# EdwardjkFeng/gradslam

Measured on AMD Instinct MI355X. Metric: RGB-D frames/sec (640x480, 10 ICP iters), higher is better.
Workload: dtype f32; 1 GPU; c2: ICP odometry localisation step, 640x480 TUM-shape synthetic RGB-D, batch 1 per GPU, dsratio 4 (~19k x ~19k points), 10 LM iterations, map 288269 points; parallelism=one sequence per GPU, final RCCL all_gather of poses, timing=one timed region of 1356 steps

## Files before the change

### gradslam_amd/_native.py

```python
import ctypes
import os
import subprocess

import torch

_HERE = os.path.dirname(os.path.abspath(__file__))
LIB_PATH = os.path.join(_HERE, "libgradslam_hip.so")
CSRC = os.path.join(_HERE, "csrc")

c_i, c_i64, c_f, c_p, c_sz = ctypes.c_int, ctypes.c_int64, ctypes.c_float, ctypes.c_void_p, ctypes.c_size_t

SIGNATURES = {
    "gs_abi_version": (c_i, []),
    "gs_last_error": (ctypes.c_char_p, []),
    "gs_vertex_normal_maps": (c_i, [c_p, c_p, c_p, c_i, c_i, c_i, c_i, c_p, c_p, c_p, c_p, c_p]),
    "gs_vertex_normal_maps_backward_ws_bytes": (c_sz, [c_i, c_i, c_i, c_i]),
    "gs_vertex_normal_maps_backward": (c_i, [c_p, c_p, c_p, c_i, c_i, c_i, c_i, c_p, c_p, c_p, c_p, c_p, c_p, c_p,
                                             c_p, c_sz, c_p]),
    "gs_vertex_normal_maps_backward_det_ws_bytes": (c_sz, [c_i, c_i, c_i, c_i]),
    "gs_vertex_normal_maps_backward_det": (c_i, [c_p, c_p, c_p, c_i, c_i, c_i, c_i, c_p, c_p, c_p, c_p, c_p, c_p, c_p,
                                                 c_p, c_sz, c_p]),
    "gs_get_alpha": (c_i, [c_p, c_i64, c_f, c_f, c_p, c_p]),
    "gs_get_alpha_backward": (c_i, [c_p, c_i64, c_f, c_f, c_p, c_p, c_p]),
    "gs_frames_from_raw": (c_i, [c_p, c_p, c_i, c_i, c_i, c_i, c_i, c_f, c_i, c_p, c_p, c_p]),
    "gs_compact_ws_bytes": (c_sz, [c_i64]),
    "gs_compact_rows": (c_i, [c_p, c_p, c_i64, c_i, c_p, c_p, c_p, c_sz, c_p]),
    "gs_compact_multi": (c_i, [c_i, c_p, c_p, c_p, c_p, c_i64, c_p, c_p, c_sz, c_p]),
    "gs_expand_multi": (c_i, [c_i, c_p, c_p, c_p, c_p, c_i64, c_p, c_sz, c_p]),
    "gs_append_rows_ws_bytes": (c_sz, [c_i64]),
    "gs_append_rows": (c_i, [c_i, c_p, c_p, c_p, c_p, c_i64, c_p, c_i, c_p, c_p, c_p, c_sz, c_p]),
    "gs_fusion_merge_inplace_ws_bytes": (c_sz, [c_i, c_i]),
    "gs_fusion_merge_inplace": (c_i, [c_p, c_p, c_i64, c_p, c_p, c_p, c_p, c_i, c_i, c_i, c_i, c_p, c_p, c_p, c_p, c_p, c_p,
                                      c_sz, c_p]),
    "gs_aggregate_update_ws_bytes": (c_sz, [c_i, c_i, c_i]),
    "gs_aggregate_update": (c_i, [c_p, c_p, c_p, c_p, c_i, c_i, c_i, c_p, c_p, c_p, c_p, c_i, c_p, c_p, c_sz, c_p]),
    "gs_pointfusion_update_ws_bytes": (c_sz, [c_i, c_i, c_i, c_i]),
    "gs_pointfusion_update": (c_i, [c_p, c_p, c_p, c_p, c_i, c_i, c_i, c_p, c_p, c_p, c_p, c_p, c_i, c_f, c_f, c_f, c_p, c_p,
                                    c_sz, c_p]),
    "gs_downsample_frame_ws_bytes": (c_sz, [c_i, c_i, c_i]),
    "gs_downsample_frame": (c_i, [c_p, c_p, c_p, c_p, c_i, c_i, c_i, c_i, c_i, c_p, c_p, c_p, c_p, c_p, c_p, c_sz, c_p]),
    "gs_build_icp_target_ws_bytes": (c_sz, [c_i, c_i, c_i, c_i]),
    "gs_build_icp_target": (c_i, [c_p, c_p, c_i64, c_i, c_i, c_i, c_i, c_p, c_p, c_i, c_i, c_p, c_p, c_p, c_p, c_p, c_p, c_p,
                                  c_p, c_p, c_sz, c_p]),
    "gs_bucket_by_pixel_ws_bytes": (c_sz, [c_i, c_i, c_i, c_i]),
    "gs_bucket_by_pixel": (c_i, [c_p, c_p, c_i64, c_i, c_i, c_i, c_i, c_p, c_i, c_i, c_p, c_p, c_p, c_p, c_p, c_sz, c_p]),
    "gs_project_active_ws_bytes": (c_sz, [c_i, c_i]),
    "gs_project_active": (c_i, [c_p, c_p, c_i, c_i, c_p, c_p, c_i, c_i, c_i, c_p, c_p, c_p, c_sz, c_p]),
    "gs_gather_table_rows_ws_bytes": (c_sz, [c_i]),
    "gs_gather_table_rows": (c_i, [c_p, c_p, c_i64, c_p, c_i, c_i, c_i, c_i, c_p, c_p, c_p, c_sz, c_p]),
    "gs_table_ds_mask": (c_i, [c_p, c_i64, c_i, c_p, c_p]),
    "gs_knn1_ws_bytes": (c_sz, [c_i]),
    "gs_knn1": (c_i, [c_p, c_p, c_i, c_p, c_p, c_i, c_p, c_p, c_sz, c_p]),
    "gs_knn1_bruteforce": (c_i, [c_p, c_p, c_i, c_p, c_p, c_i, c_p, c_p]),
    "gs_knn1_unpack": (c_i, [c_p, c_p, c_i, c_p, c_p, c_p]),
    "gs_icp_linearize_ws_bytes": (c_sz, [c_i]),
    "gs_icp_linearize": (c_i, [c_p, c_p, c_i, c_p, c_p, c_p, c_f, c_p, c_p, c_sz, c_p]),
    "gs_icp_rows": (c_i, [c_p, c_p, c_i, c_p, c_p, c_p, c_f, c_p, c_p, c_p, c_p]),
    "gs_icp_linearize_backward": (c_i, [c_p, c_p, c_i, c_p, c_p, c_p, c_f, c_p, c_p, c_p, c_p, c_p]),
    "gs_icp_linearize_backward_det_ws_bytes": (c_sz, [c_i, c_i]),
    "gs_icp_linearize_backward_det": (c_i, [c_p, c_p, c_i, c_p, c_p, c_p, c_i, c_p, c_f, c_p, c_p, c_p, c_p, c_p, c_sz, c_p]),
    "gs_transform_points": (c_i, [c_p, c_p, c_i, c_p, c_p, c_p]),
    "gs_icp_ws_bytes": (c_sz, [c_i, c_i]),
    "gs_icp_point_to_plane": (c_i, [c_p, c_p, c_i, c_p, c_p, c_p, c_i, c_p, c_i, c_f, c_f, c_p, c_p, c_p, c_p, c_p, c_sz,
                                    c_p]),
    "gs_icp_point_to_plane_grad": (c_i, [c_p, c_p, c_i, c_p, c_p, c_p, c_i, c_p, c_i, c_f, c_f, c_f, c_f, c_f, c_f,
                                         c_p, c_p, c_p, c_p, c_p, c_sz, c_p]),
    "gs_icp_tape_bytes": (c_sz, [c_i, c_i, c_i]),
    "gs_icp_point_to_plane_taped": (c_i, [c_p, c_p, c_i, c_p, c_p, c_p, c_i, c_p, c_i, c_f, c_f, c_i, c_f, c_f, c_f, c_f,
                                          c_p, c_p, c_p, c_p, c_sz, c_p, c_sz, c_p]),
    "gs_icp_backward_ws_bytes": (c_sz, [c_i]),
    "gs_icp_point_to_plane_backward": (c_i, [c_p, c_p, c_i, c_p, c_p, c_p, c_i, c_p, c_i, c_f, c_i, c_f, c_f, c_f, c_f, c_p, c_sz,
                                             c_p, c_p, c_p, c_p, c_p, c_p, c_sz, c_p]),
    "gs_icp_backward_det_ws_bytes": (c_sz, [c_i, c_i, c_i, c_i]),
    "gs_icp_point_to_plane_backward_det": (c_i, [c_p, c_p, c_i, c_p, c_p, c_p, c_i, c_p, c_i, c_f, c_i, c_f, c_f, c_f, c_f, c_p,
                                                 c_sz, c_p, c_p, c_p, c_p, c_p, c_p, c_sz, c_p]),
    "gs_slam_localize_tape_bytes": (c_sz, [c_i, c_i, c_i, c_i, c_i, c_i, c_i]),
    "gs_slam_localize_taped": (c_i, [c_p, c_p, c_p, c_p, c_i, c_i, c_i, c_i, c_p, c_p, c_p, c_i, c_i, c_i, c_f, c_f, c_f, c_f,
                                     c_f, c_f, c_p, c_p, c_sz, c_p, c_sz, c_p]),
    "gs_slam_localize_backward_ws_bytes": (c_sz, [c_i, c_i, c_i, c_i, c_i]),
    "gs_slam_localize_backward": (c_i, [c_p, c_i, c_i, c_i, c_i, c_p, c_p, c_i, c_i, c_i, c_f, c_f, c_f, c_f, c_f, c_p, c_sz,
                                        c_p, c_p, c_p, c_p, c_p, c_i, c_p, c_sz, c_p]),
    "gs_slam_localize_backward_det_ws_bytes": (c_sz, [c_i, c_i, c_i, c_i, c_i, c_i, c_i]),
    "gs_slam_localize_backward_det": (c_i, [c_p, c_i, c_i, c_i, c_i, c_p, c_p, c_i, c_i, c_i, c_f, c_f, c_f, c_f, c_f, c_p, c_sz,
                                            c_p, c_p, c_p, c_p, c_p, c_i, c_p, c_sz, c_p]),
    "gs_pointfusion_update_tape_bytes": (c_sz, [c_i, c_i, c_i]),
    "gs_pointfusion_update_taped": (c_i, [c_p, c_p, c_p, c_p, c_i, c_i, c_i, c_p, c_p, c_p, c_p, c_p, c_i, c_f, c_f, c_f, c_p, c_p,
                                          c_sz, c_p, c_sz, c_p]),
    "gs_pointfusion_update_backward_ws_bytes": (c_sz, [c_i, c_i, c_i]),
    "gs_pointfusion_update_backward": (c_i, [c_p, c_p, c_p, c_p, c_i, c_i, c_i, c_p, c_p, c_p, c_p, c_p, c_i, c_f, c_p, c_sz,
                                             c_p, c_p, c_p, c_p, c_p, c_p, c_p, c_p, c_p, c_sz, c_p]),
    "gs_compose_poses": (c_i, [c_p, c_p, c_i, c_p, c_p]),
    "gs_set_graph_mode": (None, [c_i]),
    "gs_graph_stats": (c_i, [ctypes.POINTER(ctypes.c_double)]),
    "gs_slam_localize_ws_bytes": (c_sz, [c_i, c_i, c_i, c_i, c_i]),
    "gs_slam_localize": (c_i, [c_p, c_p, c_p, c_i, c_i, c_i, c_i, c_p, c_p, c_p, c_i, c_i, c_i, c_f, c_f, c_f, c_f, c_f,
                               c_f, c_p, c_p, c_p, c_p, c_p, c_p, c_sz, c_p]),
    "gs_set_grid_search": (None, [c_i]),
    "gs_set_fused_setup": (None, [c_i]),
    "gs_set_tile_points": (None, [c_i]),
    "gs_set_loop_waves": (c_i, [c_i]),
    "gs_icp_launch_geometry": (c_i, [c_i, c_i, ctypes.POINTER(c_i), ctypes.POINTER(c_i), ctypes.POINTER(c_i)]),
    "gs_loop_counts": (c_i, [ctypes.POINTER(ctypes.c_uint), c_i]),
    "gs_profile_enable": (None, [c_i]),
    "gs_profile_read": (c_i, [c_i, ctypes.POINTER(ctypes.c_long), ctypes.POINTER(ctypes.c_double)]),
    "gs_fusion_similar": (c_i, [c_p, c_p, c_i64, c_p, c_p, c_i, c_i, c_p, c_p, c_i, c_f, c_f, c_p, c_p, c_p]),
    "gs_fusion_unique_ws_bytes": (c_sz, [c_i, c_i, c_i]),
    "gs_fusion_unique": (c_i, [c_p, c_p, c_p, c_i64, c_p, c_i, c_i, c_i, c_p, c_p, c_i, c_p, c_p, c_p, c_sz, c_p]),
    "gs_fusion_merge_ws_bytes": (c_sz, [c_i, c_i]),
    "gs_fusion_merge": (c_i, [c_p, c_p, c_i64, c_p, c_p, c_p, c_p, c_i, c_i, c_i, c_i, c_p, c_p, c_p, c_p, c_p, c_p,
                              c_p, c_p, c_p, c_p, c_sz, c_p]),
    "gs_fusion_merge_backward": (c_i, [c_p, c_p, c_i64, c_p, c_p, c_p, c_p, c_i, c_i, c_i, c_i, c_p, c_p, c_p, c_p,
                                       c_p, c_p, c_p, c_p, c_p, c_p, c_p, c_p, c_p, c_p, c_p, c_p, c_p, c_p, c_sz,
                                       c_p]),
    "gs_fusion_new_mask": (c_i, [c_p, c_p, c_p, c_i64, c_i, c_i, c_i, c_p, c_p]),
    "gs_render_map_ws_bytes": (c_sz, [c_i, c_i, c_i]),
    "gs_render_map": (c_i, [c_p, c_p, c_p, c_p, c_i, c_i, c_p, c_p, c_i, c_i, c_p, c_p, c_p, c_p, c_p, c_p, c_sz, c_p]),
    "gs_render_map_backward_ws_bytes": (c_sz, [c_i, c_i, c_i]),
    "gs_render_map_backward": (c_i, [c_p, c_p, c_i, c_i, c_p, c_i, c_i, c_p, c_p, c_p, c_p, c_p, c_p, c_p, c_p, c_p, c_p, c_sz,
                                     c_p]),
    "gs_chamfer_ws_bytes": (c_sz, [c_i, c_i, c_i]),
    "gs_chamfer": (c_i, [c_p, c_p, c_i, c_p, c_p, c_i, c_i, c_f, c_i, c_p, c_p, c_p, c_p, c_sz, c_p]),
    "gs_chamfer_backward_ws_bytes": (c_sz, [c_i, c_i, c_i]),
    "gs_chamfer_backward": (c_i, [c_p, c_p, c_i, c_p, c_p, c_i, c_i, c_p, c_p, c_p, c_p, c_p, c_p, c_p, c_sz, c_p]),
    "gs_chamfer_backward_det_ws_bytes": (c_sz, [c_i, c_i, c_i]),
    "gs_chamfer_backward_det": (c_i, [c_p, c_p, c_i, c_p, c_p, c_i, c_i, c_p, c_p, c_p, c_p, c_p, c_p, c_p, c_sz, c_p]),
}

_lib = None


def build(verbose: bool = False) -> str:
    cmd = ["make", "-s", "-C", CSRC, "-j4"]
    if verbose:
        cmd.remove("-s")
    subprocess.check_call(cmd)
    return LIB_PATH


def lib() -> ctypes.CDLL:
    global _lib
    if _lib is None:
        if not os.path.exists(LIB_PATH):
            raise RuntimeError(
                "gradslam_amd: native library {} is missing -- build it with "
                "`python -c 'import __graft_entry__ as g; g.build()'` (needs hipcc). "
                "There is no CPU / PyTorch fallback for the hot path.".format(LIB_PATH)
            )
        handle = ctypes.CDLL(LIB_PATH)
        for name, (res, args) in SIGNATURES.items():
            fn = getattr(handle, name)
            fn.restype, fn.argtypes = res, args
        if handle.gs_abi_version() != 3:
            raise RuntimeError("gradslam_amd: ABI version mismatch")
        _lib = handle
    return _lib


def ptr(t):
    return None if t is None else t.data_ptr()


_raw_stream = getattr(torch._C, "_cuda_getCurrentRawStream", None)
_raw_device = getattr(torch._C, "_cuda_getDevice", None)


def stream():
    if _raw_stream is not None and _raw_device is not None:
        return _raw_stream(_raw_device())
    return torch.cuda.current_stream().cuda_stream


def current_device_index() -> int:
    return _raw_device() if _raw_device is not None else torch.cuda.current_device()


def require_hip(*tensors, op: str = "op"):
    cur = None
    for t in tensors:
        if t is None:
            continue
        if not t.is_cuda:
            raise RuntimeError(
                "gradslam_amd.{}: tensor is on {}; the ICP / PointFusion hot path only runs on a HIP "
                "device (no CPU fallback is provided).".format(op, t.device)
            )
        if cur is None:
            cur = current_device_index()
        if t.device.index != cur:
            raise RuntimeError(
                "gradslam_amd.{}: tensor is on {} but the current HIP device is cuda:{}; kernels are launched on "
                "the current device's stream -- call torch.cuda.set_device({}) (or wrap the call in "
                "`with torch.cuda.device(...)`) first.".format(op, t.device, cur, t.device.index)
            )


def call(name: str, *args):
    rc = getattr(lib(), name)(*args)
    if rc != 0:
        msg = lib().gs_last_error().decode("utf-8", "replace")
        raise RuntimeError("{} failed (code {}): {}".format(name, rc, msg))


def ws_bytes(name: str, *args) -> int:
    return int(getattr(lib(), name)(*args))


_ws_cache = {}


def workspace(nbytes: int, device, tag: str = "default") -> torch.Tensor:
    key = (str(device), stream(), tag)
    buf = _ws_cache.get(key)
    if buf is None or buf.numel() < nbytes:
        buf = torch.empty(1 << max(int(nbytes) - 1, 255).bit_length(), dtype=torch.uint8, device=device)
        _ws_cache[key] = buf
    return buf
```

### gradslam_amd/csrc/gs_drivers.hpp

```cpp
#pragma once

#include "gs_common.hpp"
#include "gs_project.hpp"

namespace gs {

int vertex_normal_maps_cam(const float *depth, const float *intrinsics, const float *poses, int B, int H, int W, float *vertex,
                           float *normal, float *gvertex, float *gnormal, float *cam_out, hipStream_t st);
int vertex_normal_maps_fusion(const float *depth, const float *intrinsics, const float *poses, int B, int H, int W, float *gvertex,
                              float *gnormal, float *alpha, float sigma, float eps, unsigned long long *pix_key, unsigned int *pix_n,
                              int32_t *zero, int n_zero, hipStream_t st);

constexpr int kBucketPixMax = 24 * 1024;
size_t project_target1_ws_bytes(int H, int W, int ds, int Nmax);
int project_target1(const float *points, const int32_t *counts, int Nmax, const float *poses, const float *intrinsics, int H, int W, int ds,
                    const float *map_normals, int cap, int64_t *rows, int32_t *nrows, float *tgt, float *tnrm, int32_t *nt,
                    float *scan_points, int32_t *scan_orig, int32_t *pix_start, int32_t *tgt_index, int32_t *tgt_pix, void *ws,
                    size_t ws_bytes, hipStream_t st, const DsJob *frame);
int project_front1(const float *depth, const float *points, const int32_t *counts, int Nmax, const float *poses, const float *intrinsics,
                   int H, int W, int ds, const float *map_normals, int cap, float *vertex, float *normal, float *gvertex, float *gnormal,
                   float *cam_out, int32_t *row_pix, float *tgt, float *tnrm, int32_t *nt, int32_t *tgt_index, float *scan_points,
                   int32_t *scan_orig, int32_t *pix_start, const DsJob &frame, void *ws, size_t ws_bytes, hipStream_t st);

size_t fusion_corr_state_bytes(int B, int H, int W, int Nmax);
void fusion_corr_init_ptrs(void *state, int B, int H, int W, int Nmax, unsigned long long **pix_key, unsigned int **pix_n);
int fusion_correspond(void *state, const float *map_points, const float *map_normals, const float *map_ccounts, const int32_t *counts,
                      int B, int Nmax, const float *poses, const float *intrinsics, int H, int W, const float *gvertex,
                      const float *gnormal, float dist_th, float dot_th, int32_t *ctr, hipStream_t st);
int fusion_merge_corr(void *state, const int32_t *ctr, const float *gvertex, const float *gnormal, const float *rgb, const float *alpha,
                      int B, int H, int W, int Nmax, const int32_t *counts, float *points, float *normals, float *colors, float *ccounts,
                      hipStream_t st);
int fusion_append_corr(void *state, int B, int H, int W, int Nmax, int b, const float *depth, const float *const *h_src,
                       const int *h_row_floats, float *const *h_dst, const int32_t *d_count, int cap, int *d_total, void *cws,
                       hipStream_t st);
int fusion_finish(void *state, int B, int H, int W, int Nmax, int32_t *ctr, int32_t *counts, const int *totals, int cap, int32_t *appended,
                  int32_t *stats, hipStream_t st);
size_t fusion_tape_bytes(int B, int H, int W);
int fusion_tape_record(const void *state, void *tape, int B, int H, int W, int Nmax, const int32_t *counts, const float *points,
                       const float *normals, const float *colors, const float *ccounts, hipStream_t st);
int fusion_tape_appended(void *tape, int B, int H, int W, const int32_t *appended, hipStream_t st);
int fusion_update_reverse(const void *tape, int B, int H, int W, int Nmax, const float *depth, const float *gvertex, const float *gnormal,
                          const float *rgb, const float *alpha, float *points, float *normals, float *colors, float *ccounts,
                          int32_t *counts, float *Gp, float *Gn, float *Gc, float *Gcc, float *g_gvertex, float *g_gnormal, float *g_rgb,
                          float *g_alpha, void *cws, hipStream_t st);
int append_valid_pixels(int n_arrays, const float *depth_b, int64_t HW, const float *const *h_src, const int *h_row_floats,
                        float *const *h_dst, int32_t *d_count, int cap, int32_t *d_appended, int32_t *d_overflow, void *cws,
                        hipStream_t st);

}
```

### gradslam_amd/csrc/gs_icp.hpp

```cpp
#pragma once

#include "gs_common.hpp"

namespace gs {

bool profiling_enabled();
int icp_localize_run(int grad_lm, const float *src, const int32_t *d_ns, int max_ns, const float *tgt, const float *nrm,
                     const int32_t *d_nt, int max_nt, int numiters, float damp, float thresh, float lambda_max, float Bp,
                     float B2, float nu, const gs_icp_hints *hints, float *out_T, void *ws, size_t ws_bytes, hipStream_t st,
                     void *tape, size_t tape_bytes, const float *compose_right, float *compose_out);
int icp_config_stamp();

}
```

### gradslam_amd/csrc/gs_icp_loop.hpp

```cpp
#pragma once

#include "gs_icp_step.hpp"
#include "gs_project.hpp"

namespace gs {

struct LoopConst {
    const float *user_src, *tgt, *nrm, *boxes, *sboxes;
    const int32_t *d_ns, *d_nt;
    float *trace, *out_T;
    gs_icp_hints hints;
    GradParams gp;
    float thresh;
    int ns, nt;
    int cert_off;
    int tile_points;
    int grid_variant;
    CamK cam;
    int cam_ok;
    int32_t *cells;
    int cells_stride;
};

__device__ __forceinline__ f3 cam_point(const CamK &k, const f3 p) {
// ... 308 lines not shown
    }
    __syncthreads();
    if (step_mode >= 0 && blockIdx.x == 0 && threadIdx.x < kWords) {
        const int v = reinterpret_cast<const int *>(&st_sm)[threadIdx.x];
        reinterpret_cast<int *>(S_out)[threadIdx.x] = v;
        if (rec) reinterpret_cast<int *>(rec)[REC_WORDS + REC_STATE + threadIdx.x] = v;
    }
    GS_STAMP(7);
    const IcpState *S = &st_sm;
    if (tile0 >= ns) {
        if (threadIdx.x < NACC) partials[blockIdx.x * NACC + threadIdx.x] = 0.0f;
        return;
    }
    const int p_cur = S->p_cur, b_cur = S->b_cur;
    const float *in = first ? user_src : B.P(p_cur);
    float *out = B.P(out_slot >= 0 ? out_slot : 1 - p_cur);
    unsigned long long *best = B.N(out_slot >= 0 ? out_slot : 1 - b_cur);
    f3 s{0.0f, 0.0f, 0.0f};
    if (ok) {
        s = xform(S->dT, ld3(in, i));
        if (wave == 0) st3(out, i, s);
    }
    if (nt <= 0) {
        if (ok && wave == 0) best[i] = KEY_NONE;
        if (threadIdx.x < NACC) partials[blockIdx.x * NACC + threadIdx.x] = 0.0f;
        return;
    }
    unsigned long long key;
    bool need = false;
    int rel = 2;
    if (grid) {
        GS_STAMP(0);
        rel = sh.wflag[lane];
        if (wave == 0) {
            unsigned long long k0 = KEY_NONE;
            if (ok) {
                const int u = (first || b_cur == S_in->b_cur) ? 0 : 1;
                const float4 q = *reinterpret_cast<const float4 *>(sh.seed[u][lane]);
                k0 = pack_key(dist2(s, q.x, q.y, q.z), __float_as_int(q.w));
            }
            atomicMin(&sh.key[lane], k0);
        }
        {
            float bd = INFINITY;
            int bi = 0x7fffffff;
#pragma unroll
            for (int r = 0; r < WROWS; ++r) {
                const int wr = sh.win[r][lane];
                const int kk = (rel & 3) + r, wn = LaneWin::len(wr, nt);
                const int po = sh.band[WBANDS + min(kk, WBANDS - 1)];
                const float *row = sh.u.stage + 4 * (max(po, 0) + LaneWin::lo(wr) - sh.band[min(kk, WBANDS - 1)]);
                for (int p = wave; p < wn; p += NW) {
                    float4 q;
                    if (po >= 0) {
                        q = *reinterpret_cast<const float4 *>(row + 4 * p);
                    } else {
                        const int slot = LaneWin::lo(wr) + p;
                        const f3 g3 = ld3(C->hints.scan_points, slot);
                        q = make_float4(g3.x, g3.y, g3.z, __int_as_float(C->hints.scan_orig[slot]));
                    }
                    const float d = dist2(s, q.x, q.y, q.z);
                    const int jj = __float_as_int(q.w);
                    const bool better = (d < bd) | ((d == bd) & (jj < bi));
                    bd = better ? d : bd;
                    bi = better ? jj : bi;
                }
            }
            if (ok && bd < INFINITY) atomicMin(&sh.key[lane], pack_key(bd, bi));
        }
        __syncthreads();
        GS_STAMP(1);
        float bd;
        int bi;
        key_unpack(sh.key[lane], bd, bi);
        const float bound2 = (ok && C->cam_ok) ? cam_bound2(sh.cam, s, sh.centre[lane], rel >> 3) : 0.0f;
        const bool proven = !C->cert_off & ((rel & 4) != 0) & (bd * 1.0001f < bound2);
        need = ok & !proven;
        const unsigned long long need_mask = __ballot(need);
        GS_COUNT(12, (unsigned long long)__popcll(need_mask));
        bool tile_search = __popcll(need_mask) > 6;
        if (!tile_search && need_mask) {
            tile_search = !knn_point_search<NW>(sh, s, need_mask, C->hints.scan_points, C->hints.scan_orig, C->boxes, C->sboxes, nt);
        }
        if (tile_search) {
            tile_box(sh, s, need);
            __syncthreads();
            knn_prune_search<true, NW>(sh, s, ok, need, C->hints.scan_points, C->hints.scan_orig, C->boxes, C->sboxes, nt);
        }
        GS_STAMP(2);
        key = ok ? sh.key[lane] : KEY_NONE;
        GS_STAMP(3);
        GS_COUNT(5, ((unsigned long long)__builtin_amdgcn_s_getreg((31 << 11) | 4) << 16) |
                        ((unsigned long long)__builtin_amdgcn_s_getreg((31 << 11) | 20) << 48));
    } else {
        int sj = -1;
        if (!first) {
            sj = -2;
            if (wave == 0) {
                unsigned long long k0 = KEY_NONE;
                if (ok) {
                    const float4 q = *reinterpret_cast<const float4 *>(sh.seed[b_cur == S_in->b_cur ? 0 : 1][lane]);
                    k0 = pack_key(dist2(s, q.x, q.y, q.z), __float_as_int(q.w));
                }
                sh.key[lane] = k0;
            }
        }
        const bool window_seed = first && C->hints.scan_points && C->hints.src_pix && C->hints.pix_start && C->hints.grid_w > 0;
        if (window_seed) sj = -2;
        const float *scan = C->hints.scan_points ? C->hints.scan_points : C->tgt;
        const int32_t *scan_orig = C->hints.scan_points ? C->hints.scan_orig : nullptr;
        if (window_seed) knn_window_seed<NW>(sh, s, ok, i, C->hints, nt);
        key = knn_tile<NW>(sh, s, ok, sj, C->tgt, scan, scan_orig, C->boxes, C->sboxes, nt);
    }
    if (wave == 0) {
        if (ok) best[i] = key;
        if (grid && ok && C->cam_ok) C->cells[par * C->cells_stride + i] = cam_cell(sh.cam, s);
        float acc[NACC];
#pragma unroll
        for (int k = 0; k < NACC; ++k) acc[k] = 0.0f;
        const Row r = make_row_from(s, ok, key, C->tgt, C->nrm, C->thresh);
        if (r.valid) accumulate_row(r, acc);
#pragma unroll
        for (int k = 0; k < NACC; ++k) sh.u.a.rows[k][lane] = acc[k];
    }
    __syncthreads();
    static_assert(NACC * 16 <= NW * 64, "the J epilogue's first stage is one pass");
    if (threadIdx.x < NACC * 16) {
        const int k = threadIdx.x >> 4, p4 = (threadIdx.x & 15) * 4;
        sh.u.a.part[k][threadIdx.x & 15] = ((sh.u.a.rows[k][p4] + sh.u.a.rows[k][p4 + 1]) + sh.u.a.rows[k][p4 + 2]) + sh.u.a.rows[k][p4 + 3];
    }
    __syncthreads();
    if (threadIdx.x < NACC) {
        float v = 0.0f;
#pragma unroll
        for (int q = 0; q < 16; ++q) v += sh.u.a.part[threadIdx.x][q];
        partials[blockIdx.x * NACC + threadIdx.x] = v;
    }
}

__global__ void icp_init_state_k(IcpState *S, const float *__restrict__ init_T , float damp) {
    if (threadIdx.x == 0 && blockIdx.x == 0) {
        for (int i = 0; i < 16; ++i) {
            const float v = init_T ? init_T[i] : ((i % 5 == 0) ? 1.0f : 0.0f);
            S->T[i] = v; S->dT[i] = v;
        }
        for (int i = 0; i < 44; ++i) S->cur[i] = 0.0f;
        S->damp = damp;
        S->p_cur = 1;
        S->b_cur = 1; S->b_first = 0;
        S->it = 0;
    }
}

__global__ __launch_bounds__(SUPER * CHUNK) void icp_prepare_k(IcpState *S, const float *__restrict__ init_T, float damp,
                                                              const float *__restrict__ tgt, const int32_t *__restrict__ d_nt,
                                                              float *__restrict__ boxes, float *__restrict__ sboxes,
                                                              LoopConst lc, LoopConst *__restrict__ lc_out, float *__restrict__ part0,
                                                              float *__restrict__ part1, int rows_written, int rows_read) {
    static_assert(SUPER * CHUNK == 1024, "one block per super-box");
    for (int q = rows_written * NACC + blockIdx.x * blockDim.x + threadIdx.x; q < rows_read * NACC; q += gridDim.x * blockDim.x) {
        part0[q] = 0.0f; part1[q] = 0.0f;
    }
    __shared__ float wb[16][6];
    if (blockIdx.x == 0 && threadIdx.x < sizeof(LoopConst) / 4) {
        int v = reinterpret_cast<const int *>(&lc)[threadIdx.x];
        if (threadIdx.x == offsetof(LoopConst, ns) / 4) v = *lc.d_ns;
        if (threadIdx.x == offsetof(LoopConst, nt) / 4) v = *lc.d_nt;
        if (threadIdx.x == offsetof(LoopConst, tile_points) / 4) {
            atomicAdd(&g_loop_counts[0], 1u);
            if (lc.grid_variant) atomicAdd(&g_loop_counts[1], 1u);
            if (lc.tile_points != 64) atomicAdd(&g_loop_counts[2], 1u);
        }
        reinterpret_cast<int *>(lc_out)[threadIdx.x] = v;
    }
    if (lc.cells) {
        const int n = *lc.d_ns;
        int32_t *pix = lc.cells + 2 * (size_t)lc.cells_stride;
        for (int i = blockIdx.x * blockDim.x + threadIdx.x; i < lc.cells_stride; i += gridDim.x * blockDim.x)
            pix[i] = (i < n && lc.hints.src_pix) ? lc.hints.src_pix[i] : 0;
    }
    if (blockIdx.x == 0) {
        __syncthreads();
        if (threadIdx.x == 0 && lc.hints.cam_pose && lc.hints.cam_K && lc.hints.ds > 0) {
            const float *T = lc.hints.cam_pose, *K = lc.hints.cam_K;
            const Cam c = make_cam(T, K);
            for (int q = 0; q < 9; ++q) lc_out->cam.R[q] = c.R[q];
            for (int q = 0; q < 3; ++q) lc_out->cam.T[q] = c.tinv[q];
            lc_out->cam.fx = K[0]; lc_out->cam.fy = K[5]; lc_out->cam.cx = K[2]; lc_out->cam.cy = K[6];
            lc_out->cam.ds = lc.hints.ds; lc_out->cam.Wd = lc.hints.grid_w; lc_out->cam.Hd = lc.hints.grid_h;
            const bool pinhole = K[1] == 0.0f && K[3] == 0.0f && K[4] == 0.0f && K[7] == 0.0f && K[8] == 0.0f && K[9] == 0.0f &&
                                 K[10] == 1.0f && K[11] == 0.0f && K[0] != 0.0f && K[5] != 0.0f;
            lc_out->cam_ok = pinhole ? 1 : 0;
        }
    }
    if (threadIdx.x == 0 && blockIdx.x == 0) {
        for (int i = 0; i < 16; ++i) {
            const float v = init_T ? init_T[i] : ((i % 5 == 0) ? 1.0f : 0.0f);
            S->T[i] = v; S->dT[i] = v;
        }
        for (int i = 0; i < 44; ++i) S->cur[i] = 0.0f;
        for (int i = 0; i < 6; ++i) S->xi[i] = 0.0f;
        S->damp = damp;
        S->p_cur = 1;
        S->b_cur = 1; S->b_first = 0;
        S->it = 0;
    }
    const int nt = *d_nt;
    const int j = blockIdx.x * (SUPER * CHUNK) + threadIdx.x;
    if (blockIdx.x * (SUPER * CHUNK) >= nt) return;
    float lo[3] = {INFINITY, INFINITY, INFINITY}, hi[3] = {-INFINITY, -INFINITY, -INFINITY};
    if (j < nt) {
        const f3 p = ld3(tgt, j);
        lo[0] = hi[0] = p.x; lo[1] = hi[1] = p.y; lo[2] = hi[2] = p.z;
    }
#pragma unroll
    for (int a = 0; a < 3; ++a) {
#pragma unroll
        for (int off = CHUNK / 2; off > 0; off >>= 1) {
            lo[a] = fminf(lo[a], __shfl_xor(lo[a], off, kWave));
            hi[a] = fmaxf(hi[a], __shfl_xor(hi[a], off, kWave));
        }
    }
    if ((threadIdx.x % CHUNK) == 0 && j < nt) {
        float *b = boxes + 6 * (int64_t)(j / CHUNK);
        b[0] = lo[0]; b[1] = lo[1]; b[2] = lo[2]; b[3] = hi[0]; b[4] = hi[1]; b[5] = hi[2];
    }
#pragma unroll
    for (int a = 0; a < 3; ++a) {
#pragma unroll
        for (int off = 32; off >= CHUNK; off >>= 1) {
            lo[a] = fminf(lo[a], __shfl_xor(lo[a], off, kWave));
            hi[a] = fmaxf(hi[a], __shfl_xor(hi[a], off, kWave));
        }
    }
    const int lane = threadIdx.x & 63, wave = threadIdx.x >> 6;
    if (lane == 0) { wb[wave][0] = lo[0]; wb[wave][1] = lo[1]; wb[wave][2] = lo[2]; wb[wave][3] = hi[0]; wb[wave][4] = hi[1]; wb[wave][5] = hi[2]; }
    __syncthreads();
    if (threadIdx.x < 6) {
        float v = wb[0][threadIdx.x];
        for (int w = 1; w < 16; ++w) v = threadIdx.x < 3 ? fminf(v, wb[w][threadIdx.x]) : fmaxf(v, wb[w][threadIdx.x]);
        sboxes[6 * (int64_t)blockIdx.x + threadIdx.x] = v;
    }
}

__global__ void copy_best_last_k(const IcpState *__restrict__ S, LoopBufs B, const int32_t *__restrict__ d_ns,
                                 unsigned long long *__restrict__ out) {
    const unsigned long long *src = B.N(S->b_first);
    const int ns = *d_ns;
    for (int i = blockIdx.x * blockDim.x + threadIdx.x; i < ns; i += gridDim.x * blockDim.x) out[i] = src[i];
}

}
```

### gradslam_amd/csrc/icp.hip

```cpp
#include <stddef.h>
#include <stdlib.h>
#include <algorithm>
#include <vector>

#include "gs_detfold.hpp"
#include "gs_icp.hpp"
#include "gs_icp_reduce.hpp"

namespace gs {

__global__ __launch_bounds__(KNN_T) void knn1_brute_k(const float *__restrict__ src, const int32_t *__restrict__ d_ns,
                                                      const float *__restrict__ tgt, const int32_t *__restrict__ d_nt,
                                                      int nsplit, unsigned long long *__restrict__ best) {
    const int ns = *d_ns, nt = *d_nt;
    const int i = blockIdx.x * KNN_T + threadIdx.x;
    if (blockIdx.x * KNN_T >= ns) return;
    const int chunk = (nt + nsplit - 1) / nsplit;
    const int j0 = blockIdx.y * chunk, j1 = min(nt, j0 + chunk);
    const bool ok = i < ns;
    const f3 s = ok ? ld3(src, i) : f3{0.0f, 0.0f, 0.0f};
    float bd = INFINITY;
    int bi = 0;
    for (int j = j0; j < j1; ++j) {
        const float d = dist2(s, tgt[3 * j], tgt[3 * j + 1], tgt[3 * j + 2]);
        if (d < bd) { bd = d; bi = j; }
    }
    if (ok && bd < INFINITY) atomicMin(best + i, pack_key(bd, bi));
}

__global__ __launch_bounds__(64) void tgt_boxes_k(const float *__restrict__ tgt, const int32_t *__restrict__ d_nt,
                                                  float *__restrict__ boxes) {
    const int nt = *d_nt;
    const int j = blockIdx.x * 64 + threadIdx.x;
    if (blockIdx.x * 64 >= nt) return;
    float lo[3] = {INFINITY, INFINITY, INFINITY}, hi[3] = {-INFINITY, -INFINITY, -INFINITY};
    if (j < nt) {
        const f3 p = ld3(tgt, j);
        lo[0] = hi[0] = p.x; lo[1] = hi[1] = p.y; lo[2] = hi[2] = p.z;
    }
#pragma unroll
    for (int a = 0; a < 3; ++a) {
#pragma unroll
        for (int off = CHUNK / 2; off > 0; off >>= 1) {
            lo[a] = fminf(lo[a], __shfl_xor(lo[a], off, kWave));
            hi[a] = fmaxf(hi[a], __shfl_xor(hi[a], off, kWave));
        }
    }
    if ((threadIdx.x % CHUNK) == 0 && j < nt) {
        float *b = boxes + 6 * (int64_t)(j / CHUNK);
        b[0] = lo[0]; b[1] = lo[1]; b[2] = lo[2]; b[3] = hi[0]; b[4] = hi[1]; b[5] = hi[2];
    }
}

__global__ __launch_bounds__(KNN_BT) void knn1_box_k(const float *__restrict__ src, const int32_t *__restrict__ d_ns,
                                                     const float *__restrict__ tgt, const float *__restrict__ boxes,
                                                     const int32_t *__restrict__ d_nt, unsigned long long *__restrict__ best) {
    __shared__ KnnShared sh;
    const int ns = *d_ns, nt = *d_nt;
    const int tile0 = blockIdx.x * 64;
    if (tile0 >= ns) return;
    const int lane = threadIdx.x & 63, wave = threadIdx.x >> 6;
    const int i = tile0 + lane;
    const bool ok = i < ns;
    const f3 s = ok ? ld3(src, i) : f3{0.0f, 0.0f, 0.0f};
    if (nt <= 0) {
        if (ok && wave == 0) best[i] = KEY_NONE;
        return;
    }
    const unsigned long long key = knn_tile<KNN_NW>(sh, s, ok, -1, tgt, tgt, nullptr, boxes, nullptr, nt);
    if (ok && wave == 0) best[i] = key;
}

__global__ void knn_unpack_k(const unsigned long long *__restrict__ best, const int32_t *__restrict__ d_ns,
                             float *__restrict__ dist2_out, int64_t *__restrict__ idx) {
    const int ns = *d_ns;
    for (int i = blockIdx.x * blockDim.x + threadIdx.x; i < ns; i += gridDim.x * blockDim.x) {
        const unsigned long long k = best[i];
        if (dist2_out) dist2_out[i] = bitsf((uint32_t)(k >> 32));
        if (idx) idx[i] = (int64_t)(uint32_t)(k & 0xffffffffu);
    }
}

__global__ void fill_u64_k(unsigned long long *__restrict__ p, int n, unsigned long long v) {
    for (int i = blockIdx.x * blockDim.x + threadIdx.x; i < n; i += gridDim.x * blockDim.x) p[i] = v;
}

__global__ __launch_bounds__(LIN_T) void linearize_k(const float *__restrict__ src, const int32_t *__restrict__ d_ns,
                                                     const float *__restrict__ tgt, const float *__restrict__ nrm,
                                                     const unsigned long long *__restrict__ best, float thresh,
                                                     float *__restrict__ partials ) {
    const int ns = *d_ns;
    float acc[NACC];
#pragma unroll
    for (int k = 0; k < NACC; ++k) acc[k] = 0.0f;
    for (int i = blockIdx.x * LIN_T + threadIdx.x; i < ns; i += gridDim.x * LIN_T) {
        const Row r = make_row(src, tgt, nrm, best, i, ns, thresh);
        if (r.valid) accumulate_row(r, acc);
    }
    block_reduce_store(acc, partials);
}

__global__ __launch_bounds__(1024) void finalize44_k(const float *__restrict__ partials, int nblocks, float *__restrict__ out44) {
    __shared__ float acc[NACC];
    reduce_partials(partials, nblocks, acc);
    if (threadIdx.x == 0) expand44(acc, out44);
}

__global__ void icp_rows_k(const float *__restrict__ src, const int32_t *__restrict__ d_ns, const float *__restrict__ tgt,
                           const float *__restrict__ nrm, const unsigned long long *__restrict__ best, float thresh,
                           float *__restrict__ A, float *__restrict__ bvec, uint8_t *__restrict__ keep) {
    const int ns = *d_ns;
    for (int i = blockIdx.x * blockDim.x + threadIdx.x; i < ns; i += gridDim.x * blockDim.x) {
        const Row r = make_row(src, tgt, nrm, best, i, ns, thresh);
        keep[i] = r.valid ? 1 : 0;
#pragma unroll
        for (int u = 0; u < 6; ++u) A[6 * (int64_t)i + u] = r.valid ? r.a[u] : 0.0f;
        bvec[i] = r.valid ? r.b : 0.0f;
    }
}

template <bool DET>
__global__ void linearize_bwd_k(const float *__restrict__ src, const int32_t *__restrict__ d_ns,
                                const float *__restrict__ tgt, const float *__restrict__ nrm,
                                const unsigned long long *__restrict__ best, float thresh,
                                const float *__restrict__ gout , float *__restrict__ g_src,
                                float *__restrict__ g_tgt, float *__restrict__ g_nrm) {
    const int ns = *d_ns;
    __shared__ float G[43];
    if (threadIdx.x < 43) G[threadIdx.x] = gout[threadIdx.x];
    __syncthreads();
    for (int i = blockIdx.x * blockDim.x + threadIdx.x; i < ns; i += gridDim.x * blockDim.x) {
        const Row r = make_row(src, tgt, nrm, best, i, ns, thresh);
        if (!r.valid) {
            if (g_src) st3(g_src, i, f3{0, 0, 0});
            if (DET && g_tgt) det_store_none(g_tgt, i);
            continue;
        }
        const uint32_t j = (uint32_t)(best[i] & 0xffffffffu);
        const f3 s = ld3(src, i), d = ld3(tgt, j), n = ld3(nrm, j);
        float ab[6];
#pragma unroll
        for (int u = 0; u < 6; ++u) {
            float v = G[36 + u] * r.b;
#pragma unroll
            for (int w = 0; w < 6; ++w) v += (G[6 * u + w] + G[6 * w + u]) * r.a[w];
            ab[u] = v;
        }
        float bb = 2.0f * G[42] * r.b;
#pragma unroll
        for (int u = 0; u < 6; ++u) bb += G[36 + u] * r.a[u];
        const f3 an{ab[0], ab[1], ab[2]}, ac{ab[3], ab[4], ab[5]};
        f3 sb{n.y * ac.z - n.z * ac.y, n.z * ac.x - n.x * ac.z, n.x * ac.y - n.y * ac.x};
        f3 nb{an.x + (ac.y * s.z - ac.z * s.y), an.y + (ac.z * s.x - ac.x * s.z), an.z + (ac.x * s.y - ac.y * s.x)};
        sb.x -= bb * n.x; sb.y -= bb * n.y; sb.z -= bb * n.z;
        nb.x += bb * (d.x - s.x); nb.y += bb * (d.y - s.y); nb.z += bb * (d.z - s.z);
        if (g_src) st3(g_src, i, sb);
        if constexpr (DET) {
            if (g_tgt) det_store_row(g_tgt, i, f3{bb * n.x, bb * n.y, bb * n.z}, nb, (int)j);
            continue;
        }
        if (g_tgt) {
            atomicAdd(g_tgt + 3 * (int64_t)j, bb * n.x);
            atomicAdd(g_tgt + 3 * (int64_t)j + 1, bb * n.y);
            atomicAdd(g_tgt + 3 * (int64_t)j + 2, bb * n.z);
        }
        if (g_nrm) {
            atomicAdd(g_nrm + 3 * (int64_t)j, nb.x);
            atomicAdd(g_nrm + 3 * (int64_t)j + 1, nb.y);
            atomicAdd(g_nrm + 3 * (int64_t)j + 2, nb.z);
        }
    }
}

__global__ void transform_k(const float *__restrict__ pts, const int32_t *__restrict__ d_n, const float *__restrict__ T,
                            float *__restrict__ out) {
    const int n = *d_n;
    for (int i = blockIdx.x * blockDim.x + threadIdx.x; i < n; i += gridDim.x * blockDim.x) st3(out, i, xform(T, ld3(pts, i)));
}

}

#include "gs_icp_loop.hpp"
#include "gs_icp_bwd.hpp"

namespace gs {

static inline int knn_nsplit_brute(int max_ns, int max_nt) {
    const int tiles = cdiv(max_ns, KNN_T);
    int ns = cdiv(2048, tiles);
    const int cap = cdiv(max_nt, 64);
    if (ns > cap) ns = cap;
    if (ns < 1) ns = 1;
    if (ns > 4096) ns = 4096;
    return ns;
}
static inline int lin_blocks(int max_ns) {
    int nb = cdiv(max_ns, LIN_T);
    if (nb > LIN_MAXB) nb = LIN_MAXB;
    if (nb < 1) nb = 1;
    return nb;
}
static inline size_t boxes_bytes(int max_nt) { return align_up((size_t)cdiv(max_nt > 0 ? max_nt : 1, CHUNK) * 6 * 4, 256); }

struct Prof {
    bool on = false;
    std::vector<hipEvent_t> ev[2][2];
    size_t used[2] = {0, 0};
    double total_ms[2] = {0.0, 0.0};
    long count[2] = {0, 0};
};
static Prof g_prof;
static inline void prof_mark(int tag, int which, hipStream_t st) {
    if (!g_prof.on) return;
    auto &v = g_prof.ev[tag][which];
    const size_t i = g_prof.used[tag];
    if (i >= v.size()) {
        hipEvent_t e;
        if (hipEventCreate(&e) != hipSuccess) return;
        v.push_back(e);
    }
    (void)hipEventRecord(v[i], st);
    if (which == 1) g_prof.used[tag] = i + 1;
}

bool profiling_enabled() { return g_prof.on; }

static int g_grid_mode = getenv("GS_GRID_MODE") ? atoi(getenv("GS_GRID_MODE")) : 1;
static int g_tile_points = 0;
static int g_loop_waves = 0;

constexpr int TILE_MIN = 32;
static inline int loop_tile_points() {
    static const int env = getenv("GS_TILE_POINTS") ? atoi(getenv("GS_TILE_POINTS")) : 0;
    const int forced = g_tile_points ? g_tile_points : env;
    return (forced >= TILE_MIN && forced <= 64) ? forced : 64;
}
constexpr int LOOP_WAVES_DENSE = 64;
static inline int loop_waves(bool grid_search, int max_nt, int cells) {
    static const int env = getenv("GS_LOOP_WAVES") ? atoi(getenv("GS_LOOP_WAVES")) : 0;
    const int forced = g_loop_waves ? g_loop_waves : env;
    if (forced == 8 || forced == 16) return forced;
    return (grid_search && (int64_t)max_nt <= (int64_t)LOOP_WAVES_DENSE * cells) ? 8 : 16;
}
int icp_config_stamp() { return g_grid_mode | (g_tile_points << 4) | (g_loop_waves << 12); }
static inline int loop_blocks_max(int max_ns) { return cdiv(max_ns, TILE_MIN); }
static inline int partial_rows_alloc(int max_ns) { return std::max(loop_blocks_max(max_ns), 32 * RP_LOADS) + 1; }

struct IcpWs {
    IcpState *S[2];
    LoopBufs B;
    float *partials[2];
    float *boxes, *sboxes;
    LoopConst *lc;
    int32_t *cells;
};
static inline size_t icp_ws_layout(int max_ns, int max_nt, void *ws, IcpWs *out) {
    size_t off = 0;
    auto take = [&](size_t bytes) { size_t o = off; off += align_up(bytes, 256); return o; };
    const size_t oS = take(sizeof(IcpState)), oS1 = take(sizeof(IcpState));
    const size_t oP0 = take((size_t)max_ns * 12), oP1 = take((size_t)max_ns * 12);
    const size_t oB0 = take((size_t)max_ns * 8), oB1 = take((size_t)max_ns * 8);
    const size_t oPart = take((size_t)partial_rows_alloc(max_ns) * NACC * 4), oPart1 = take((size_t)partial_rows_alloc(max_ns) * NACC * 4);
    const size_t oBox = take(boxes_bytes(max_nt)), oSBox = take((size_t)cdiv(max_nt > 0 ? max_nt : 1, 1024) * 6 * 4);
    const size_t oLc = take(sizeof(LoopConst)), oCells = take((size_t)max_ns * 12);
    if (ws && out) {
        char *p = (char *)ws;
        out->S[0] = (IcpState *)(p + oS); out->S[1] = (IcpState *)(p + oS1);
        out->B.pts = (float *)(p + oP0);
        out->B.pts_stride = (int64_t)(oP1 - oP0) / 4;
        out->B.best = (unsigned long long *)(p + oB0);
        out->B.best_stride = (int64_t)(oB1 - oB0) / 8;
        out->partials[0] = (float *)(p + oPart); out->partials[1] = (float *)(p + oPart1);
        out->boxes = (float *)(p + oBox);
        out->sboxes = (float *)(p + oSBox);
        out->lc = (LoopConst *)(p + oLc);
        out->cells = (int32_t *)(p + oCells);
    }
    return off;
}

struct Tape {
    float *rec;
    LoopBufs B;
    int nslots;
};
static inline int tape_launches(bool grad, int numiters) { return grad ? 2 * numiters : numiters + 1; }
static inline size_t tape_layout(bool grad, int max_ns, int numiters, void *tape, Tape *out) {
    const int n = tape_launches(grad, numiters > 0 ? numiters : 1);
    const size_t rec_b = align_up((size_t)(n + 1) * REC_WORDS * 4, 256);
    const size_t pts_b = align_up((size_t)max_ns * 12, 256), best_b = align_up((size_t)max_ns * 8, 256);
    if (tape && out) {
        char *p = (char *)tape;
        out->rec = (float *)p;
        out->B.pts = (float *)(p + rec_b);
        out->B.pts_stride = (int64_t)pts_b / 4;
        out->B.best = (unsigned long long *)(p + rec_b + (size_t)n * pts_b);
        out->B.best_stride = (int64_t)best_b / 8;
        out->nslots = n;
    }
    return rec_b + (size_t)n * (pts_b + best_b);
}

static inline GradParams make_grad_params(float lambda_max, float B, float B2, float nu) {
    return GradParams{(float)(1.0 / (double)lambda_max), (float)((double)lambda_max - 1.0 / (double)lambda_max), B, B2,
                      (float)(1.0 / (double)nu)};
}
static inline GradParams lm_grad_params() { return GradParams{0.5f, 1.5f, 1.0f, 1.0f, 0.005f}; }

static int icp_run(bool grad, const float *src, const int32_t *d_ns, int max_ns, const float *tgt, const float *nrm,
                   const int32_t *d_nt, int max_nt, const float *init_T, int numiters, float damp, float thresh,
                   GradParams gp, const gs_icp_hints *hints_in, float *out_T, uint64_t *best_last, float *trace, void *ws,
                   size_t ws_bytes, hipStream_t st, const char *name, void *tape = nullptr, size_t tape_bytes = 0,
                   const float *compose_right = nullptr, float *compose_out = nullptr) {
    gs_icp_hints hints{nullptr, nullptr, nullptr, nullptr, nullptr, 0, 0, nullptr, nullptr, 0};
    if (hints_in) hints = *hints_in;
    GS_REQUIRE(!hints.scan_points || hints.scan_orig, "%s: hints.scan_points needs hints.scan_orig", name);
    GS_REQUIRE(src && d_ns && tgt && nrm && d_nt && out_T, "%s: NULL argument", name);
    GS_REQUIRE(max_ns > 0 && max_nt > 0 && numiters >= 0, "%s: bad sizes max_ns=%d max_nt=%d numiters=%d", name, max_ns, max_nt, numiters);
    if (!ws || ws_bytes < icp_ws_layout(max_ns, max_nt, nullptr, nullptr)) {
        set_error("%s: workspace too small (%zu < %zu)", name, ws_bytes, icp_ws_layout(max_ns, max_nt, nullptr, nullptr));
        return GS_ERR_WORKSPACE_TOO_SMALL;
    }
    if (numiters == 0) {
        if (init_T) {
            GS_HIP(hipMemcpyAsync(out_T, init_T, 64, hipMemcpyDeviceToDevice, st), name);
        } else {
            hipLaunchKernelGGL(icp_init_state_k, dim3(1), dim3(64), 0, st, (IcpState *)ws, init_T, damp);
            GS_HIP(hipMemcpyAsync(out_T, ws, 64, hipMemcpyDeviceToDevice, st), name);
        }
        return GS_OK;
    }
    IcpWs w;
    icp_ws_layout(max_ns, max_nt, ws, &w);
    Tape tp{nullptr, {}, 0};
    if (tape) {
        if (tape_bytes < tape_layout(grad, max_ns, numiters, nullptr, nullptr)) {
            set_error("%s: tape too small (%zu < %zu)", name, tape_bytes, tape_layout(grad, max_ns, numiters, nullptr, nullptr));
            return GS_ERR_WORKSPACE_TOO_SMALL;
        }
        tape_layout(grad, max_ns, numiters, tape, &tp);
        w.B = tp.B;
    }
    int n_assoc = 0, n_step = 0;
    const int tile_points = loop_tile_points();
    const dim3 kgrid(cdiv(max_ns, tile_points));
    const int lb = (int)kgrid.x;
    const int fb = min(cdiv(max_ns, 256), 256);

    static const int cert_off = getenv("GS_CERT_OFF") != nullptr;
    static const bool grid_off = getenv("GS_NO_GRID_SEARCH") != nullptr;
    const bool grid_search = !grid_off && g_grid_mode != 0 && hints.scan_points && hints.scan_orig && hints.src_pix && hints.pix_start &&
                             hints.cam_pose && hints.cam_K && hints.ds > 0 && hints.grid_w > 0 && hints.grid_h > 0;
    LoopConst lc{src, tgt, nrm, w.boxes, w.sboxes, d_ns, d_nt, trace, out_T, hints, gp, thresh, 0, 0, cert_off, tile_points,
                 grid_search ? 1 : 0, CamK{}, 0, w.cells, max_ns};
    hipLaunchKernelGGL(icp_prepare_k, dim3(cdiv(max_nt, SUPER * CHUNK)), dim3(SUPER * CHUNK), 0, st, w.S[0], init_T, damp,
                       hints.scan_points ? hints.scan_points : tgt, d_nt, w.boxes, w.sboxes, lc, w.lc, w.partials[0], w.partials[1], lb,
                       std::max(lb, 32 * RP_LOADS));
    GS_LAUNCH_CHECK(name);
    int cur = 0;
    int pending = -1;
    int pending_slot = -1;
    const bool fold = (int)kgrid.x <= 2 * 256;
    auto assoc = [&](int first) {
        if (!fold && pending >= 0) {
            hipLaunchKernelGGL(icp_step_k, dim3(1), dim3(1024), 0, st, w.S[cur], w.partials[cur], lb, pending, gp, trace, out_T,
                               pending_slot, tape ? tp.rec + (size_t)n_step * REC_WORDS : nullptr, 1, (const float *)nullptr,
                               (float *)nullptr);
            ++n_step;
            pending = -1;
        }
        const int nxt = pending >= 0 ? 1 - cur : cur;
        prof_mark(0, 0, st);
        float *rec_p = (tape && pending >= 0) ? tp.rec + (size_t)n_step * REC_WORDS : nullptr;
        const int nw = loop_waves(grid_search, max_nt, hints.grid_w * hints.grid_h);
        auto launch_nw = [&](auto kernel, int waves) {
            hipLaunchKernelGGL(kernel, kgrid, dim3(waves * 64), 0, st, (const LoopConst *)w.lc, (const IcpState *)w.S[cur], (const float *)w.partials[cur],
                               (const int32_t *)(w.cells + 2 * (size_t)max_ns), (const int32_t *)(w.cells + (size_t)(1 - (n_assoc & 1)) * max_ns),
                               max_ns, tile_points, first | ((n_assoc & 1) << 1), pending, pending_slot, lb, w.S[nxt], rec_p,
                               tape ? n_assoc : -1, w.B, w.partials[nxt], src);
        };
        auto launch = [&](auto k16, auto k8) {
            if (nw == 16) launch_nw(k16, 16); else launch_nw(k8, 8);
        };
        if (grid_search && lb <= 32 * RP_FEW) launch(knn1_loop_k<true, RP_FEW, 16>, knn1_loop_k<true, RP_FEW, 8>);
        else if (grid_search) launch(knn1_loop_k<true, RP_LOADS, 16>, knn1_loop_k<true, RP_LOADS, 8>);
        else launch(knn1_loop_k<false, RP_LOADS, 16>, knn1_loop_k<false, RP_LOADS, 8>);
        prof_mark(0, 1, st);
        if (pending >= 0) ++n_step;
        cur = nxt;
        pending = -1;
        ++n_assoc;
    };
    auto step = [&](int mode) {
        pending = mode;
        pending_slot = tape ? n_assoc - 1 : -1;
    };
    auto finish = [&]() {
        hipLaunchKernelGGL(icp_step_k, dim3(1), dim3(1024), 0, st, w.S[cur], w.partials[cur], lb, pending, gp, trace, out_T,
                           pending_slot, tape ? tp.rec + (size_t)n_step * REC_WORDS : nullptr, 0, compose_right, compose_out);
        ++n_step;
        pending = -1;
    };
    assoc(1);
    step(STEP_ADOPT);
    if (!grad) {
        for (int it = 0; it < numiters; ++it) {
            assoc(0);
            step(STEP_LM);
        }
    } else {
        for (int it = 0; it < numiters; ++it) {
            assoc(0);
            step(STEP_GRAD_B);
            if (it + 1 < numiters) {
                assoc(0);
                step(STEP_ADOPT);
            }
        }
    }
    finish();
    GS_LAUNCH_CHECK(name);
    if (best_last) {
        hipLaunchKernelGGL(copy_best_last_k, dim3(fb), dim3(256), 0, st, w.S[cur], w.B, d_ns, (unsigned long long *)best_last);
        GS_LAUNCH_CHECK(name);
    }
    return GS_OK;
}

static inline int bwd_launches(bool grad, int numiters) { return grad ? 2 * numiters : numiters; }
static inline size_t bwd_det_ws_bytes(bool grad, int max_ns, int max_nt, int numiters) {
    return align_up(bwd_ws_layout(max_ns, nullptr, nullptr), 256) +
           det_ws_layout(bwd_launches(grad, numiters > 0 ? numiters : 1), max_ns, max_nt, nullptr, nullptr);
}

static int icp_backward_run(bool grad, const float *src, const int32_t *d_ns, int max_ns, const float *tgt, const float *nrm,
                            const int32_t *d_nt, int max_nt, const float *init_T, int numiters, float thresh, GradParams gp, const void *tape,
                            size_t tape_bytes, const float *grad_T, float *g_src, float *g_tgt, float *g_nrm, float *g_init_T,
                            void *ws, size_t ws_bytes, hipStream_t st, bool det = false) {
    const char *name = det ? "gs_icp_backward_det" : "gs_icp_backward";
    GS_REQUIRE(src && d_ns && tgt && nrm && d_nt && init_T && tape && grad_T && g_src && g_init_T, "%s: NULL argument", name);
    GS_REQUIRE(max_ns > 0 && max_nt > 0 && numiters >= 0, "%s: bad sizes", name);
    GS_REQUIRE(!det || bwd_launches(grad, numiters) <= 65535, "%s: too many iterations for the deterministic fold", name);
    if (!ws || ws_bytes < (det ? bwd_det_ws_bytes(grad, max_ns, max_nt, numiters) : bwd_ws_layout(max_ns, nullptr, nullptr))) {
        set_error("%s: workspace too small", name);
        return GS_ERR_WORKSPACE_TOO_SMALL;
    }
    GS_REQUIRE(tape_bytes >= tape_layout(grad, max_ns, numiters, nullptr, nullptr), "%s: tape too small", name);
    Tape tp;
    tape_layout(grad, max_ns, numiters, (void *)tape, &tp);
    BwdWs w;
    bwd_ws_layout(max_ns, ws, &w);
    DetWs dw{};
    const bool fold = det && (g_tgt || g_nrm);
    if (fold) det_ws_layout(bwd_launches(grad, numiters), max_ns, max_nt, (char *)ws + align_up(bwd_ws_layout(max_ns, nullptr, nullptr), 256), &dw);
    auto rows_of = [&](int q) { return fold ? dw.rows + (size_t)q * max_ns * DET_ROW : nullptr; };
    float *walk_nrm = det ? nullptr : g_nrm;
    const int nb = min(cdiv(max_ns, BWD_T), BWD_MAXB);
    int cur = 0;
    hipLaunchKernelGGL(bwd_begin_k, dim3(min(cdiv(3 * max(max_nt, max_ns), 256), 1024)), dim3(256), 0, st, w.S[0], grad_T, w.gP, 3 * max_ns,
                       w.partials[0], nb * 12, det ? nullptr : g_tgt, walk_nrm, d_nt, max_nt);
    for (int k = numiters - 1, q = 0; k >= 0; --k) {
        if (!grad) {
            const float *rec = tp.rec + (size_t)(1 + k) * REC_WORDS;
            float *gt = det ? rows_of(q++) : g_tgt;
            hipLaunchKernelGGL(det ? bwd_lin_k<true> : bwd_lin_k<false>, dim3(nb), dim3(BWD_T), 0, st, (const BwdState *)w.S[cur],
                               w.S[1 - cur], (int)FOLD_LM, rec, (const float *)w.partials[cur], nb, k, 1, tp.B, src, d_ns, tgt, nrm, thresh,
                               w.gP, gt, walk_nrm, w.partials[1 - cur]);
            cur = 1 - cur;
        } else {
            const float *rec = tp.rec + (size_t)(1 + 2 * k) * REC_WORDS;
            float *gt = det ? rows_of(q++) : g_tgt;
            hipLaunchKernelGGL(det ? bwd_look_k<true> : bwd_look_k<false>, dim3(nb), dim3(BWD_T), 0, st, (const BwdState *)w.S[cur],
                               w.S[1 - cur], rec, (const float *)w.partials[cur], nb, gp, k == 0 ? -1 : (k == 1 ? 0 : 2 * (k - 1)), tp.B, d_ns,
                               tgt, nrm, thresh, w.gP, gt, walk_nrm, w.partials[1 - cur]);
            cur = 1 - cur;
            gt = det ? rows_of(q++) : g_tgt;
            hipLaunchKernelGGL(det ? bwd_lin_k<true> : bwd_lin_k<false>, dim3(nb), dim3(BWD_T), 0, st, (const BwdState *)w.S[cur],
                               w.S[1 - cur], (int)FOLD_G2, rec, (const float *)w.partials[cur], nb, 0, 0, tp.B, src, d_ns, tgt, nrm, thresh,
                               w.gP, gt, walk_nrm, w.partials[1 - cur]);
            cur = 1 - cur;
        }
    }
    hipLaunchKernelGGL(bwd_finish_k, dim3(nb), dim3(BWD_T), 0, st, init_T, d_ns, (const float *)w.gP, g_src, (const BwdState *)w.S[cur],
                       (const float *)w.partials[cur], nb, g_init_T);
    GS_LAUNCH_CHECK(name);
    if (fold) return det_fold_run(dw, bwd_launches(grad, numiters), max_ns, d_ns, d_nt, max_nt, g_tgt, g_nrm, st, name);
    return GS_OK;
}

int icp_localize_run(int grad_lm, const float *src, const int32_t *d_ns, int max_ns, const float *tgt, const float *nrm,
                     const int32_t *d_nt, int max_nt, int numiters, float damp, float thresh, float lambda_max, float Bp,
                     float B2, float nu, const gs_icp_hints *hints, float *out_T, void *ws, size_t ws_bytes, hipStream_t st,
                     void *tape, size_t tape_bytes, const float *compose_right, float *compose_out) {
    const GradParams gp = grad_lm ? make_grad_params(lambda_max, Bp, B2, nu) : lm_grad_params();
    return icp_run(grad_lm != 0, src, d_ns, max_ns, tgt, nrm, d_nt, max_nt, nullptr, numiters, damp, thresh, gp, hints, out_T, nullptr,
                   nullptr, ws, ws_bytes, st, "gs_slam_localize/icp", tape, tape_bytes, compose_right, compose_out);
}

}

using namespace gs;

extern "C" {

#ifdef GS_DIAG_STAMPS
int gs_diag_set_buffer(void *p) {
    return (int)hipMemcpyToSymbol(HIP_SYMBOL(g_diag), &p, sizeof(p));
}
#endif

void gs_set_grid_search(int on) { g_grid_mode = on; }
void gs_set_tile_points(int n) { g_tile_points = n; }
int gs_set_loop_waves(int n) {
    if (n == 0 || n == 8 || n == 16) g_loop_waves = n;
    return g_loop_waves;
}
int gs_icp_launch_geometry(int max_ns, int have_hints, int *blocks, int *tile_points_dense, int *partial_rows) {
    GS_REQUIRE(max_ns > 0, "gs_icp_launch_geometry: max_ns must be positive");
    (void)have_hints;
    const int tp = loop_tile_points();
    if (blocks) *blocks = cdiv(max_ns, tp);
    if (tile_points_dense) *tile_points_dense = tp;
    if (partial_rows) *partial_rows = partial_rows_alloc(max_ns);
    return GS_OK;
}

int gs_loop_counts(unsigned int *out4, int reset) {
    GS_REQUIRE(out4, "gs_loop_counts: NULL argument");
    GS_HIP(hipMemcpyFromSymbol(out4, HIP_SYMBOL(g_loop_counts), 16), "gs_loop_counts");
    if (reset) {
        const unsigned int z[4] = {0, 0, 0, 0};
        GS_HIP(hipMemcpyToSymbol(HIP_SYMBOL(g_loop_counts), z, 16), "gs_loop_counts/reset");
    }
    return GS_OK;
}

void gs_profile_enable(int on) {
    g_prof.on = on != 0;
    for (int t = 0; t < 2; ++t) { g_prof.used[t] = 0; g_prof.total_ms[t] = 0.0; g_prof.count[t] = 0; }
}

int gs_profile_read(int tag, long *launches, double *total_ms) {
    GS_REQUIRE(tag == 0 || tag == 1, "gs_profile_read: tag must be 0 or 1");
    for (int t = 0; t < 2; ++t) {
        for (size_t i = 0; i < g_prof.used[t]; ++i) {
            float ms = 0.0f;
            if (hipEventElapsedTime(&ms, g_prof.ev[t][0][i], g_prof.ev[t][1][i]) == hipSuccess) {
                g_prof.total_ms[t] += ms;
                g_prof.count[t] += 1;
            }
        }
        g_prof.used[t] = 0;
    }
    if (launches) *launches = g_prof.count[tag];
    if (total_ms) *total_ms = g_prof.total_ms[tag];
    return GS_OK;
}

size_t gs_knn1_ws_bytes(int max_nt) { return boxes_bytes(max_nt); }

int gs_knn1(const float *src, const int32_t *d_ns, int max_ns, const float *tgt, const int32_t *d_nt, int max_nt,
            uint64_t *best, void *ws, size_t ws_bytes, gs_stream_t stream) {
    GS_REQUIRE(src && d_ns && tgt && d_nt && best, "gs_knn1: NULL argument");
    GS_REQUIRE(max_ns >= 0 && max_nt >= 0, "gs_knn1: negative size");
    if (max_ns == 0) return GS_OK;
    hipStream_t st = (hipStream_t)stream;
    if (max_nt == 0) {
        hipLaunchKernelGGL(fill_u64_k, dim3(min(cdiv(max_ns, 256), 1024)), dim3(256), 0, st, (unsigned long long *)best, max_ns, KEY_NONE);
        GS_LAUNCH_CHECK("gs_knn1/fill");
        return GS_OK;
    }
    if (!ws || ws_bytes < boxes_bytes(max_nt)) {
        set_error("gs_knn1: workspace too small (%zu < %zu)", ws_bytes, boxes_bytes(max_nt));
        return GS_ERR_WORKSPACE_TOO_SMALL;
    }
    hipLaunchKernelGGL(tgt_boxes_k, dim3(cdiv(max_nt, 64)), dim3(64), 0, st, tgt, d_nt, (float *)ws);
    GS_LAUNCH_CHECK("gs_knn1/boxes");
    hipLaunchKernelGGL(knn1_box_k, dim3(cdiv(max_ns, 64)), dim3(KNN_BT), 0, st, src, d_ns, tgt, (const float *)ws, d_nt,
                       (unsigned long long *)best);
    GS_LAUNCH_CHECK("gs_knn1");
    return GS_OK;
}

int gs_knn1_bruteforce(const float *src, const int32_t *d_ns, int max_ns, const float *tgt, const int32_t *d_nt,
                       int max_nt, uint64_t *best, gs_stream_t stream) {
    GS_REQUIRE(src && d_ns && tgt && d_nt && best, "gs_knn1_bruteforce: NULL argument");
    GS_REQUIRE(max_ns >= 0 && max_nt >= 0, "gs_knn1_bruteforce: negative size");
    if (max_ns == 0) return GS_OK;
    hipStream_t st = (hipStream_t)stream;
    hipLaunchKernelGGL(fill_u64_k, dim3(min(cdiv(max_ns, 256), 1024)), dim3(256), 0, st, (unsigned long long *)best, max_ns, KEY_NONE);
    GS_LAUNCH_CHECK("gs_knn1_bruteforce/fill");
    if (max_nt == 0) return GS_OK;
    const int nsplit = knn_nsplit_brute(max_ns, max_nt);
    hipLaunchKernelGGL(knn1_brute_k, dim3(cdiv(max_ns, KNN_T), nsplit), dim3(KNN_T), 0, st, src, d_ns, tgt, d_nt, nsplit,
                       (unsigned long long *)best);
    GS_LAUNCH_CHECK("gs_knn1_bruteforce");
    return GS_OK;
}

int gs_knn1_unpack(const uint64_t *best, const int32_t *d_ns, int max_ns, float *dist2, int64_t *idx, gs_stream_t stream) {
    GS_REQUIRE(best && d_ns && max_ns >= 0, "gs_knn1_unpack: bad arguments");
    if (max_ns == 0) return GS_OK;
    hipLaunchKernelGGL(knn_unpack_k, dim3(min(cdiv(max_ns, 256), 1024)), dim3(256), 0, (hipStream_t)stream,
                       (const unsigned long long *)best, d_ns, dist2, idx);
    GS_LAUNCH_CHECK("gs_knn1_unpack");
    return GS_OK;
}

size_t gs_icp_linearize_ws_bytes(int max_ns) { (void)max_ns; return align_up((size_t)LIN_MAXB * NACC * 4, 256); }

int gs_icp_linearize(const float *src, const int32_t *d_ns, int max_ns, const float *tgt, const float *tgt_normals,
                     const uint64_t *best, float dist_thresh, float *out44, void *ws, size_t ws_bytes,
                     gs_stream_t stream) {
    GS_REQUIRE(src && d_ns && tgt && tgt_normals && best && out44, "gs_icp_linearize: NULL argument");
    GS_REQUIRE(max_ns >= 0, "gs_icp_linearize: negative size");
    if (!ws || ws_bytes < gs_icp_linearize_ws_bytes(max_ns)) {
        set_error("gs_icp_linearize: workspace too small");
        return GS_ERR_WORKSPACE_TOO_SMALL;
    }
    hipStream_t st = (hipStream_t)stream;
    const int nb = lin_blocks(max_ns);
    hipLaunchKernelGGL(linearize_k, dim3(nb), dim3(LIN_T), 0, st, src, d_ns, tgt, tgt_normals,
                       (const unsigned long long *)best, dist_thresh, (float *)ws);
    GS_LAUNCH_CHECK("gs_icp_linearize");
    hipLaunchKernelGGL(finalize44_k, dim3(1), dim3(1024), 0, st, (const float *)ws, nb, out44);
    GS_LAUNCH_CHECK("gs_icp_linearize/finalize");
    return GS_OK;
}

int gs_icp_rows(const float *src, const int32_t *d_ns, int max_ns, const float *tgt, const float *tgt_normals,
                const uint64_t *best, float dist_thresh, float *A, float *b, uint8_t *keep, gs_stream_t stream) {
    GS_REQUIRE(src && d_ns && tgt && tgt_normals && best && A && b && keep, "gs_icp_rows: NULL argument");
    if (max_ns <= 0) return GS_OK;
    hipLaunchKernelGGL(icp_rows_k, dim3(min(cdiv(max_ns, 256), 2048)), dim3(256), 0, (hipStream_t)stream, src, d_ns, tgt,
                       tgt_normals, (const unsigned long long *)best, dist_thresh, A, b, keep);
    GS_LAUNCH_CHECK("gs_icp_rows");
    return GS_OK;
}

int gs_icp_linearize_backward(const float *src, const int32_t *d_ns, int max_ns, const float *tgt,
                              const float *tgt_normals, const uint64_t *best, float dist_thresh, const float *g_out43,
                              float *g_src, float *g_tgt, float *g_normals, gs_stream_t stream) {
    GS_REQUIRE(src && d_ns && tgt && tgt_normals && best && g_out43, "gs_icp_linearize_backward: NULL argument");
    if (max_ns <= 0) return GS_OK;
    hipLaunchKernelGGL(linearize_bwd_k<false>, dim3(min(cdiv(max_ns, 256), 2048)), dim3(256), 0, (hipStream_t)stream, src, d_ns,
                       tgt, tgt_normals, (const unsigned long long *)best, dist_thresh, g_out43, g_src, g_tgt, g_normals);
    GS_LAUNCH_CHECK("gs_icp_linearize_backward");
    return GS_OK;
}
// ... 120 lines not shown
```

### gradslam_amd/csrc/project.hip

```cpp
#include "gs_common.hpp"
#include "gs_compact.hpp"
#include "gs_drivers.hpp"
#include "gs_maps.hpp"
#include "gs_project.hpp"

namespace gs {

constexpr int kCamB = 32;
__device__ __forceinline__ Cam *cam_cache() {
    __shared__ Cam cams[kCamB];
    return cams;
}

__global__ void build_cams_k(const float *__restrict__ poses, const float *__restrict__ Ks, int B, Cam *__restrict__ cams) {
    const int b = blockIdx.x * blockDim.x + threadIdx.x;
    if (b >= B) return;
    const float *T = poses + 16 * b;
    Cam c;
#pragma unroll
    for (int i = 0; i < 3; ++i)
#pragma unroll
        for (int j = 0; j < 3; ++j) c.R[3 * i + j] = T[4 * i + j];
    const float t0 = T[3], t1 = T[7], t2 = T[11];
#pragma unroll
    for (int j = 0; j < 3; ++j) {
        c.tinv[j] = ((-T[j]) * t0 + (-T[4 + j]) * t1) + (-T[8 + j]) * t2;
    }
#pragma unroll
    for (int i = 0; i < 16; ++i) c.K[i] = Ks[16 * b + i];
    cams[b] = c;
}

struct ActivePred {
    const float *points;
    const int32_t *counts;
    const Cam *cams;
    int Nmax, H, W, ds;
    float umax, vmax;
    __device__ bool operator()(int64_t i) const {
        const int b = (int)(i / Nmax), n = (int)(i - (int64_t)b * Nmax);
        if (n >= counts[b]) return false;
        int h, w;
        if (!project_point(cams[b], ld3(points, i), H, W, umax, vmax, h, w)) return false;
        return ds <= 0 || ((h % ds == 0) && (w % ds == 0));
    }
};
struct ActiveWriter {
    const float *points;
    const Cam *cams;
    int64_t *rows;
    int Nmax, H, W;
    float umax, vmax;
    __device__ void operator()(int64_t i, int64_t pos) const {
        const int b = (int)(i / Nmax), n = (int)(i - (int64_t)b * Nmax);
        int h, w;
        project_point(cams[b], ld3(points, i), H, W, umax, vmax, h, w);
        st_table_row(rows, pos, b, n, h, w);
    }
};

struct ActivePredL {
    const float *points;
    const int32_t *counts;
    const float *poses, *Ks;
    int B, Nmax, H, W, ds;
    float umax, vmax;
    __device__ void block_init(int , int , int ) const {
        for (int b = threadIdx.x; b < B; b += blockDim.x) cam_cache()[b] = make_cam(poses + 16 * b, Ks + 16 * b);
    }
    struct Item { f3 p; };
    __device__ Item fetch(int64_t i) const { return Item{ld3(points, i)}; }
    __device__ bool test(const Item &it, int64_t i) const {
        const int b = (int)(i / Nmax), n = (int)(i - (int64_t)b * Nmax);
        if (n >= counts[b]) return false;
        int h, w;
        if (!project_point(cam_cache()[b], it.p, H, W, umax, vmax, h, w)) return false;
        return ds <= 0 || ((h % ds == 0) && (w % ds == 0));
    }
    __device__ bool operator()(int64_t i) const { return test(fetch(i), i); }
};
struct ActiveWriterL {
    const float *points;
    int64_t *rows;
    int Nmax, H, W;
    float umax, vmax;
    __device__ void put(const ActivePredL::Item &it, int64_t i, int64_t pos) const {
        const int b = (int)(i / Nmax), n = (int)(i - (int64_t)b * Nmax);
        int h, w;
        project_point(cam_cache()[b], it.p, H, W, umax, vmax, h, w);
        longlong4 r;
        r.x = b; r.y = n; r.z = h; r.w = w;
        st_table_row(rows, pos, r);
    }
    __device__ void operator()(int64_t i, int64_t pos) const { put(ActivePredL::Item{ld3(points, i)}, i, pos); }
};

struct ActivePredH {
    const float *points;
    const int32_t *counts;
    const float *poses, *Ks;
    int Nmax, H, W, ds;
    float umax, vmax;
    int *cnt, *fill;
    int npix;
    __device__ void block_init(int pass, int bid, int nb) const {
        if (threadIdx.x == 0) cam_cache()[0] = make_cam(poses, Ks);
        if (pass == 0)
            for (int i = bid * blockDim.x + threadIdx.x; i < npix; i += nb * blockDim.x) { cnt[i] = 0; fill[i] = 0; }
    }
    struct Item { f3 p; };
    __device__ Item fetch(int64_t i) const { return Item{ld3(points, i)}; }
    __device__ bool test(const Item &it, int64_t i) const {
        if (i >= counts[0]) return false;
        int h, w;
        if (!project_point(cam_cache()[0], it.p, H, W, umax, vmax, h, w)) return false;
        return (h % ds == 0) && (w % ds == 0);
    }
    __device__ bool operator()(int64_t i) const { return test(fetch(i), i); }
};
struct ActiveWriterH {
    const float *points;
    int64_t *rows;
    int H, W, ds, Wd;
    float umax, vmax;
    int *cnt;
    __device__ void put(const ActivePredH::Item &it, int64_t i, int64_t pos) const {
        int h, w;
        project_point(cam_cache()[0], it.p, H, W, umax, vmax, h, w);
        st_table_row(rows, pos, 0, i, h, w);
        atomicAdd(cnt + (h / ds) * Wd + (w / ds), 1);
    }
    __device__ void operator()(int64_t i, int64_t pos) const { put(ActivePredH::Item{ld3(points, i)}, i, pos); }
};

struct ActiveWriterT {
    const float *points, *normals;
    int H, W, ds, Wd;
    float umax, vmax;
    int *cnt;
    int cap;
    float *tgt, *tnrm;
    int32_t *tgt_index;
    int32_t *row_pix;
    __device__ void put(const ActivePredH::Item &it, int64_t i, int64_t pos) const {
        int h, w;
        project_point(cam_cache()[0], it.p, H, W, umax, vmax, h, w);
        const int pix = (h / ds) * Wd + (w / ds);
        atomicAdd(cnt + pix, 1);
        row_pix[pos] = pix;
        if (pos < cap) {
            st3(tgt, pos, it.p);
            st3(tnrm, pos, ld3(normals, i));
            if (tgt_index) tgt_index[pos] = (int32_t)i;
        }
    }
    __device__ void operator()(int64_t i, int64_t pos) const { put(ActivePredH::Item{ld3(points, i)}, i, pos); }
};

__global__ void table_starts_k(const int64_t *__restrict__ rows, const int32_t *__restrict__ d_n, int B, int32_t *__restrict__ starts) {
    const int b = blockIdx.x * blockDim.x + threadIdx.x;
    if (b > B) return;
    const int n = *d_n;
    int lo = 0, hi = n;
    while (lo < hi) {
        const int mid = (lo + hi) >> 1;
        if (rows[4 * (int64_t)mid] < b) lo = mid + 1; else hi = mid;
    }
    starts[b] = lo;
}

__global__ void gather_table_k(const int64_t *__restrict__ rows, const int32_t *__restrict__ d_n,
                               const int32_t *__restrict__ starts, const float *__restrict__ attr, int B, int Nmax, int C,
                               int cap, float *__restrict__ out, int32_t *__restrict__ counts) {
    const int n = *d_n;
    if (blockIdx.x == 0 && threadIdx.x < B && counts) counts[threadIdx.x] = starts[threadIdx.x + 1] - starts[threadIdx.x];
    for (int64_t i = (int64_t)blockIdx.x * blockDim.x + threadIdx.x; i < n; i += (int64_t)gridDim.x * blockDim.x) {
        const int b = (int)rows[4 * i], p = (int)rows[4 * i + 1];
        const int k = (int)(i - starts[b]);
        if (k >= cap) continue;
        const float *s = attr + ((int64_t)b * Nmax + p) * C;
        float *d = out + ((int64_t)b * cap + k) * C;
        for (int c = 0; c < C; ++c) d[c] = s[c];
    }
}

__global__ void table_ds_mask_k(const int64_t *__restrict__ rows, int64_t n, int ds, uint8_t *__restrict__ mask) {
    for (int64_t i = (int64_t)blockIdx.x * blockDim.x + threadIdx.x; i < n; i += (int64_t)gridDim.x * blockDim.x)
        mask[i] = ((rows[4 * i + 2] % ds) == 0 && (rows[4 * i + 3] % ds) == 0) ? 1 : 0;
}

__global__ void pix_count_k(const int64_t *__restrict__ rows, const int32_t *__restrict__ d_n,
                            const int32_t *__restrict__ starts, int Wd, int npix, int ds, int *__restrict__ cnt) {
    const int n = *d_n;
    for (int64_t i = (int64_t)blockIdx.x * blockDim.x + threadIdx.x; i < n; i += (int64_t)gridDim.x * blockDim.x) {
        const longlong4 r = ld_table_row(rows, i);
        const int b = (int)r.x;
        const int pix = (int)(r.z / ds) * Wd + (int)(r.w / ds);
        atomicAdd(cnt + (int64_t)b * npix + pix, 1);
    }
}
constexpr int PIX_TILE = 24 * 1024;
__global__ __launch_bounds__(1024) void pix_scan_k(const int *__restrict__ cnt, int npix, int *__restrict__ start) {
    __shared__ int sm[1024 / 64 + 1];
    __shared__ int bins[PIX_TILE];
    __shared__ int carry;
    const int b = blockIdx.x;
    cnt += (int64_t)b * npix; start += (int64_t)b * (npix + 1);
    if (threadIdx.x == 0) carry = 0;
    __syncthreads();
    for (int t0 = 0; t0 < npix; t0 += PIX_TILE) {
        const int nb = min(PIX_TILE, npix - t0);
        for (int i = threadIdx.x; i < nb; i += 1024) bins[i] = cnt[t0 + i];
        __syncthreads();
        const int per = (nb + 1023) / 1024;
        const int i0 = min(nb, (int)threadIdx.x * per), i1 = min(nb, i0 + per);
        int sum = 0;
        for (int i = i0; i < i1; ++i) sum += bins[i];
        int total;
        int run = carry + block_excl_scan<1024>(sum, sm, &total);
        for (int i = i0; i < i1; ++i) { const int c = bins[i]; bins[i] = run; run += c; }
        __syncthreads();
        for (int i = threadIdx.x; i < nb; i += 1024) start[t0 + i] = bins[i];
        if (threadIdx.x == 0) carry += total;
        __syncthreads();
    }
    if (threadIdx.x == 0) start[npix] = carry;
}
__global__ void pix_scatter_k(const int64_t *__restrict__ rows, const int32_t *__restrict__ d_n,
                              const int32_t *__restrict__ starts, int Wd, int npix, int ds,
                              const int *__restrict__ start, int *__restrict__ fill, const float *__restrict__ map_points,
                              int Nmax, int cap, float *__restrict__ scan_pts, int32_t *__restrict__ scan_orig,
                              int32_t *__restrict__ tgt_pix ) {
    const int n = *d_n;
    for (int64_t i = (int64_t)blockIdx.x * blockDim.x + threadIdx.x; i < n; i += (int64_t)gridDim.x * blockDim.x) {
        const longlong4 r = ld_table_row(rows, i);
        const int b = (int)r.x;
        const int pix = (int)(r.z / ds) * Wd + (int)(r.w / ds);
        const int k = (int)(i - starts[b]);
        if (tgt_pix && k < cap) tgt_pix[(int64_t)b * cap + k] = pix;
        const int slot = start[(int64_t)b * (npix + 1) + pix] + atomicAdd(fill + (int64_t)b * npix + pix, 1);
        if (slot >= cap) continue;
        st3(scan_pts, (int64_t)b * cap + slot, ld3(map_points, (int64_t)b * Nmax + r.y));
        scan_orig[(int64_t)b * cap + slot] = (int32_t)k;
    }
}
__global__ void tgt_init_k(int *__restrict__ cnt, int *__restrict__ fill, int64_t n, const int64_t *__restrict__ rows,
                           const int32_t *__restrict__ d_n, int B, int32_t *__restrict__ starts) {
    for (int64_t i = (int64_t)blockIdx.x * blockDim.x + threadIdx.x; i < n; i += (int64_t)gridDim.x * blockDim.x) {
        cnt[i] = 0; fill[i] = 0;
    }
    if (blockIdx.x == 0) {
        for (int b = threadIdx.x; b <= B; b += blockDim.x) {
            int lo = 0, hi = *d_n;
            while (lo < hi) {
                const int mid = (lo + hi) >> 1;
                if (rows[4 * (int64_t)mid] < b) lo = mid + 1; else hi = mid;
            }
            starts[b] = lo;
        }
    }
}
__global__ void tgt_gather_count_k(const int64_t *__restrict__ rows, const int32_t *__restrict__ d_n,
                                   const int32_t *__restrict__ starts, const float *__restrict__ map_points,
                                   const float *__restrict__ map_normals, int B, int Nmax, int cap,
                                   float *__restrict__ tgt, float *__restrict__ tnrm, int32_t *__restrict__ counts, int Wd,
                                   int npix, int ds, int *__restrict__ cnt, int32_t *__restrict__ tgt_index) {
    const int n = *d_n;
    if (blockIdx.x == 0 && threadIdx.x < B) counts[threadIdx.x] = starts[threadIdx.x + 1] - starts[threadIdx.x];
    for (int64_t i = (int64_t)blockIdx.x * blockDim.x + threadIdx.x; i < n; i += (int64_t)gridDim.x * blockDim.x) {
        const longlong4 r = ld_table_row(rows, i);
        const int b = (int)r.x;
        const int k = (int)(i - starts[b]);
        const int pix = (int)(r.z / ds) * Wd + (int)(r.w / ds);
        atomicAdd(cnt + (int64_t)b * npix + pix, 1);
        if (k >= cap) continue;
        const int64_t src = (int64_t)b * Nmax + r.y, dst = (int64_t)b * cap + k;
        st3(tgt, dst, ld3(map_points, src));
        st3(tnrm, dst, ld3(map_normals, src));
        if (tgt_index) tgt_index[dst] = (int32_t)r.y;
    }
}

__global__ void tgt_scatter_gather1_k(const int64_t *__restrict__ rows, const int32_t *__restrict__ d_n,
                                      const float *__restrict__ map_points, const float *__restrict__ map_normals, int cap,
                                      float *__restrict__ tgt, float *__restrict__ tnrm, int32_t *__restrict__ counts,
                                      int32_t *__restrict__ tgt_index, int Wd, int ds, const int *__restrict__ start,
                                      int *__restrict__ fill, float *__restrict__ scan_pts, int32_t *__restrict__ scan_orig,
                                      int32_t *__restrict__ tgt_pix ) {
    const int n = *d_n;
    if (blockIdx.x == 0 && threadIdx.x == 0) counts[0] = n;
    for (int64_t i = (int64_t)blockIdx.x * blockDim.x + threadIdx.x; i < n; i += (int64_t)gridDim.x * blockDim.x) {
        const longlong4 r = ld_table_row(rows, i);
        const f3 p = ld3(map_points, r.y);
        if (i < cap) {
            st3(tgt, i, p);
            st3(tnrm, i, ld3(map_normals, r.y));
            if (tgt_index) tgt_index[i] = (int32_t)r.y;
        }
        const int pix = (int)(r.z / ds) * Wd + (int)(r.w / ds);
        if (tgt_pix && i < cap) tgt_pix[i] = pix;
        const int slot = start[pix] + atomicAdd(fill + pix, 1);
        if (slot >= cap) continue;
        st3(scan_pts, slot, p);
        scan_orig[slot] = (int32_t)i;
    }
}

}

using namespace gs;

extern "C" {

size_t gs_project_active_ws_bytes(int B, int Nmax) {
    return align_up(sizeof(Cam) * (size_t)(B > 0 ? B : 1), 256) + compact_ws_bytes((int64_t)B * Nmax);
}

int gs_project_active(const float *points, const int32_t *counts, int B, int Nmax, const float *poses,
                      const float *intrinsics, int H, int W, int ds, int64_t *out_rows, int32_t *out_count, void *ws,
                      size_t ws_bytes, gs_stream_t stream) {
    GS_REQUIRE(points && counts && poses && intrinsics && out_rows && out_count, "gs_project_active: NULL argument");
    GS_REQUIRE(B > 0 && Nmax > 0 && H > 0 && W > 0, "gs_project_active: bad shape B=%d Nmax=%d H=%d W=%d", B, Nmax, H, W);
    if (!ws || ws_bytes < gs_project_active_ws_bytes(B, Nmax)) {
        set_error("gs_project_active: workspace too small (%zu < %zu)", ws_bytes, gs_project_active_ws_bytes(B, Nmax));
        return GS_ERR_WORKSPACE_TOO_SMALL;
    }
    hipStream_t st = (hipStream_t)stream;
    Cam *cams = (Cam *)ws;
    void *cws = (char *)ws + align_up(sizeof(Cam) * (size_t)B, 256);
    const float umax = (float)((double)W - 0.999), vmax = (float)((double)H - 0.999);
    if (B <= kCamB) {
        ActivePredL pred{points, counts, poses, intrinsics, B, Nmax, H, W, ds, umax, vmax};
        ActiveWriterL wr{points, out_rows, Nmax, H, W, umax, vmax};
        return compact_launch((int64_t)B * Nmax, pred, wr, out_count, cws, st, "gs_project_active");
    }
    hipLaunchKernelGGL(build_cams_k, dim3(cdiv(B, 64)), dim3(64), 0, st, poses, intrinsics, B, cams);
    GS_LAUNCH_CHECK("gs_project_active/cams");
    ActivePred pred{points, counts, cams, Nmax, H, W, ds, umax, vmax};
    ActiveWriter wr{points, cams, out_rows, Nmax, H, W, umax, vmax};
    return compact_launch((int64_t)B * Nmax, pred, wr, out_count, cws, st, "gs_project_active");
}

}

namespace gs {
size_t project_target1_ws_bytes(int H, int W, int ds, int Nmax) {
    const size_t npix = (size_t)cdiv(H, ds) * cdiv(W, ds);
    return compact_ws_bytes(Nmax) + 2 * align_up(npix * 4, 256) + compact_flags_bytes(Nmax) + compact_ws_bytes((int64_t)npix);
}
int project_target1(const float *points, const int32_t *counts, int Nmax, const float *poses, const float *intrinsics, int H,
                    int W, int ds, const float *map_normals, int cap, int64_t *rows, int32_t *nrows, float *tgt, float *tnrm,
                    int32_t *nt, float *scan_points, int32_t *scan_orig, int32_t *pix_start, int32_t *tgt_index, int32_t *tgt_pix,
                    void *ws, size_t ws_bytes, hipStream_t st, const DsJob *frame) {
    const char *name = "gs_slam_localize/target";
    if (!ws || ws_bytes < project_target1_ws_bytes(H, W, ds, Nmax)) {
        set_error("%s: workspace too small", name);
        return GS_ERR_WORKSPACE_TOO_SMALL;
    }
    const int Wd = cdiv(W, ds), npix = cdiv(H, ds) * Wd;
    char *p = (char *)ws;
    void *cws = p; p += compact_ws_bytes(Nmax);
    int *cnt = (int *)p, *fill = (int *)(p + align_up((size_t)npix * 4, 256));
    unsigned char *flags = (unsigned char *)(p + 2 * align_up((size_t)npix * 4, 256));
    const float umax = (float)((double)W - 0.999), vmax = (float)((double)H - 0.999);
    ActivePredH pred{points, counts, poses, intrinsics, Nmax, H, W, ds, umax, vmax, cnt, fill, npix};
    ActiveWriterH wr{points, rows, H, W, ds, Wd, umax, vmax, cnt};
    int rc;
    if (frame) {
        const int Hd = cdiv(H, ds);
        DsPred dp{frame->depth, W, Wd, ds};
        DsWriter dw{frame->gvertex, nullptr, nullptr, frame->out_points, nullptr, nullptr, frame->out_pix, W, Wd, ds};
        void *dws = (char *)flags + compact_flags_bytes(Nmax);
        if (compact_blocks((int64_t)Hd * Wd) <= kSelfScanBlocks) {
            rc = compact_launch2((int64_t)Nmax, pred, wr, nrows, cws, flags, (int64_t)Hd * Wd, dp, dw, frame->count, dws, st, name);
        } else {
            rc = compact_launch((int64_t)Hd * Wd, dp, dw, frame->count, dws, st, name);
            if (rc == GS_OK) rc = compact_launch((int64_t)Nmax, pred, wr, nrows, cws, st, name, flags);
        }
    } else {
        rc = compact_launch((int64_t)Nmax, pred, wr, nrows, cws, st, name, flags);
    }
    if (rc) return rc;
    hipLaunchKernelGGL(pix_scan_k, dim3(1), dim3(1024), 0, st, cnt, npix, pix_start);
    hipLaunchKernelGGL(tgt_scatter_gather1_k, dim3(min(cdiv(Nmax, 256), 1024)), dim3(256), 0, st, rows, nrows, points, map_normals, cap,
                       tgt, tnrm, nt, tgt_index, Wd, ds, pix_start, fill, scan_points, scan_orig, tgt_pix);
    GS_LAUNCH_CHECK(name);
    return GS_OK;
}

template <class PA, class PB>
__global__ __launch_bounds__(kCT) void setup_count_k(int64_t nA, PA pa, int *__restrict__ countsA, unsigned char *__restrict__ flagsA, int nbA,
                                                     int64_t nB, PB pb, int *__restrict__ countsB, int nbB, const float *__restrict__ depth,
                                                     const float *__restrict__ Ks, const float *__restrict__ poses, int H, int W, int gx,
                                                     float *__restrict__ vertex, float *__restrict__ normal, float *__restrict__ gvertex,
                                                     float *__restrict__ gnormal, VnExtra ex) {
    static_assert(kCT == TW * TH, "one block size for all three jobs");
    const int bid = (int)blockIdx.x;
    if (bid < nbA) {
        compact_count_body(nA, pa, countsA, flagsA, bid, nbA);
    } else if (bid < nbA + nbB) {
        compact_count_body(nB, pb, countsB, (unsigned char *)nullptr, bid - nbA, nbB);
    } else {
        const int t = bid - nbA - nbB;
        vertex_normal_body(depth, Ks, poses, 1, H, W, vertex, normal, gvertex, gnormal, ex, t % gx, t / gx, 0);
    }
}

constexpr int kBucketBlocks = 128;
__global__ __launch_bounds__(1024) void bucket_scatter_k(const float *__restrict__ tgt, const int32_t *__restrict__ d_nt, int cap,
                                                         const int32_t *__restrict__ row_pix, const int *__restrict__ cnt,
                                                         int *__restrict__ fill, int npix, int32_t *__restrict__ pix_start,
                                                         float *__restrict__ scan_pts, int32_t *__restrict__ scan_orig) {
    __shared__ int starts[kBucketPixMax];
    __shared__ int sm[1024 / 64 + 1];
    const int nt = *d_nt;
    for (int i = threadIdx.x; i < npix; i += 1024) starts[i] = cnt[i];
    const int stride = gridDim.x * 1024;
    int r = blockIdx.x * 1024 + threadIdx.x, pix = 0;
    f3 p{0.0f, 0.0f, 0.0f};
    if (r < nt) { pix = row_pix[r]; p = ld3(tgt, r); }
    __syncthreads();
    const int per = (npix + 1023) / 1024;
    const int i0 = min(npix, (int)threadIdx.x * per), i1 = min(npix, i0 + per);
    int sum = 0;
    for (int i = i0; i < i1; ++i) sum += starts[i];
    int total;
    int run = block_excl_scan<1024>(sum, sm, &total);
    for (int i = i0; i < i1; ++i) { const int c = starts[i]; starts[i] = run; run += c; }
    __syncthreads();
    if (blockIdx.x == 0) {
        for (int i = threadIdx.x; i < npix; i += 1024) pix_start[i] = starts[i];
        if (threadIdx.x == 0) pix_start[npix] = total;
    }
    for (; r < nt; r += stride) {
        const int slot = starts[pix] + atomicAdd(fill + pix, 1);
        const int rn = r + stride;
        int pn = 0;
        f3 pp{0.0f, 0.0f, 0.0f};
        if (rn < nt) { pn = row_pix[rn]; pp = ld3(tgt, rn); }
        if (slot < cap) {
            st3(scan_pts, slot, p);
            scan_orig[slot] = r;
        }
        pix = pn; p = pp;
    }
}

int project_front1(const float *depth, const float *points, const int32_t *counts, int Nmax, const float *poses, const float *intrinsics,
                   int H, int W, int ds, const float *map_normals, int cap, float *vertex, float *normal, float *gvertex, float *gnormal,
                   float *cam_out, int32_t *row_pix, float *tgt, float *tnrm, int32_t *nt, int32_t *tgt_index, float *scan_points,
                   int32_t *scan_orig, int32_t *pix_start, const DsJob &frame, void *ws, size_t ws_bytes, hipStream_t st) {
    const char *name = "gs_slam_localize/front";
    if (!ws || ws_bytes < project_target1_ws_bytes(H, W, ds, Nmax)) {
        set_error("%s: workspace too small", name);
        return GS_ERR_WORKSPACE_TOO_SMALL;
    }
    const int Wd = cdiv(W, ds), Hd = cdiv(H, ds), npix = Hd * Wd;
    if (npix > kBucketPixMax) {
        set_error("%s: ds-grid too large for the fused form", name);
        return GS_ERR_INVALID_ARG;
    }
    int *cnt = (int *)ws, *fill = (int *)((char *)ws + align_up((size_t)npix * 4, 256));
    char *p = (char *)ws + 2 * align_up((size_t)npix * 4, 256);
    int *countsA = (int *)p; p += compact_ws_bytes(Nmax);
    unsigned char *flags = (unsigned char *)p; p += compact_flags_bytes(Nmax);
    int *countsB = (int *)p;
    const float umax = (float)((double)W - 0.999), vmax = (float)((double)H - 0.999);
    ActivePredH pa{points, counts, poses, intrinsics, Nmax, H, W, ds, umax, vmax, cnt, fill, npix};
    ActiveWriterT wa{points, map_normals, H, W, ds, Wd, umax, vmax, cnt, cap, tgt, tnrm, tgt_index, row_pix};
    DsPred pb{frame.depth, W, Wd, ds};
    DsWriter wb{frame.gvertex, nullptr, nullptr, frame.out_points, nullptr, nullptr, frame.out_pix, W, Wd, ds};
    const int64_t nA = Nmax, nB = (int64_t)npix;
    const int nbA = compact_blocks(nA), nbB = compact_blocks(nB), gx = cdiv(W, TW), nbV = depth ? gx * cdiv(H, TH) : 0;
    if (nbB > kSelfScanBlocks) {
        set_error("%s: ds-grid too large for the fused form", name);
        return GS_ERR_INVALID_ARG;
    }
    const VnExtra ex{nullptr, 1.0f, 0.0f, nullptr, nullptr, nullptr, 0, cam_out};
    hipLaunchKernelGGL((setup_count_k<ActivePredH, DsPred>), dim3(nbA + nbB + nbV), dim3(kCT), 0, st, nA, pa, countsA, flags, nbA, nB, pb,
                       countsB, nbB, depth, intrinsics, poses, H, W, gx, vertex, normal, gvertex, gnormal, ex);
    GS_LAUNCH_CHECK(name);
    if (nbA <= kSelfScanBlocks) {
        hipLaunchKernelGGL((compact_write2_k<ActivePredH, ActiveWriterT, true, DsPred, DsWriter>), dim3(nbA + nbB), dim3(kCT), 0, st, nA, pa, wa,
                           (const int *)countsA, nt, (const unsigned char *)flags, nbA, nB, pb, wb, (const int *)countsB, frame.count, nbB);
    } else {
        int *offsetsA = countsA + nbA;
        hipLaunchKernelGGL(compact_scan_k, dim3(1), dim3(1024), 0, st, countsA, nbA, offsetsA, nt);
        GS_LAUNCH_CHECK(name);
        hipLaunchKernelGGL((compact_write2_k<ActivePredH, ActiveWriterT, false, DsPred, DsWriter>), dim3(nbA + nbB), dim3(kCT), 0, st, nA, pa, wa,
                           (const int *)offsetsA, (int *)nullptr, (const unsigned char *)flags, nbA, nB, pb, wb, (const int *)countsB,
                           frame.count, nbB);
    }
    GS_LAUNCH_CHECK(name);
    hipLaunchKernelGGL(bucket_scatter_k, dim3(std::min(cdiv(cap, 1024), kBucketBlocks)), dim3(1024), 0, st, (const float *)tgt,
                       (const int32_t *)nt, cap, (const int32_t *)row_pix, (const int *)cnt, fill, npix, pix_start, scan_points, scan_orig);
    GS_LAUNCH_CHECK(name);
    return GS_OK;
}
}

extern "C" {

size_t gs_gather_table_rows_ws_bytes(int B) { return align_up(sizeof(int32_t) * (size_t)(B + 1), 256); }

int gs_gather_table_rows(const int64_t *rows, const int32_t *d_n_rows, int64_t max_rows, const float *attr, int B,
                         int Nmax, int C, int cap, float *out, int32_t *counts, void *ws, size_t ws_bytes,
                         gs_stream_t stream) {
    GS_REQUIRE(rows && d_n_rows && attr && out, "gs_gather_table_rows: NULL argument");
    GS_REQUIRE(B > 0 && B <= 256 && Nmax > 0 && C > 0 && cap >= 0 && max_rows >= 0, "gs_gather_table_rows: bad shape (B <= 256)");
    if (!ws || ws_bytes < gs_gather_table_rows_ws_bytes(B)) {
        set_error("gs_gather_table_rows: workspace too small");
        return GS_ERR_WORKSPACE_TOO_SMALL;
    }
    hipStream_t st = (hipStream_t)stream;
    int32_t *starts = (int32_t *)ws;
    hipLaunchKernelGGL(table_starts_k, dim3(cdiv(B + 1, 64)), dim3(64), 0, st, rows, d_n_rows, B, starts);
    GS_LAUNCH_CHECK("gs_gather_table_rows/starts");
    const int nb = max_rows > 0 ? min(cdiv(max_rows, 256), 2048) : 1;
    hipLaunchKernelGGL(gather_table_k, dim3(nb), dim3(256), 0, st, rows, d_n_rows, starts, attr, B, Nmax,
                       C, cap, out, counts);
    GS_LAUNCH_CHECK("gs_gather_table_rows");
    return GS_OK;
}

size_t gs_bucket_by_pixel_ws_bytes(int B, int H, int W, int ds) {
    const size_t npix = (size_t)cdiv(H, ds) * cdiv(W, ds);
    return align_up(sizeof(int32_t) * (size_t)(B + 1), 256) + 2 * align_up((size_t)B * npix * 4, 256);
}

int gs_bucket_by_pixel(const int64_t *rows, const int32_t *d_n_rows, int64_t max_rows, int B, int H, int W, int ds,
                       const float *map_points, int Nmax, int cap, float *scan_points, int32_t *scan_orig,
                       int32_t *pix_start, int32_t *tgt_pix, void *ws, size_t ws_bytes, gs_stream_t stream) {
    GS_REQUIRE(rows && d_n_rows && map_points && scan_points && scan_orig && pix_start, "gs_bucket_by_pixel: NULL argument");
    GS_REQUIRE(B > 0 && B <= 256 && H > 0 && W > 0 && ds > 0 && Nmax > 0 && cap > 0 && max_rows >= 0, "gs_bucket_by_pixel: bad shape");
    if (!ws || ws_bytes < gs_bucket_by_pixel_ws_bytes(B, H, W, ds)) {
        set_error("gs_bucket_by_pixel: workspace too small");
        return GS_ERR_WORKSPACE_TOO_SMALL;
    }
    hipStream_t st = (hipStream_t)stream;
    const int Wd = cdiv(W, ds), npix = cdiv(H, ds) * Wd;
    char *p = (char *)ws;
    int32_t *starts = (int32_t *)p; p += align_up(sizeof(int32_t) * (size_t)(B + 1), 256);
    const size_t seg = align_up((size_t)B * npix * 4, 256);
    int *cnt = (int *)p, *fill = (int *)(p + seg);
    const int64_t nbins = (int64_t)B * npix;
    hipLaunchKernelGGL(tgt_init_k, dim3(min(cdiv(nbins, 256), 1024)), dim3(256), 0, st, cnt, fill, nbins, rows, d_n_rows, B, starts);
    const int nb = max_rows > 0 ? min(cdiv(max_rows, 256), 1024) : 1;
    hipLaunchKernelGGL(pix_count_k, dim3(nb), dim3(256), 0, st, rows, d_n_rows, starts, Wd, npix, ds, cnt);
    hipLaunchKernelGGL(pix_scan_k, dim3(B), dim3(1024), 0, st, cnt, npix, pix_start);
    hipLaunchKernelGGL(pix_scatter_k, dim3(nb), dim3(256), 0, st, rows, d_n_rows, starts, Wd, npix, ds, pix_start, fill, map_points,
                       Nmax, cap, scan_points, scan_orig, tgt_pix);
    GS_LAUNCH_CHECK("gs_bucket_by_pixel");
    return GS_OK;
}

size_t gs_build_icp_target_ws_bytes(int B, int H, int W, int ds) { return gs_bucket_by_pixel_ws_bytes(B, H, W, ds); }

int gs_build_icp_target(const int64_t *rows, const int32_t *d_n_rows, int64_t max_rows, int B, int H, int W, int ds,
                        const float *map_points, const float *map_normals, int Nmax, int cap, float *tgt, float *tgt_normals,
                        int32_t *counts, float *scan_points, int32_t *scan_orig, int32_t *pix_start, int32_t *tgt_index,
                        int32_t *tgt_pix, void *ws, size_t ws_bytes, gs_stream_t stream) {
    GS_REQUIRE(rows && d_n_rows && map_points && map_normals && tgt && tgt_normals && counts && scan_points && scan_orig && pix_start,
               "gs_build_icp_target: NULL argument");
    GS_REQUIRE(B > 0 && B <= 256 && H > 0 && W > 0 && ds > 0 && Nmax > 0 && cap > 0 && max_rows >= 0, "gs_build_icp_target: bad shape");
    if (!ws || ws_bytes < gs_build_icp_target_ws_bytes(B, H, W, ds)) {
        set_error("gs_build_icp_target: workspace too small");
        return GS_ERR_WORKSPACE_TOO_SMALL;
    }
    hipStream_t st = (hipStream_t)stream;
    const int Wd = cdiv(W, ds), npix = cdiv(H, ds) * Wd;
    char *p = (char *)ws;
    int32_t *starts = (int32_t *)p; p += align_up(sizeof(int32_t) * (size_t)(B + 1), 256);
    const size_t seg = align_up((size_t)B * npix * 4, 256);
    int *cnt = (int *)p, *fill = (int *)(p + seg);
    const int64_t nbins = (int64_t)B * npix;
    hipLaunchKernelGGL(tgt_init_k, dim3(min(cdiv(nbins, 256), 1024)), dim3(256), 0, st, cnt, fill, nbins, rows, d_n_rows, B, starts);
    const int nb = max_rows > 0 ? min(cdiv(max_rows, 256), 1024) : 1;
    hipLaunchKernelGGL(tgt_gather_count_k, dim3(nb), dim3(256), 0, st, rows, d_n_rows, starts, map_points, map_normals, B, Nmax,
                       cap, tgt, tgt_normals, counts, Wd, npix, ds, cnt, tgt_index);
    hipLaunchKernelGGL(pix_scan_k, dim3(B), dim3(1024), 0, st, cnt, npix, pix_start);
    hipLaunchKernelGGL(pix_scatter_k, dim3(nb), dim3(256), 0, st, rows, d_n_rows, starts, Wd, npix, ds, pix_start, fill, map_points,
                       Nmax, cap, scan_points, scan_orig, tgt_pix);
    GS_LAUNCH_CHECK("gs_build_icp_target");
    return GS_OK;
}

int gs_table_ds_mask(const int64_t *rows, int64_t n_rows, int ds, uint8_t *mask, gs_stream_t stream) {
    GS_REQUIRE(rows && mask && n_rows >= 0 && ds > 0, "gs_table_ds_mask: bad arguments");
    if (n_rows == 0) return GS_OK;
    hipLaunchKernelGGL(table_ds_mask_k, dim3(min(cdiv(n_rows, 256), 2048)), dim3(256), 0, (hipStream_t)stream, rows,
                       n_rows, ds, mask);
    GS_LAUNCH_CHECK("gs_table_ds_mask");
    return GS_OK;
}

}
```

### gradslam_amd/csrc/slam.hip

```cpp
#include <algorithm>
#include <chrono>
#include <mutex>
#include <stdlib.h>
#include <vector>

#include "gs_common.hpp"
#include "gs_drivers.hpp"
#include "gs_icp.hpp"

namespace gs {

struct GraphKey {
    void *ws;
    int B, capS, capT, numiters, use_grad;
    float damp, thresh, lmax, Bp, B2, nu;
    int icp_cfg;
    int H, W, ds;
    bool operator==(const GraphKey &o) const {
        return H == o.H && W == o.W && ds == o.ds && ws == o.ws && B == o.B && capS == o.capS && capT == o.capT && numiters == o.numiters && use_grad == o.use_grad &&
               damp == o.damp && thresh == o.thresh && lmax == o.lmax && Bp == o.Bp && B2 == o.B2 && nu == o.nu &&
               icp_cfg == o.icp_cfg;
    }
};
struct GraphEntry {
    GraphKey key;
    int device;
    hipGraphExec_t exec;
    unsigned long long last_use;
};
static std::mutex g_graph_mu;
static std::vector<GraphEntry> g_graphs;
static std::vector<GraphKey> g_seen_once;
static unsigned long long g_graph_clock = 0;
static int g_graph_mode = -1;
constexpr double kSlowLaunchUs = 8.0;
static int g_auto_samples = 0;
static double g_auto_min_us = 1e30;
static int g_captures = 0, g_replays = 0;
static bool graphs_allowed() {
    static const bool env_off = getenv("GS_NO_GRAPH") != nullptr, env_on = getenv("GS_GRAPH") != nullptr;
    if (profiling_enabled()) return false;
    if (g_graph_mode >= 0) return g_graph_mode != 0;
    if (env_off) return false;
    if (env_on) return true;
    return g_auto_samples >= 4 && g_auto_min_us > kSlowLaunchUs;
}

template <class Enqueue>
static int graph_replay(const GraphKey &key, hipStream_t st, Enqueue &&enqueue, bool *launched) {
    std::lock_guard<std::mutex> lock(g_graph_mu);
    int device = 0;
    (void)hipGetDevice(&device);
    GraphEntry *hit = nullptr;
    for (auto &e : g_graphs)
        if (e.device == device && e.key == key) hit = &e;
    bool seen = false;
    if (!hit) {
        for (auto &k : g_seen_once) seen = seen || (k == key);
        if (!seen) {
            if (g_seen_once.size() >= 16) g_seen_once.erase(g_seen_once.begin());
            g_seen_once.push_back(key);
        }
    }
    if (!hit && seen) {
        hipStream_t cs = nullptr;
        hipGraph_t graph = nullptr;
        hipGraphExec_t exec = nullptr;
        bool ok = hipStreamCreateWithFlags(&cs, hipStreamNonBlocking) == hipSuccess;
        ok = ok && hipStreamBeginCapture(cs, hipStreamCaptureModeThreadLocal) == hipSuccess;
        if (ok) {
            const int r = enqueue(cs);
            const hipError_t e = hipStreamEndCapture(cs, &graph);
            ok = (r == GS_OK) && e == hipSuccess && graph != nullptr;
        }
        ok = ok && hipGraphInstantiate(&exec, graph, nullptr, nullptr, 0) == hipSuccess;
        if (graph) (void)hipGraphDestroy(graph);
        if (cs) (void)hipStreamDestroy(cs);
        if (ok) {
            if (g_graphs.size() >= 8) {
                size_t v = 0;
                for (size_t i = 1; i < g_graphs.size(); ++i)
                    if (g_graphs[i].last_use < g_graphs[v].last_use) v = i;
                (void)hipGraphExecDestroy(g_graphs[v].exec);
                g_graphs.erase(g_graphs.begin() + v);
            }
            g_graphs.push_back(GraphEntry{key, device, exec, 0});
            hit = &g_graphs.back();
            ++g_captures;
        } else {
            (void)hipGetLastError();
        }
    }
    if (hit) {
        hit->last_use = ++g_graph_clock;
        ++g_replays;
        GS_HIP(hipGraphLaunch(hit->exec, st), "gs_slam_localize/graph");
        *launched = true;
    }
    return GS_OK;
}

template <class Enqueue>
static int eager_timed(int launches, Enqueue &&enqueue) {
    const auto t0 = std::chrono::steady_clock::now();
    const int rc = enqueue();
    if (rc) return rc;
    const double us = std::chrono::duration<double, std::micro>(std::chrono::steady_clock::now() - t0).count();
    std::lock_guard<std::mutex> lock(g_graph_mu);
    if (g_auto_samples < 64) {
        ++g_auto_samples;
        g_auto_min_us = std::min(g_auto_min_us, us / launches);
    }
    return GS_OK;
}

__global__ void compose_k(const float *__restrict__ T, const float *__restrict__ P, int B, float *__restrict__ out) {
    const int b = blockIdx.x * blockDim.x + threadIdx.x;
    if (b >= B) return;
    compose44(T + 16 * b, P + 16 * b, out + 16 * b);
}

__global__ void eye4_k(float *__restrict__ T, int B) {
    const int i = blockIdx.x * blockDim.x + threadIdx.x;
    if (i < 16 * B) T[i] = ((i % 16) % 5 == 0) ? 1.0f : 0.0f;
}

struct LocWs {
    float *src;
    int32_t *src_pix;
    float *scan;
    int32_t *scan_orig;
    int32_t *pix_start;
    int32_t *ns;
    int64_t *rows;
    int32_t *nrows;
    float *tgt, *tnrm;
    int32_t *nt;
    float *T;
    float *eye;
    float *cam;
    void *sub;
    size_t sub_bytes;
};

static inline int target_cap(int Nmax) {
    int c = 1024;
    while (c < Nmax && c < (1 << 30)) c <<= 1;
    return c;
}

static size_t loc_layout(int B, int H, int W, int ds, int Nmax, void *ws, LocWs *out) {
    const int capS = cdiv(H, ds) * cdiv(W, ds), capT = target_cap(Nmax);
    Carve c{(char *)ws};
    LocWs scratch, &w = out ? *out : scratch;
    w.src = c.take<float>((size_t)B * capS * 12); w.ns = c.take<int32_t>((size_t)B * 4);
    w.src_pix = c.take<int32_t>((size_t)B * capS * 4); w.scan = c.take<float>((size_t)B * capT * 12);
    w.scan_orig = c.take<int32_t>((size_t)B * capT * 4); w.pix_start = c.take<int32_t>((size_t)B * (capS + 1) * 4);
    w.rows = c.take<int64_t>((size_t)B * capT * 32); w.nrows = c.take<int32_t>(4);
    w.tgt = c.take<float>((size_t)B * capT * 12); w.tnrm = c.take<float>((size_t)B * capT * 12); w.nt = c.take<int32_t>((size_t)B * 4);
    w.T = c.take<float>((size_t)B * 64); w.eye = c.take<float>((size_t)B * 64); w.cam = c.take<float>((size_t)B * 128);
    w.sub_bytes = std::max({gs_downsample_frame_ws_bytes(H, W, ds), gs_project_active_ws_bytes(B, Nmax), gs_gather_table_rows_ws_bytes(B),
                            gs_bucket_by_pixel_ws_bytes(B, H, W, ds), gs_icp_ws_bytes(capS, capT), project_target1_ws_bytes(H, W, ds, Nmax)});
    w.sub = c.take(w.sub_bytes);
    return c.off;
}

static int g_fused_setup = getenv("GS_FUSED_SETUP") ? atoi(getenv("GS_FUSED_SETUP")) : 1;
static inline bool fused_front(int B, int H, int W, int ds) {
    return g_fused_setup != 0 && B == 1 && (int64_t)cdiv(H, ds) * cdiv(W, ds) <= kBucketPixMax;
}

static int enqueue_front(const float *depth, const float *gvertex, const float *intrinsics, const float *prev_poses, int B, int H, int W,
                         int ds, const float *map_points, const float *map_normals, const int32_t *map_counts, int Nmax, const LocWs &w,
                         float *src, int32_t *src_pix, int32_t *ns, int32_t *nt, int32_t *tgt_index, bool compute_maps, float *vertex,
                         float *normal, float *gvertex_out, float *gnormal, float *cam_out, hipStream_t st) {
    const int capS = cdiv(H, ds) * cdiv(W, ds), capT = target_cap(Nmax);
    const DsJob frame{depth, gvertex, src, src_pix, ns};
    int rc;
    if (fused_front(B, H, W, ds))
        return project_front1(compute_maps ? depth : nullptr, map_points, map_counts, Nmax, prev_poses, intrinsics, H, W, ds, map_normals,
                              capT, vertex, normal, gvertex_out, gnormal, cam_out, (int32_t *)w.rows, w.tgt, w.tnrm, nt, tgt_index, w.scan,
                              w.scan_orig, w.pix_start, frame, w.sub, w.sub_bytes, st);
    if (compute_maps &&
        (rc = vertex_normal_maps_cam(depth, intrinsics, prev_poses, B, H, W, vertex, normal, gvertex_out, gnormal, cam_out, st))) return rc;
    if (B == 1)
        return project_target1(map_points, map_counts, Nmax, prev_poses, intrinsics, H, W, ds, map_normals, capT, w.rows, w.nrows, w.tgt,
                               w.tnrm, nt, w.scan, w.scan_orig, w.pix_start, tgt_index, nullptr, w.sub, w.sub_bytes, st, &frame);
    if ((rc = gs_downsample_frame(depth, gvertex, nullptr, nullptr, B, H, W, ds, capS, src, nullptr, nullptr, src_pix, ns, w.sub,
                                  w.sub_bytes, (gs_stream_t)st))) return rc;
    if ((rc = gs_project_active(map_points, map_counts, B, Nmax, prev_poses, intrinsics, H, W, ds, w.rows, w.nrows, w.sub, w.sub_bytes,
                                (gs_stream_t)st))) return rc;
    return gs_build_icp_target(w.rows, w.nrows, (int64_t)B * Nmax, B, H, W, ds, map_points, map_normals, Nmax, capT, w.tgt, w.tnrm, nt,
                               w.scan, w.scan_orig, w.pix_start, tgt_index, nullptr, w.sub, w.sub_bytes, (gs_stream_t)st);
}

static inline gs_icp_hints loc_hints(const LocWs &w, const int32_t *src_pix, int b, int H, int W, int ds, int capS, int capT,
                                     const float *pose, const float *intrinsics) {
    return gs_icp_hints{w.scan + (size_t)b * capT * 3, w.scan_orig + (size_t)b * capT, src_pix + (size_t)b * capS,
                        w.pix_start + (size_t)b * (capS + 1), nullptr, cdiv(W, ds), cdiv(H, ds), pose, intrinsics, ds};
}

struct FuseWs {
    float *gV, *gN, *alpha;
    void *state;
    int32_t *ctr;
    int32_t *appended;
    int *totals;
    void *sub;
    size_t sub_bytes;
};
constexpr size_t kCompactTotalBytes = 256;
static inline size_t compact_total_ws_bytes(int H, int W) { return gs_compact_ws_bytes((int64_t)H * W) + kCompactTotalBytes; }

constexpr int kCtrWords = 64;
static size_t fuse_layout(int B, int H, int W, int Nmax, void *ws, FuseWs *out) {
    const size_t npix = (size_t)B * H * W;
    Carve c{(char *)ws};
    FuseWs scratch, &w = out ? *out : scratch;
    w.gV = c.take<float>(npix * 12); w.gN = c.take<float>(npix * 12); w.alpha = c.take<float>(npix * 4);
    w.state = c.take(fusion_corr_state_bytes(B, H, W, Nmax));
    w.ctr = c.take<int32_t>((size_t)(kCtrWords + 2 * 64) * 4);
    w.appended = w.ctr + kCtrWords; w.totals = (int *)(w.ctr + kCtrWords + 64);
    w.sub_bytes = compact_total_ws_bytes(H, W);
    w.sub = c.take(w.sub_bytes);
    return c.off;
}

struct FuseBwdWs {
    float *V, *N, *gV, *gN, *alpha, *g_alpha;
    void *cws;
};
static size_t fuse_bwd_layout(int B, int H, int W, void *ws, FuseBwdWs *out) {
    const size_t npix = (size_t)B * H * W;
    Carve c{(char *)ws};
    FuseBwdWs scratch, &w = out ? *out : scratch;
    w.V = c.take<float>(npix * 12); w.N = c.take<float>(npix * 12); w.gV = c.take<float>(npix * 12); w.gN = c.take<float>(npix * 12);
    w.alpha = c.take<float>(npix * 4); w.g_alpha = c.take<float>(npix * 4);
    w.cws = c.take(compact_total_ws_bytes(H, W));
    c.take(256);
    return c.off;
}

struct AggWs {
    float *gV, *gN;
    int32_t *overflow, *appended;
    size_t counter_bytes;
    void *cws;
};
static size_t agg_layout(int B, int H, int W, void *ws, AggWs *out) {
    const size_t npix = (size_t)B * H * W;
    Carve c{(char *)ws};
    AggWs scratch, &w = out ? *out : scratch;
    w.gV = c.take<float>(npix * 12); w.gN = c.take<float>(npix * 12);
    const size_t counters = c.off;
    w.overflow = c.take<int32_t>(4); w.appended = c.take<int32_t>((size_t)B * 4);
    w.counter_bytes = c.off - counters;
    w.cws = c.take(compact_total_ws_bytes(H, W));
    return c.off;
}

__global__ void fuse_stats_k(const int32_t *__restrict__ nrows, const int32_t *__restrict__ ucnt, const int32_t *__restrict__ overflow,
                             const float *__restrict__ max_dot, const int32_t *__restrict__ appended, int B,
                             int32_t *__restrict__ stats) {
    if (threadIdx.x == 0) {
        stats[0] = *nrows; stats[1] = *ucnt; stats[2] = *overflow; stats[3] = __float_as_int(*max_dot);
    }
    if ((int)threadIdx.x < B) stats[4 + threadIdx.x] = appended[threadIdx.x];
}

struct LocTape {
    float *src;
    int32_t *src_pix;
    int32_t *ns, *nt;
    int32_t *tgt_index;
    float *T;
    char *icp;
    size_t icp_bytes;
};
static size_t loc_tape_layout(int B, int H, int W, int ds, int Nmax, int numiters, int grad_lm, void *tape, LocTape *out) {
    const int capS = cdiv(H, ds) * cdiv(W, ds), capT = target_cap(Nmax);
    Carve c{(char *)tape};
    LocTape scratch, &t = out ? *out : scratch;
    t.src = c.take<float>((size_t)B * capS * 12); t.src_pix = c.take<int32_t>((size_t)B * capS * 4);
    t.ns = c.take<int32_t>((size_t)B * 4); t.nt = c.take<int32_t>((size_t)B * 4);
    t.tgt_index = c.take<int32_t>((size_t)B * capT * 4); t.T = c.take<float>((size_t)B * 64);
    t.icp_bytes = align_up(gs_icp_tape_bytes(capS, numiters, grad_lm), 256);
    t.icp = c.take<char>((size_t)B * t.icp_bytes);
    return c.off;
}

struct LocBwdWs {
    float *tgt, *tnrm, *g_tgt, *g_nrm;
    float *g_src;
    float *g_T, *g_init, *eye;
    void *sub;
    size_t sub_bytes;
};
static size_t loc_bwd_layout(bool det, int B, int H, int W, int ds, int Nmax, int numiters, int grad_lm, void *ws, LocBwdWs *out) {
    const int capS = cdiv(H, ds) * cdiv(W, ds), capT = target_cap(Nmax);
    Carve c{(char *)ws};
    LocBwdWs scratch, &w = out ? *out : scratch;
    w.tgt = c.take<float>((size_t)capT * 12); w.tnrm = c.take<float>((size_t)capT * 12);
    w.g_tgt = c.take<float>((size_t)capT * 12); w.g_nrm = c.take<float>((size_t)capT * 12);
    w.g_src = c.take<float>((size_t)capS * 12);
    w.g_T = c.take<float>((size_t)B * 64); w.g_init = c.take<float>((size_t)B * 64); w.eye = c.take<float>((size_t)B * 64);
    w.sub_bytes = det ? gs_icp_backward_det_ws_bytes(capS, capT, numiters, grad_lm) : gs_icp_backward_ws_bytes(capS);
    w.sub = c.take(w.sub_bytes);
    return c.off;
}

__global__ void compose_bwd_k(const float *__restrict__ T, const float *__restrict__ P, const float *__restrict__ gO, int B,
                              float *__restrict__ gT, float *__restrict__ gP) {
    const int b = blockIdx.x * blockDim.x + threadIdx.x;
    if (b >= B) return;
    const float *a = T + 16 * b, *p = P + 16 * b, *g = gO + 16 * b;
    float *ga = gT + 16 * b, *gp = gP + 16 * b;
    for (int i = 0; i < 3; ++i) {
        for (int k = 0; k < 3; ++k) ga[4 * i + k] = ((g[4 * i] * p[4 * k] + g[4 * i + 1] * p[4 * k + 1]) + g[4 * i + 2] * p[4 * k + 2]) + g[4 * i + 3] * p[4 * k + 3];
        ga[4 * i + 3] = g[4 * i + 3];
    }
    for (int k = 0; k < 3; ++k)
        for (int j = 0; j < 4; ++j) gp[4 * k + j] = (a[k] * g[j] + a[4 + k] * g[4 + j]) + a[8 + k] * g[8 + j];
    for (int j = 0; j < 4; ++j) { ga[12 + j] = 0.0f; gp[12 + j] = 0.0f; }
}

__global__ void regather_k(const int32_t *__restrict__ tgt_index, const int32_t *__restrict__ nt, int capT,
                           const float *__restrict__ map_points, const float *__restrict__ map_normals, int Nmax,
                           float *__restrict__ tgt, float *__restrict__ tnrm) {
    const int b = blockIdx.y, n = min(nt[b], capT);
    for (int k = blockIdx.x * blockDim.x + threadIdx.x; k < n; k += gridDim.x * blockDim.x) {
        const int64_t srcI = (int64_t)b * Nmax + tgt_index[(int64_t)b * capT + k], dst = (int64_t)b * capT + k;
        st3(tgt, dst, ld3(map_points, srcI));
        st3(tnrm, dst, ld3(map_normals, srcI));
    }
}

__global__ void scatter_grads_k(const float *__restrict__ g_src, const int32_t *__restrict__ src_pix, const int32_t *__restrict__ ns,
                                int capS, int Wd, int ds, int H, int W, float *__restrict__ g_gvertex ,
                                const float *__restrict__ g_tgt, const float *__restrict__ g_nrm,
                                const int32_t *__restrict__ tgt_index, const int32_t *__restrict__ nt, int capT,
                                float *__restrict__ g_map_points, float *__restrict__ g_map_normals , int accumulate) {
    const int n_s = min(*ns, capS), n_t = min(*nt, capT);
    const int stride = gridDim.x * blockDim.x;
    for (int i = blockIdx.x * blockDim.x + threadIdx.x; i < n_s; i += stride) {
        const int pix = src_pix[i];
        const int64_t at = (int64_t)(pix / Wd) * ds * W + (int64_t)(pix % Wd) * ds;
        st3(g_gvertex, at, ld3(g_src, i));
    }
    for (int k = blockIdx.x * blockDim.x + threadIdx.x; k < n_t; k += stride) {
        const int64_t at = tgt_index[k];
        f3 gp = g_map_points ? ld3(g_tgt, k) : f3{0, 0, 0}, gq = g_map_normals ? ld3(g_nrm, k) : f3{0, 0, 0};
        if (accumulate) {
            if (g_map_points) { const f3 o = ld3(g_map_points, at); gp = f3{o.x + gp.x, o.y + gp.y, o.z + gp.z}; }
            if (g_map_normals) { const f3 o = ld3(g_map_normals, at); gq = f3{o.x + gq.x, o.y + gq.y, o.z + gq.z}; }
        }
        if (g_map_points) st3(g_map_points, at, gp);
        if (g_map_normals) st3(g_map_normals, at, gq);
    }
}

}

using namespace gs;

extern "C" {

void gs_set_graph_mode(int mode) { g_graph_mode = mode; }

void gs_set_fused_setup(int on) { g_fused_setup = on; }

int gs_graph_stats(double *out4) {
    GS_REQUIRE(out4, "gs_graph_stats: NULL argument");
    std::lock_guard<std::mutex> lock(g_graph_mu);
    out4[0] = g_auto_samples; out4[1] = g_auto_min_us; out4[2] = g_captures; out4[3] = g_replays;
    return GS_OK;
}

int gs_compose_poses(const float *T, const float *P, int B, float *out, gs_stream_t stream) {
    GS_REQUIRE(T && P && out && B > 0, "gs_compose_poses: bad arguments");
    hipLaunchKernelGGL(compose_k, dim3(cdiv(B, 64)), dim3(64), 0, (hipStream_t)stream, T, P, B, out);
    GS_LAUNCH_CHECK("gs_compose_poses");
    return GS_OK;
}

size_t gs_slam_localize_ws_bytes(int B, int H, int W, int ds, int Nmax) {
    if (B <= 0 || H <= 0 || W <= 0 || ds <= 0 || Nmax <= 0) return 0;
    return loc_layout(B, H, W, ds, Nmax, nullptr, nullptr);
}

int gs_slam_localize(const float *depth, const float *intrinsics, const float *prev_poses, int B, int H, int W, int ds,
                     const float *map_points, const float *map_normals, const int32_t *map_counts, int Nmax,
                     int use_grad_lm, int numiters, float damp, float dist_thresh, float lambda_max, float Bp, float B2,
                     float nu, float *vertex, float *normal, float *gvertex, float *gnormal, float *out_poses, void *ws,
                     size_t ws_bytes, gs_stream_t stream) {
    GS_REQUIRE(depth && intrinsics && prev_poses && map_points && map_normals && map_counts && gvertex && out_poses,
               "gs_slam_localize: NULL argument (gvertex is required, the other maps are optional)");
    GS_REQUIRE(B > 0 && H >= 2 && W >= 2 && ds > 0 && Nmax > 0 && numiters >= 0, "gs_slam_localize: bad shape");
    if (!ws || ws_bytes < gs_slam_localize_ws_bytes(B, H, W, ds, Nmax)) {
        set_error("gs_slam_localize: workspace too small (%zu < %zu)", ws_bytes, gs_slam_localize_ws_bytes(B, H, W, ds, Nmax));
        return GS_ERR_WORKSPACE_TOO_SMALL;
    }
    hipStream_t st = (hipStream_t)stream;
    LocWs w;
    loc_layout(B, H, W, ds, Nmax, ws, &w);
    const int capS = cdiv(H, ds) * cdiv(W, ds), capT = target_cap(Nmax);
    int rc;
    if ((rc = enqueue_front(depth, gvertex, intrinsics, prev_poses, B, H, W, ds, map_points, map_normals, map_counts, Nmax, w, w.src,
                            w.src_pix, w.ns, w.nt, nullptr, true, vertex, normal, gvertex, gnormal, w.cam, st))) return rc;
    auto enqueue_loops = [&](hipStream_t s, bool fold_compose) -> int {
        for (int b = 0; b < B; ++b) {
            const gs_icp_hints hints = loc_hints(w, w.src_pix, b, H, W, ds, capS, capT, w.cam + 32 * b, w.cam + 32 * b + 16);
            const int r = icp_localize_run(use_grad_lm, w.src + (size_t)b * capS * 3, w.ns + b, capS, w.tgt + (size_t)b * capT * 3,
                                           w.tnrm + (size_t)b * capT * 3, w.nt + b, capT, numiters, damp, dist_thresh, lambda_max, Bp,
                                           B2, nu, &hints, w.T + 16 * b, w.sub, w.sub_bytes, s, nullptr, 0,
                                           fold_compose ? prev_poses + 16 * b : nullptr, fold_compose ? out_poses + 16 * b : nullptr);
            if (r) return r;
        }
        return GS_OK;
    };
    bool launched = false;
    if (graphs_allowed() && numiters > 0) {
        const GraphKey key{ws, B, capS, capT, numiters, use_grad_lm, damp, dist_thresh, lambda_max, Bp, B2, nu,
                           icp_config_stamp(), H, W, ds};
        if ((rc = graph_replay(key, st, [&](hipStream_t cs) { return enqueue_loops(cs, false); }, &launched))) return rc;
    }
    if (!launched) {
        if (numiters > 0)
            return eager_timed(B * ((use_grad_lm ? 2 * numiters : numiters + 1) + 2), [&] { return enqueue_loops(st, true); });
        if ((rc = enqueue_loops(st, false))) return rc;
    }
    return gs_compose_poses(w.T, prev_poses, B, out_poses, stream);
}

size_t gs_pointfusion_update_ws_bytes(int B, int H, int W, int Nmax) {
    if (B <= 0 || H <= 0 || W <= 0 || Nmax <= 0) return 0;
    return fuse_layout(B, H, W, Nmax, nullptr, nullptr);
}

static int pointfusion_update_impl(const float *depth, const float *rgb, const float *intrinsics, const float *poses, int B, int H, int W,
                                   float *map_points, float *map_normals, float *map_colors, float *map_ccounts, int32_t *map_counts,
                                   int Nmax, float dist_th, float dot_th, float sigma, int32_t *stats, void *ws, size_t ws_bytes,
                                   gs_stream_t stream, void *tape, const char *name) {
    GS_REQUIRE(depth && rgb && intrinsics && poses && map_points && map_normals && map_colors && map_ccounts && map_counts,
               "%s: NULL argument", name);
    GS_REQUIRE(B > 0 && B <= 60 && H >= 2 && W >= 2 && Nmax > 0, "%s: bad shape", name);
    if (!ws || ws_bytes < gs_pointfusion_update_ws_bytes(B, H, W, Nmax)) {
        set_error("%s: workspace too small (%zu < %zu)", name, ws_bytes, gs_pointfusion_update_ws_bytes(B, H, W, Nmax));
        return GS_ERR_WORKSPACE_TOO_SMALL;
    }
    hipStream_t st = (hipStream_t)stream;
    FuseWs w;
    fuse_layout(B, H, W, Nmax, ws, &w);
    int rc;
    unsigned long long *pix_key; unsigned int *pix_n;
    fusion_corr_init_ptrs(w.state, B, H, W, Nmax, &pix_key, &pix_n);
    if ((rc = vertex_normal_maps_fusion(depth, intrinsics, poses, B, H, W, w.gV, w.gN, w.alpha, sigma, 1e-7f, pix_key, pix_n, w.ctr,
                                        kCtrWords + 2 * 64, st))) return rc;
    if ((rc = fusion_correspond(w.state, map_points, map_normals, map_ccounts, map_counts, B, Nmax, poses, intrinsics, H, W, w.gV, w.gN,
                                dist_th, dot_th, w.ctr, st))) return rc;
    if (tape && (rc = fusion_tape_record(w.state, tape, B, H, W, Nmax, map_counts, map_points, map_normals, map_colors, map_ccounts, st)))
        return rc;
    if ((rc = fusion_merge_corr(w.state, w.ctr, w.gV, w.gN, rgb, w.alpha, B, H, W, Nmax, map_counts, map_points, map_normals, map_colors,
                                map_ccounts, st))) return rc;
    const int64_t HW = (int64_t)H * W;
    for (int b = 0; b < B; ++b) {
        const float *src[4] = {w.gV + b * HW * 3, w.gN + b * HW * 3, rgb + b * HW * 3, w.alpha + b * HW};
        float *dst[4] = {map_points + (size_t)b * Nmax * 3, map_normals + (size_t)b * Nmax * 3, map_colors + (size_t)b * Nmax * 3,
                         map_ccounts + (size_t)b * Nmax};
        const int widths[4] = {3, 3, 3, 1};
        if ((rc = fusion_append_corr(w.state, B, H, W, Nmax, b, depth, src, widths, dst, map_counts + b, Nmax, w.totals + b, w.sub, st)))
            return rc;
    }
    if ((rc = fusion_finish(w.state, B, H, W, Nmax, w.ctr, map_counts, w.totals, Nmax, w.appended, stats, st))) return rc;
    if (tape && (rc = fusion_tape_appended(tape, B, H, W, w.appended, st))) return rc;
    return GS_OK;
}

int gs_pointfusion_update(const float *depth, const float *rgb, const float *intrinsics, const float *poses, int B, int H, int W,
                          float *map_points, float *map_normals, float *map_colors, float *map_ccounts, int32_t *map_counts,
                          int Nmax, float dist_th, float dot_th, float sigma, int32_t *stats, void *ws, size_t ws_bytes,
                          gs_stream_t stream) {
    return pointfusion_update_impl(depth, rgb, intrinsics, poses, B, H, W, map_points, map_normals, map_colors, map_ccounts, map_counts,
                                   Nmax, dist_th, dot_th, sigma, stats, ws, ws_bytes, stream, nullptr, "gs_pointfusion_update");
}

size_t gs_pointfusion_update_tape_bytes(int B, int H, int W) {
    if (B <= 0 || H <= 0 || W <= 0) return 0;
    return fusion_tape_bytes(B, H, W);
}

int gs_pointfusion_update_taped(const float *depth, const float *rgb, const float *intrinsics, const float *poses, int B, int H, int W,
                                float *map_points, float *map_normals, float *map_colors, float *map_ccounts, int32_t *map_counts,
                                int Nmax, float dist_th, float dot_th, float sigma, int32_t *stats, void *tape, size_t tape_bytes,
                                void *ws, size_t ws_bytes, gs_stream_t stream) {
    GS_REQUIRE(tape && tape_bytes >= gs_pointfusion_update_tape_bytes(B, H, W), "gs_pointfusion_update_taped: tape missing or too small");
    return pointfusion_update_impl(depth, rgb, intrinsics, poses, B, H, W, map_points, map_normals, map_colors, map_ccounts, map_counts,
                                   Nmax, dist_th, dot_th, sigma, stats, ws, ws_bytes, stream, tape, "gs_pointfusion_update_taped");
}

size_t gs_pointfusion_update_backward_ws_bytes(int B, int H, int W) {
    if (B <= 0 || H <= 0 || W <= 0) return 0;
    return fuse_bwd_layout(B, H, W, nullptr, nullptr);
}

int gs_pointfusion_update_backward(const float *depth, const float *rgb, const float *intrinsics, const float *poses, int B, int H,
                                   int W, float *map_points, float *map_normals, float *map_colors, float *map_ccounts,
                                   int32_t *map_counts, int Nmax, float sigma, const void *tape, size_t tape_bytes, float *G_points,
                                   float *G_normals, float *G_colors, float *G_ccounts, float *g_vertex, float *g_gvertex,
                                   float *g_gnormal, float *g_rgb, void *ws, size_t ws_bytes, gs_stream_t stream) {
    const char *name = "gs_pointfusion_update_backward";
    GS_REQUIRE(depth && rgb && intrinsics && poses && map_points && map_normals && map_colors && map_ccounts && map_counts && tape &&
                   G_points && G_normals && G_colors && G_ccounts && g_vertex && g_gvertex && g_gnormal && g_rgb, "%s: NULL argument", name);
    GS_REQUIRE(B > 0 && B <= 60 && H >= 2 && W >= 2 && Nmax > 0, "%s: bad shape", name);
    GS_REQUIRE(tape_bytes >= gs_pointfusion_update_tape_bytes(B, H, W), "%s: tape too small", name);
    if (!ws || ws_bytes < gs_pointfusion_update_backward_ws_bytes(B, H, W)) {
        set_error("%s: workspace too small (%zu < %zu)", name, ws_bytes, gs_pointfusion_update_backward_ws_bytes(B, H, W));
        return GS_ERR_WORKSPACE_TOO_SMALL;
    }
    hipStream_t st = (hipStream_t)stream;
    const size_t npix = (size_t)B * H * W;
    FuseBwdWs w;
    fuse_bwd_layout(B, H, W, ws, &w);
    int rc;
    if ((rc = gs_vertex_normal_maps(depth, intrinsics, poses, B, 1, H, W, w.V, w.N, w.gV, w.gN, stream))) return rc;
    if ((rc = gs_get_alpha(w.V, (int64_t)npix, sigma, 1e-7f, w.alpha, stream))) return rc;
    if ((rc = fusion_update_reverse(tape, B, H, W, Nmax, depth, w.gV, w.gN, rgb, w.alpha, map_points, map_normals, map_colors, map_ccounts,
                                    map_counts, G_points, G_normals, G_colors, G_ccounts, g_gvertex, g_gnormal, g_rgb, w.g_alpha, w.cws,
                                    st))) return rc;
    GS_HIP(hipMemsetAsync(g_vertex, 0, npix * 12, st), name);
    return gs_get_alpha_backward(w.V, (int64_t)npix, sigma, 1e-7f, w.g_alpha, g_vertex, stream);
}

size_t gs_aggregate_update_ws_bytes(int B, int H, int W) {
    if (B <= 0 || H <= 0 || W <= 0) return 0;
    return agg_layout(B, H, W, nullptr, nullptr);
}

int gs_aggregate_update(const float *depth, const float *rgb, const float *intrinsics, const float *poses, int B, int H, int W,
                        float *map_points, float *map_normals, float *map_colors, int32_t *map_counts, int Nmax, int32_t *stats,
                        void *ws, size_t ws_bytes, gs_stream_t stream) {
    const char *name = "gs_aggregate_update";
    GS_REQUIRE(depth && rgb && intrinsics && poses && map_points && map_normals && map_colors && map_counts, "%s: NULL argument", name);
    GS_REQUIRE(B > 0 && B <= 60 && H >= 2 && W >= 2 && Nmax > 0, "%s: bad shape", name);
    if (!ws || ws_bytes < gs_aggregate_update_ws_bytes(B, H, W)) {
        set_error("%s: workspace too small (%zu < %zu)", name, ws_bytes, gs_aggregate_update_ws_bytes(B, H, W));
        return GS_ERR_WORKSPACE_TOO_SMALL;
    }
    hipStream_t st = (hipStream_t)stream;
    AggWs w;
    agg_layout(B, H, W, ws, &w);
    GS_HIP(hipMemsetAsync(w.overflow, 0, w.counter_bytes, st), name);
    int rc;
    if ((rc = gs_vertex_normal_maps(depth, intrinsics, poses, B, 1, H, W, nullptr, nullptr, w.gV, w.gN, stream))) return rc;
    const int64_t HW = (int64_t)H * W;
    for (int b = 0; b < B; ++b) {
        const float *src[3] = {w.gV + b * HW * 3, w.gN + b * HW * 3, rgb + b * HW * 3};
        float *dst[3] = {map_points + (size_t)b * Nmax * 3, map_normals + (size_t)b * Nmax * 3, map_colors + (size_t)b * Nmax * 3};
        const int widths[3] = {3, 3, 3};
        if ((rc = append_valid_pixels(3, depth + b * HW, HW, src, widths, dst, map_counts + b, Nmax, w.appended + b, w.overflow, w.cws,
                                      st))) return rc;
    }
    if (stats) {
        hipLaunchKernelGGL(fuse_stats_k, dim3(1), dim3(64), 0, st, w.overflow, w.overflow, w.overflow, (const float *)w.overflow, w.appended, B,
                           stats);
        GS_LAUNCH_CHECK(name);
    }
    return GS_OK;
}

size_t gs_slam_localize_tape_bytes(int B, int H, int W, int ds, int Nmax, int numiters, int use_grad_lm) {
    if (B <= 0 || H <= 0 || W <= 0 || ds <= 0 || Nmax <= 0 || numiters < 0) return 0;
    return loc_tape_layout(B, H, W, ds, Nmax, numiters, use_grad_lm, nullptr, nullptr);
}

int gs_slam_localize_taped(const float *depth, const float *gvertex, const float *intrinsics, const float *prev_poses, int B, int H,
                           int W, int ds, const float *map_points, const float *map_normals, const int32_t *map_counts, int Nmax,
                           int use_grad_lm, int numiters, float damp, float dist_thresh, float lambda_max, float Bp, float B2,
                           float nu, float *out_poses, void *tape, size_t tape_bytes, void *ws, size_t ws_bytes,
                           gs_stream_t stream) {
    GS_REQUIRE(depth && gvertex && intrinsics && prev_poses && map_points && map_normals && map_counts && out_poses && tape,
               "gs_slam_localize_taped: NULL argument");
    GS_REQUIRE(B > 0 && H >= 2 && W >= 2 && ds > 0 && Nmax > 0 && numiters >= 0, "gs_slam_localize_taped: bad shape");
    if (!ws || ws_bytes < gs_slam_localize_ws_bytes(B, H, W, ds, Nmax)) {
        set_error("gs_slam_localize_taped: workspace too small (%zu < %zu)", ws_bytes, gs_slam_localize_ws_bytes(B, H, W, ds, Nmax));
        return GS_ERR_WORKSPACE_TOO_SMALL;
    }
    GS_REQUIRE(tape_bytes >= gs_slam_localize_tape_bytes(B, H, W, ds, Nmax, numiters, use_grad_lm),
               "gs_slam_localize_taped: tape too small");
    hipStream_t st = (hipStream_t)stream;
    LocWs w;
    loc_layout(B, H, W, ds, Nmax, ws, &w);
    LocTape tp;
    loc_tape_layout(B, H, W, ds, Nmax, numiters, use_grad_lm, tape, &tp);
    const int capS = cdiv(H, ds) * cdiv(W, ds), capT = target_cap(Nmax);
    int rc;
    if ((rc = enqueue_front(depth, gvertex, intrinsics, prev_poses, B, H, W, ds, map_points, map_normals, map_counts, Nmax, w, tp.src,
                            tp.src_pix, tp.ns, tp.nt, tp.tgt_index, false, nullptr, nullptr, nullptr, nullptr, nullptr, st))) return rc;
    for (int b = 0; b < B; ++b) {
        const gs_icp_hints hints = loc_hints(w, tp.src_pix, b, H, W, ds, capS, capT, prev_poses + 16 * b, intrinsics + 16 * b);
        if ((rc = icp_localize_run(use_grad_lm, tp.src + (size_t)b * capS * 3, tp.ns + b, capS, w.tgt + (size_t)b * capT * 3,
                                   w.tnrm + (size_t)b * capT * 3, tp.nt + b, capT, numiters, damp, dist_thresh, lambda_max, Bp, B2, nu,
                                   &hints, tp.T + 16 * b, w.sub, w.sub_bytes, st, tp.icp + (size_t)b * tp.icp_bytes, tp.icp_bytes,
                                   prev_poses + 16 * b, out_poses + 16 * b)))
            return rc;
    }
    if (numiters == 0) return gs_compose_poses(tp.T, prev_poses, B, out_poses, stream);
    return GS_OK;
}

size_t gs_slam_localize_backward_ws_bytes(int B, int H, int W, int ds, int Nmax) {
    if (B <= 0 || H <= 0 || W <= 0 || ds <= 0 || Nmax <= 0) return 0;
    return loc_bwd_layout(false, B, H, W, ds, Nmax, 0, 0, nullptr, nullptr);
}

size_t gs_slam_localize_backward_det_ws_bytes(int B, int H, int W, int ds, int Nmax, int numiters, int grad_lm) {
    if (B <= 0 || H <= 0 || W <= 0 || ds <= 0 || Nmax <= 0) return 0;
    return loc_bwd_layout(true, B, H, W, ds, Nmax, numiters, grad_lm, nullptr, nullptr);
}

static int localize_backward(bool det, const float *prev_poses, int B, int H, int W, int ds, const float *map_points,
                             const float *map_normals, int Nmax, int use_grad_lm, int numiters, float dist_thresh,
                             float lambda_max, float Bp, float B2, float nu, const void *tape, size_t tape_bytes,
                             const float *grad_out_poses, float *grad_gvertex, float *grad_map_points, float *grad_map_normals,
                             float *grad_prev_poses, int accumulate_map_grads, void *ws, size_t ws_bytes, gs_stream_t stream) {
    const char *name = det ? "gs_slam_localize_backward_det" : "gs_slam_localize_backward";
    GS_REQUIRE(prev_poses && map_points && map_normals && tape && grad_out_poses && grad_gvertex && grad_prev_poses,
               "%s: NULL argument", name);
    GS_REQUIRE(B > 0 && H >= 2 && W >= 2 && ds > 0 && Nmax > 0 && numiters >= 0, "%s: bad shape", name);
    if (!ws || ws_bytes < loc_bwd_layout(det, B, H, W, ds, Nmax, numiters, use_grad_lm, nullptr, nullptr)) {
        set_error("%s: workspace too small", name);
        return GS_ERR_WORKSPACE_TOO_SMALL;
    }
    GS_REQUIRE(tape_bytes >= gs_slam_localize_tape_bytes(B, H, W, ds, Nmax, numiters, use_grad_lm), "%s: tape too small", name);
    hipStream_t st = (hipStream_t)stream;
    LocTape tp;
    loc_tape_layout(B, H, W, ds, Nmax, numiters, use_grad_lm, (void *)tape, &tp);
    const int capS = cdiv(H, ds) * cdiv(W, ds), capT = target_cap(Nmax);
    LocBwdWs w;
    loc_bwd_layout(det, B, H, W, ds, Nmax, numiters, use_grad_lm, ws, &w);
    auto icp_backward = det ? gs_icp_point_to_plane_backward_det : gs_icp_point_to_plane_backward;

    GS_HIP(hipMemsetAsync(grad_gvertex, 0, (size_t)B * H * W * 12, st), name);
    if (grad_map_points && !accumulate_map_grads) GS_HIP(hipMemsetAsync(grad_map_points, 0, (size_t)B * Nmax * 12, st), name);
    if (grad_map_normals && !accumulate_map_grads) GS_HIP(hipMemsetAsync(grad_map_normals, 0, (size_t)B * Nmax * 12, st), name);
    hipLaunchKernelGGL(eye4_k, dim3(cdiv(16 * B, 64)), dim3(64), 0, st, w.eye, B);
    hipLaunchKernelGGL(compose_bwd_k, dim3(cdiv(B, 64)), dim3(64), 0, st, tp.T, prev_poses, grad_out_poses, B, w.g_T, grad_prev_poses);
    GS_LAUNCH_CHECK(name);
    const int gb = min(cdiv(capS, 256), 512);
    for (int b = 0; b < B; ++b) {
        hipLaunchKernelGGL(regather_k, dim3(gb, 1), dim3(256), 0, st, tp.tgt_index + (size_t)b * capT, tp.nt + b, capT,
                           map_points + (size_t)b * Nmax * 3, map_normals + (size_t)b * Nmax * 3, Nmax, w.tgt, w.tnrm);
        GS_LAUNCH_CHECK(name);
        int rc;
        if ((rc = icp_backward(tp.src + (size_t)b * capS * 3, tp.ns + b, capS, w.tgt, w.tnrm, tp.nt + b, capT, w.eye + 16 * b, numiters,
                               dist_thresh, use_grad_lm, lambda_max, Bp, B2, nu, tp.icp + (size_t)b * tp.icp_bytes, tp.icp_bytes,
                               w.g_T + 16 * b, w.g_src, grad_map_points ? w.g_tgt : nullptr, grad_map_normals ? w.g_nrm : nullptr,
                               w.g_init + 16 * b, w.sub, w.sub_bytes, stream)))
            return rc;
        hipLaunchKernelGGL(scatter_grads_k, dim3(gb), dim3(256), 0, st, w.g_src, tp.src_pix + (size_t)b * capS, tp.ns + b, capS,
                           cdiv(W, ds), ds, H, W, grad_gvertex + (size_t)b * H * W * 3, w.g_tgt, w.g_nrm, tp.tgt_index + (size_t)b * capT,
                           tp.nt + b, capT, grad_map_points ? grad_map_points + (size_t)b * Nmax * 3 : nullptr,
                           grad_map_normals ? grad_map_normals + (size_t)b * Nmax * 3 : nullptr, accumulate_map_grads);
        GS_LAUNCH_CHECK(name);
    }
    return GS_OK;
}

int gs_slam_localize_backward(const float *prev_poses, int B, int H, int W, int ds, const float *map_points,
                              const float *map_normals, int Nmax, int use_grad_lm, int numiters, float dist_thresh,
                              float lambda_max, float Bp, float B2, float nu, const void *tape, size_t tape_bytes,
                              const float *grad_out_poses, float *grad_gvertex, float *grad_map_points, float *grad_map_normals,
                              float *grad_prev_poses, int accumulate_map_grads, void *ws, size_t ws_bytes, gs_stream_t stream) {
    return localize_backward(false, prev_poses, B, H, W, ds, map_points, map_normals, Nmax, use_grad_lm, numiters, dist_thresh, lambda_max,
                             Bp, B2, nu, tape, tape_bytes, grad_out_poses, grad_gvertex, grad_map_points, grad_map_normals, grad_prev_poses,
                             accumulate_map_grads, ws, ws_bytes, stream);
}

int gs_slam_localize_backward_det(const float *prev_poses, int B, int H, int W, int ds, const float *map_points,
                                  const float *map_normals, int Nmax, int use_grad_lm, int numiters, float dist_thresh,
                                  float lambda_max, float Bp, float B2, float nu, const void *tape, size_t tape_bytes,
                                  const float *grad_out_poses, float *grad_gvertex, float *grad_map_points, float *grad_map_normals,
                                  float *grad_prev_poses, int accumulate_map_grads, void *ws, size_t ws_bytes, gs_stream_t stream) {
    return localize_backward(true, prev_poses, B, H, W, ds, map_points, map_normals, Nmax, use_grad_lm, numiters, dist_thresh, lambda_max,
                             Bp, B2, nu, tape, tape_bytes, grad_out_poses, grad_gvertex, grad_map_points, grad_map_normals, grad_prev_poses,
                             accumulate_map_grads, ws, ws_bytes, stream);
}

}
```

### include/gradslam_hip.h

```cpp
#ifndef GRADSLAM_HIP_H
#define GRADSLAM_HIP_H

#include <stddef.h>
#include <stdint.h>

#ifdef __cplusplus
extern "C" {
#endif

#define GS_ABI_VERSION 3
#define GS_OK 0
#define GS_ERR_INVALID_ARG (-1)
#define GS_ERR_WORKSPACE_TOO_SMALL (-2)
#define GS_ERR_UNSUPPORTED (-3)

typedef void *gs_stream_t;

int gs_abi_version(void);
const char *gs_last_error(void);

int gs_vertex_normal_maps(const float *depth, const float *intrinsics ,
                          const float *poses , int B, int L, int H, int W,
                          float *vertex, float *normal, float *gvertex, float *gnormal,
                          gs_stream_t stream);
// ... 52 lines not shown
                         const float *attr, int B, int Nmax, int C, int cap, float *out,
                         int32_t *counts, void *ws, size_t ws_bytes, gs_stream_t stream);

size_t gs_bucket_by_pixel_ws_bytes(int B, int H, int W, int ds);
int gs_bucket_by_pixel(const int64_t *rows, const int32_t *d_n_rows, int64_t max_rows, int B, int H,
                       int W, int ds, const float *map_points, int Nmax, int cap, float *scan_points,
                       int32_t *scan_orig, int32_t *pix_start, int32_t *tgt_pix, void *ws, size_t ws_bytes,
                       gs_stream_t stream);

size_t gs_build_icp_target_ws_bytes(int B, int H, int W, int ds);
int gs_build_icp_target(const int64_t *rows, const int32_t *d_n_rows, int64_t max_rows, int B, int H,
                        int W, int ds, const float *map_points, const float *map_normals, int Nmax,
                        int cap, float *tgt, float *tgt_normals, int32_t *counts, float *scan_points,
                        int32_t *scan_orig, int32_t *pix_start, int32_t *tgt_index, int32_t *tgt_pix,
                        void *ws, size_t ws_bytes, gs_stream_t stream);

int gs_table_ds_mask(const int64_t *rows, int64_t n_rows, int ds, uint8_t *mask, gs_stream_t stream);

size_t gs_knn1_ws_bytes(int max_nt);
int gs_knn1(const float *src, const int32_t *d_ns, int max_ns, const float *tgt,
            const int32_t *d_nt, int max_nt, uint64_t *best, void *ws, size_t ws_bytes,
            gs_stream_t stream);
int gs_knn1_bruteforce(const float *src, const int32_t *d_ns, int max_ns, const float *tgt,
                       const int32_t *d_nt, int max_nt, uint64_t *best, gs_stream_t stream);
int gs_knn1_unpack(const uint64_t *best, const int32_t *d_ns, int max_ns, float *dist2,
                   int64_t *idx, gs_stream_t stream);

size_t gs_icp_linearize_ws_bytes(int max_ns);
int gs_icp_linearize(const float *src, const int32_t *d_ns, int max_ns, const float *tgt,
                     const float *tgt_normals, const uint64_t *best, float dist_thresh,
                     float *out44, void *ws, size_t ws_bytes, gs_stream_t stream);

int gs_icp_rows(const float *src, const int32_t *d_ns, int max_ns, const float *tgt,
                const float *tgt_normals, const uint64_t *best, float dist_thresh, float *A,
                float *b, uint8_t *keep, gs_stream_t stream);

int gs_icp_linearize_backward(const float *src, const int32_t *d_ns, int max_ns, const float *tgt,
                              const float *tgt_normals, const uint64_t *best, float dist_thresh,
                              const float *g_out43, float *g_src, float *g_tgt, float *g_normals,
                              gs_stream_t stream);
size_t gs_icp_linearize_backward_det_ws_bytes(int max_ns, int max_nt);
int gs_icp_linearize_backward_det(const float *src, const int32_t *d_ns, int max_ns, const float *tgt,
                                  const float *tgt_normals, const int32_t *d_nt, int max_nt, const uint64_t *best,
                                  float dist_thresh, const float *g_out43, float *g_src, float *g_tgt,
                                  float *g_normals, void *ws, size_t ws_bytes, gs_stream_t stream);

int gs_transform_points(const float *pts, const int32_t *d_n, int max_n, const float *T,
                        float *out, gs_stream_t stream);

typedef struct gs_icp_hints {
    const float *scan_points;
    const int32_t *scan_orig;
    const int32_t *src_pix;
    const int32_t *pix_start;
    const int32_t *tgt_pix;
    int32_t grid_w, grid_h;
    const float *cam_pose, *cam_K;
    int32_t ds;
} gs_icp_hints;

size_t gs_icp_ws_bytes(int max_ns, int max_nt);
int gs_icp_point_to_plane(const float *src, const int32_t *d_ns, int max_ns, const float *tgt,
                          const float *tgt_normals, const int32_t *d_nt, int max_nt,
                          const float *init_T, int numiters, float damp, float dist_thresh,
                          const gs_icp_hints *hints, float *out_T, uint64_t *best_last,
                          float *trace, void *ws, size_t ws_bytes, gs_stream_t stream);

int gs_icp_point_to_plane_grad(const float *src, const int32_t *d_ns, int max_ns, const float *tgt,
                               const float *tgt_normals, const int32_t *d_nt, int max_nt,
                               const float *init_T, int numiters, float damp, float dist_thresh,
                               float lambda_max, float B, float B2, float nu,
                               const gs_icp_hints *hints, float *out_T, uint64_t *best_last,
                               float *trace, void *ws, size_t ws_bytes, gs_stream_t stream);

size_t gs_icp_tape_bytes(int max_ns, int numiters, int grad_lm);
int gs_icp_point_to_plane_taped(const float *src, const int32_t *d_ns, int max_ns, const float *tgt,
                                const float *tgt_normals, const int32_t *d_nt, int max_nt,
                                const float *init_T, int numiters, float damp, float dist_thresh,
                                int grad_lm, float lambda_max, float B, float B2, float nu,
                                const gs_icp_hints *hints, float *out_T, uint64_t *best_last,
                                void *tape, size_t tape_bytes, void *ws, size_t ws_bytes,
                                gs_stream_t stream);
size_t gs_icp_backward_ws_bytes(int max_ns);
int gs_icp_point_to_plane_backward(const float *src, const int32_t *d_ns, int max_ns, const float *tgt,
                                   const float *tgt_normals, const int32_t *d_nt, int max_nt, const float *init_T,
                                   int numiters, float dist_thresh, int grad_lm, float lambda_max,
                                   float B, float B2, float nu, const void *tape, size_t tape_bytes,
                                   const float *grad_T, float *grad_src, float *grad_tgt,
                                   float *grad_normals, float *grad_init_T, void *ws, size_t ws_bytes,
                                   gs_stream_t stream);
size_t gs_icp_backward_det_ws_bytes(int max_ns, int max_nt, int numiters, int grad_lm);
int gs_icp_point_to_plane_backward_det(const float *src, const int32_t *d_ns, int max_ns, const float *tgt,
                                       const float *tgt_normals, const int32_t *d_nt, int max_nt, const float *init_T,
                                       int numiters, float dist_thresh, int grad_lm, float lambda_max,
                                       float B, float B2, float nu, const void *tape, size_t tape_bytes,
                                       const float *grad_T, float *grad_src, float *grad_tgt,
                                       float *grad_normals, float *grad_init_T, void *ws, size_t ws_bytes,
                                       gs_stream_t stream);

size_t gs_pointfusion_update_ws_bytes(int B, int H, int W, int Nmax);
int gs_pointfusion_update(const float *depth, const float *rgb, const float *intrinsics, const float *poses,
                          int B, int H, int W, float *map_points, float *map_normals, float *map_colors,
                          float *map_ccounts, int32_t *map_counts, int Nmax, float dist_th, float dot_th,
                          float sigma, int32_t *stats, void *ws, size_t ws_bytes, gs_stream_t stream);

size_t gs_pointfusion_update_tape_bytes(int B, int H, int W);
int gs_pointfusion_update_taped(const float *depth, const float *rgb, const float *intrinsics, const float *poses,
                                int B, int H, int W, float *map_points, float *map_normals, float *map_colors,
                                float *map_ccounts, int32_t *map_counts, int Nmax, float dist_th, float dot_th,
                                float sigma, int32_t *stats, void *tape, size_t tape_bytes, void *ws,
                                size_t ws_bytes, gs_stream_t stream);
size_t gs_pointfusion_update_backward_ws_bytes(int B, int H, int W);
int gs_pointfusion_update_backward(const float *depth, const float *rgb, const float *intrinsics, const float *poses,
                                   int B, int H, int W, float *map_points, float *map_normals, float *map_colors,
                                   float *map_ccounts, int32_t *map_counts, int Nmax, float sigma, const void *tape,
                                   size_t tape_bytes, float *G_points, float *G_normals, float *G_colors,
                                   float *G_ccounts, float *g_vertex, float *g_gvertex, float *g_gnormal,
                                   float *g_rgb, void *ws, size_t ws_bytes, gs_stream_t stream);

size_t gs_aggregate_update_ws_bytes(int B, int H, int W);
int gs_aggregate_update(const float *depth, const float *rgb, const float *intrinsics, const float *poses, int B,
                        int H, int W, float *map_points, float *map_normals, float *map_colors,
                        int32_t *map_counts, int Nmax, int32_t *stats, void *ws, size_t ws_bytes,
                        gs_stream_t stream);

size_t gs_slam_localize_tape_bytes(int B, int H, int W, int ds, int Nmax, int numiters, int use_grad_lm);
int gs_slam_localize_taped(const float *depth, const float *gvertex, const float *intrinsics,
                           const float *prev_poses, int B, int H, int W, int ds, const float *map_points,
                           const float *map_normals, const int32_t *map_counts, int Nmax, int use_grad_lm,
                           int numiters, float damp, float dist_thresh, float lambda_max, float Bp,
                           float B2, float nu, float *out_poses, void *tape, size_t tape_bytes, void *ws,
                           size_t ws_bytes, gs_stream_t stream);
size_t gs_slam_localize_backward_ws_bytes(int B, int H, int W, int ds, int Nmax);
int gs_slam_localize_backward(const float *prev_poses, int B, int H, int W, int ds, const float *map_points,
                              const float *map_normals, int Nmax, int use_grad_lm, int numiters,
                              float dist_thresh, float lambda_max, float Bp, float B2, float nu,
                              const void *tape, size_t tape_bytes, const float *grad_out_poses,
                              float *grad_gvertex, float *grad_map_points, float *grad_map_normals,
                              float *grad_prev_poses, int accumulate_map_grads ,
                              void *ws, size_t ws_bytes, gs_stream_t stream);
size_t gs_slam_localize_backward_det_ws_bytes(int B, int H, int W, int ds, int Nmax, int numiters, int use_grad_lm);
int gs_slam_localize_backward_det(const float *prev_poses, int B, int H, int W, int ds, const float *map_points,
                                  const float *map_normals, int Nmax, int use_grad_lm, int numiters,
                                  float dist_thresh, float lambda_max, float Bp, float B2, float nu,
                                  const void *tape, size_t tape_bytes, const float *grad_out_poses,
                                  float *grad_gvertex, float *grad_map_points, float *grad_map_normals,
                                  float *grad_prev_poses, int accumulate_map_grads, void *ws, size_t ws_bytes,
                                  gs_stream_t stream);

void gs_set_graph_mode(int mode);
int gs_graph_stats(double *out4);
int gs_compose_poses(const float *T, const float *P, int B, float *out, gs_stream_t stream);
size_t gs_slam_localize_ws_bytes(int B, int H, int W, int ds, int Nmax);
int gs_slam_localize(const float *depth, const float *intrinsics, const float *prev_poses, int B,
                     int H, int W, int ds, const float *map_points, const float *map_normals,
                     const int32_t *map_counts, int Nmax, int use_grad_lm, int numiters, float damp,
                     float dist_thresh, float lambda_max, float Bp, float B2, float nu,
                     float *vertex, float *normal, float *gvertex, float *gnormal, float *out_poses,
                     void *ws, size_t ws_bytes, gs_stream_t stream);

void gs_profile_enable(int on);
int gs_profile_read(int tag, long *launches, double *total_ms);

void gs_set_grid_search(int on);

void gs_set_fused_setup(int on);

void gs_set_tile_points(int n);
int gs_set_loop_waves(int n);
int gs_icp_launch_geometry(int max_ns, int have_hints, int *blocks, int *tile_points_dense, int *partial_rows);
int gs_loop_counts(unsigned int *out4, int reset);

int gs_fusion_similar(const int64_t *rows, const int32_t *d_n_rows, int64_t max_rows,
                      const float *gvertex, const float *gnormal, int H, int W,
                      const float *map_points, const float *map_normals, int Nmax, float dist_th,
                      float dot_th, uint8_t *keep, float *max_dot, gs_stream_t stream);

size_t gs_fusion_unique_ws_bytes(int B, int H, int W);
int gs_fusion_unique(const int64_t *rows, const uint8_t *keep, const int32_t *d_n_rows,
                     int64_t max_rows, const float *gvertex, int B, int H, int W,
                     const float *map_points, const float *map_ccounts, int Nmax,
                     int64_t *out_rows, int32_t *out_count, void *ws, size_t ws_bytes,
                     gs_stream_t stream);

size_t gs_fusion_merge_ws_bytes(int B, int Nmax);
int gs_fusion_merge(const int64_t *rows, const int32_t *d_n_rows, int64_t max_rows,
                    const float *gvertex, const float *gnormal, const float *rgb,
                    const float *alpha, int B, int H, int W, int Nmax, const int32_t *counts,
                    const float *in_points, const float *in_normals, const float *in_colors,
                    const float *in_ccounts, float *out_points, float *out_normals,
                    float *out_colors, float *out_ccounts, void *ws, size_t ws_bytes,
                    gs_stream_t stream);
int gs_fusion_merge_backward(const int64_t *rows, const int32_t *d_n_rows, int64_t max_rows,
                             const float *gvertex, const float *gnormal, const float *rgb,
                             const float *alpha, int B, int H, int W, int Nmax,
                             const int32_t *counts, const float *in_points,
                             const float *in_normals, const float *in_colors,
                             const float *in_ccounts, const float *g_out_points,
                             const float *g_out_normals, const float *g_out_colors,
                             const float *g_out_ccounts, float *g_in_points, float *g_in_normals,
                             float *g_in_colors, float *g_in_ccounts, float *g_gvertex,
                             float *g_gnormal, float *g_rgb, float *g_alpha, void *ws,
                             size_t ws_bytes, gs_stream_t stream);

size_t gs_fusion_merge_inplace_ws_bytes(int B, int Nmax);
int gs_fusion_merge_inplace(const int64_t *rows, const int32_t *d_n_rows, int64_t max_rows,
                            const float *gvertex, const float *gnormal, const float *rgb,
                            const float *alpha, int B, int H, int W, int Nmax, const int32_t *counts,
                            float *points, float *normals, float *colors, float *ccounts, void *ws,
                            size_t ws_bytes, gs_stream_t stream);

int gs_fusion_new_mask(const float *depth, const int64_t *rows, const int32_t *d_n_rows,
                       int64_t max_rows, int B, int H, int W, uint8_t *mask, gs_stream_t stream);

size_t gs_render_map_ws_bytes(int B, int H, int W);
int gs_render_map(const float *points, const float *normals, const float *colors, const int32_t *counts,
                  int B, int Nmax, const float *poses, const float *intrinsics, int H, int W,
                  int32_t *out_index, float *out_depth, float *out_points, float *out_normals,
                  float *out_colors, void *ws, size_t ws_bytes, gs_stream_t stream);

size_t gs_render_map_backward_ws_bytes(int B, int H, int W);
int gs_render_map_backward(const float *points, const int32_t *counts, int B, int Nmax, const float *poses,
                           int H, int W, const int32_t *index, const float *g_depth,
                           const float *g_out_points, const float *g_out_normals,
                           const float *g_out_colors, float *g_points, float *g_normals, float *g_colors,
                           float *g_poses, void *ws, size_t ws_bytes, gs_stream_t stream);

size_t gs_chamfer_ws_bytes(int B, int Na_max, int Nb_max);
int gs_chamfer(const float *a, const int32_t *a_counts, int Na_max, const float *b, const int32_t *b_counts,
               int Nb_max, int B, float tau2, int reorder, double *stats, uint64_t *keys_ab, uint64_t *keys_ba,
               void *ws, size_t ws_bytes, gs_stream_t stream);

size_t gs_chamfer_backward_ws_bytes(int B, int Na_max, int Nb_max);
int gs_chamfer_backward(const float *a, const int32_t *a_counts, int Na_max, const float *b,
                        const int32_t *b_counts, int Nb_max, int B, const uint64_t *keys_ab,
                        const uint64_t *keys_ba, const float *g2, const float *g1, float *g_a, float *g_b,
                        void *ws, size_t ws_bytes, gs_stream_t stream);
size_t gs_chamfer_backward_det_ws_bytes(int B, int Na_max, int Nb_max);
int gs_chamfer_backward_det(const float *a, const int32_t *a_counts, int Na_max, const float *b,
                            const int32_t *b_counts, int Nb_max, int B, const uint64_t *keys_ab,
                            const uint64_t *keys_ba, const float *g2, const float *g1, float *g_a, float *g_b,
                            void *ws, size_t ws_bytes, gs_stream_t stream);

#ifdef __cplusplus
}
#endif
#endif
```

Baseline: 5559 frames/s.

## Fuse ICP prepare and super-box construction into front-end scatter kernel

Adds a front_boxes kernel that runs the per-pixel prefix scan, scatters target rows into scan order, computes the ICP bounding boxes and super-boxes, and uses spare blocks to perform the ICP loop preparation (state init, partial zeroing, LoopConst publish). This removes the separate icp_prepare_k launch and a pass over the scattered target points, cutting one kernel from the per-frame sequence. The ICP workspace is split out of the shared sub-workspace so the prep can be computed before the front end, and the graph key now includes the mode. Each range block rescans all keys for every super-box it owns, which may cost more than it saves for large targets.

```diff
diff --git a/gradslam_amd/_native.py b/gradslam_amd/_native.py
--- a/gradslam_amd/_native.py
+++ b/gradslam_amd/_native.py
@@ -97,6 +97,8 @@
                                c_f, c_p, c_p, c_p, c_p, c_p, c_p, c_sz, c_p]),
     "gs_set_grid_search": (None, [c_i]),
     "gs_set_fused_setup": (None, [c_i]),
+    "gs_set_front_boxes": (c_i, [c_i]),
+    "gs_slam_localize_ws_offsets": (c_i, [c_i, c_i, c_i, c_i, c_i, ctypes.POINTER(c_sz)]),
     "gs_set_tile_points": (None, [c_i]),
     "gs_set_loop_waves": (c_i, [c_i]),
     "gs_icp_launch_geometry": (c_i, [c_i, c_i, ctypes.POINTER(c_i), ctypes.POINTER(c_i), ctypes.POINTER(c_i)]),
diff --git a/gradslam_amd/csrc/gs_drivers.hpp b/gradslam_amd/csrc/gs_drivers.hpp
--- a/gradslam_amd/csrc/gs_drivers.hpp
+++ b/gradslam_amd/csrc/gs_drivers.hpp
@@ -1,6 +1,7 @@
 #pragma once
 
 #include "gs_common.hpp"
+#include "gs_icp.hpp"
 #include "gs_project.hpp"
 
 namespace gs {
@@ -20,7 +21,11 @@
 int project_front1(const float *depth, const float *points, const int32_t *counts, int Nmax, const float *poses, const float *intrinsics,
                    int H, int W, int ds, const float *map_normals, int cap, float *vertex, float *normal, float *gvertex, float *gnormal,
                    float *cam_out, int32_t *row_pix, float *tgt, float *tnrm, int32_t *nt, int32_t *tgt_index, float *scan_points,
-                   int32_t *scan_orig, int32_t *pix_start, const DsJob &frame, void *ws, size_t ws_bytes, hipStream_t st);
+                   int32_t *scan_orig, int32_t *pix_start, const DsJob &frame, void *ws, size_t ws_bytes, hipStream_t st,
+                   const LoopPrep *prep = nullptr);
+
+int front_boxes_launch(const float *tgt, const int32_t *d_nt, int cap, const int32_t *row_key, const int *cnt, int npix,
+                       int32_t *pix_start, float *scan_points, int32_t *scan_orig, const LoopPrep &prep, hipStream_t st);
 
 size_t fusion_corr_state_bytes(int B, int H, int W, int Nmax);
 void fusion_corr_init_ptrs(void *state, int B, int H, int W, int Nmax, unsigned long long **pix_key, unsigned int **pix_n);
diff --git a/gradslam_amd/csrc/gs_icp.hpp b/gradslam_amd/csrc/gs_icp.hpp
--- a/gradslam_amd/csrc/gs_icp.hpp
+++ b/gradslam_amd/csrc/gs_icp.hpp
@@ -5,10 +5,28 @@
 namespace gs {
 
 bool profiling_enabled();
+
+constexpr size_t kLoopConstBytes = 320;
+struct LoopPrep {
+    alignas(8) unsigned char lc[kLoopConstBytes];
+    void *state;
+    void *lc_out;
+    float *boxes, *sboxes;
+    float *part0, *part1;
+    int rows_written, rows_read;
+    float damp;
+};
+
 int icp_localize_run(int grad_lm, const float *src, const int32_t *d_ns, int max_ns, const float *tgt, const float *nrm,
                      const int32_t *d_nt, int max_nt, int numiters, float damp, float thresh, float lambda_max, float Bp,
                      float B2, float nu, const gs_icp_hints *hints, float *out_T, void *ws, size_t ws_bytes, hipStream_t st,
-                     void *tape, size_t tape_bytes, const float *compose_right, float *compose_out);
+                     void *tape, size_t tape_bytes, const float *compose_right, float *compose_out,
+                     const LoopPrep *prepared = nullptr);
 int icp_config_stamp();
 
+int icp_localize_prep(int grad_lm, const float *src, const int32_t *d_ns, int max_ns, const float *tgt, const float *nrm,
+                      const int32_t *d_nt, int max_nt, float damp, float thresh, float lambda_max, float Bp, float B2, float nu,
+                      const gs_icp_hints *hints, float *out_T, void *ws, size_t ws_bytes, LoopPrep *out);
+void icp_ws_offsets(int max_ns, int max_nt, size_t *out12);
+
 }
diff --git a/gradslam_amd/csrc/gs_icp_loop.hpp b/gradslam_amd/csrc/gs_icp_loop.hpp
--- a/gradslam_amd/csrc/gs_icp_loop.hpp
+++ b/gradslam_amd/csrc/gs_icp_loop.hpp
@@ -484,17 +484,13 @@
     }
 }
 
-__global__ __launch_bounds__(SUPER * CHUNK) void icp_prepare_k(IcpState *S, const float *__restrict__ init_T, float damp,
-                                                              const float *__restrict__ tgt, const int32_t *__restrict__ d_nt,
-                                                              float *__restrict__ boxes, float *__restrict__ sboxes,
-                                                              LoopConst lc, LoopConst *__restrict__ lc_out, float *__restrict__ part0,
-                                                              float *__restrict__ part1, int rows_written, int rows_read) {
-    static_assert(SUPER * CHUNK == 1024, "one block per super-box");
-    for (int q = rows_written * NACC + blockIdx.x * blockDim.x + threadIdx.x; q < rows_read * NACC; q += gridDim.x * blockDim.x) {
+__device__ __forceinline__ void loop_prepare_body(IcpState *S, const float *__restrict__ init_T, float damp, const LoopConst &lc,
+                                                  LoopConst *__restrict__ lc_out, float *__restrict__ part0, float *__restrict__ part1,
+                                                  int rows_written, int rows_read, int vb, int nvb) {
+    for (int q = rows_written * NACC + vb * blockDim.x + threadIdx.x; q < rows_read * NACC; q += nvb * blockDim.x) {
         part0[q] = 0.0f; part1[q] = 0.0f;
     }
-    __shared__ float wb[16][6];
-    if (blockIdx.x == 0 && threadIdx.x < sizeof(LoopConst) / 4) {
+    if (vb == 0 && threadIdx.x < sizeof(LoopConst) / 4) {
         int v = reinterpret_cast<const int *>(&lc)[threadIdx.x];
         if (threadIdx.x == offsetof(LoopConst, ns) / 4) v = *lc.d_ns;
         if (threadIdx.x == offsetof(LoopConst, nt) / 4) v = *lc.d_nt;
@@ -508,10 +504,10 @@
     if (lc.cells) {
         const int n = *lc.d_ns;
         int32_t *pix = lc.cells + 2 * (size_t)lc.cells_stride;
-        for (int i = blockIdx.x * blockDim.x + threadIdx.x; i < lc.cells_stride; i += gridDim.x * blockDim.x)
+        for (int i = vb * blockDim.x + threadIdx.x; i < lc.cells_stride; i += nvb * blockDim.x)
             pix[i] = (i < n && lc.hints.src_pix) ? lc.hints.src_pix[i] : 0;
     }
-    if (blockIdx.x == 0) {
+    if (vb == 0) {
         __syncthreads();
         if (threadIdx.x == 0 && lc.hints.cam_pose && lc.hints.cam_K && lc.hints.ds > 0) {
             const float *T = lc.hints.cam_pose, *K = lc.hints.cam_K;
@@ -525,7 +521,7 @@
             lc_out->cam_ok = pinhole ? 1 : 0;
         }
     }
-    if (threadIdx.x == 0 && blockIdx.x == 0) {
+    if (threadIdx.x == 0 && vb == 0) {
         for (int i = 0; i < 16; ++i) {
             const float v = init_T ? init_T[i] : ((i % 5 == 0) ? 1.0f : 0.0f);
             S->T[i] = v; S->dT[i] = v;
@@ -537,14 +533,14 @@
         S->b_cur = 1; S->b_first = 0;
         S->it = 0;
     }
-    const int nt = *d_nt;
-    const int j = blockIdx.x * (SUPER * CHUNK) + threadIdx.x;
-    if (blockIdx.x * (SUPER * CHUNK) >= nt) return;
+}
+
+__device__ __forceinline__ void super_box_body(const f3 p, int sb, int nt, float *__restrict__ boxes, float *__restrict__ sboxes,
+                                               float (*wb)[6]) {
+    static_assert(SUPER * CHUNK == 1024, "one block per super-box");
+    const int j = sb * (SUPER * CHUNK) + threadIdx.x;
     float lo[3] = {INFINITY, INFINITY, INFINITY}, hi[3] = {-INFINITY, -INFINITY, -INFINITY};
-    if (j < nt) {
-        const f3 p = ld3(tgt, j);
-        lo[0] = hi[0] = p.x; lo[1] = hi[1] = p.y; lo[2] = hi[2] = p.z;
-    }
+    if (j < nt) { lo[0] = hi[0] = p.x; lo[1] = hi[1] = p.y; lo[2] = hi[2] = p.z; }
 #pragma unroll
     for (int a = 0; a < 3; ++a) {
 #pragma unroll
@@ -571,8 +567,23 @@
     if (threadIdx.x < 6) {
         float v = wb[0][threadIdx.x];
         for (int w = 1; w < 16; ++w) v = threadIdx.x < 3 ? fminf(v, wb[w][threadIdx.x]) : fmaxf(v, wb[w][threadIdx.x]);
-        sboxes[6 * (int64_t)blockIdx.x + threadIdx.x] = v;
-    }
+        sboxes[6 * (int64_t)sb + threadIdx.x] = v;
+    }
+}
+
+__global__ __launch_bounds__(SUPER * CHUNK) void icp_prepare_k(IcpState *S, const float *__restrict__ init_T, float damp,
+                                                              const float *__restrict__ tgt, const int32_t *__restrict__ d_nt,
+                                                              float *__restrict__ boxes, float *__restrict__ sboxes,
+                                                              LoopConst lc, LoopConst *__restrict__ lc_out, float *__restrict__ part0,
+                                                              float *__restrict__ part1, int rows_written, int rows_read) {
+    __shared__ float wb[16][6];
+    loop_prepare_body(S, init_T, damp, lc, lc_out, part0, part1, rows_written, rows_read, blockIdx.x, gridDim.x);
+    const int nt = *d_nt;
+    const int j = blockIdx.x * (SUPER * CHUNK) + threadIdx.x;
+    if (blockIdx.x * (SUPER * CHUNK) >= nt) return;
+    f3 p{0.0f, 0.0f, 0.0f};
+    if (j < nt) p = ld3(tgt, j);
+    super_box_body(p, blockIdx.x, nt, boxes, sboxes, wb);
 }
 
 __global__ void copy_best_last_k(const IcpState *__restrict__ S, LoopBufs B, const int32_t *__restrict__ d_ns,
diff --git a/gradslam_amd/csrc/icp.hip b/gradslam_amd/csrc/icp.hip
--- a/gradslam_amd/csrc/icp.hip
+++ b/gradslam_amd/csrc/icp.hip
@@ -1,9 +1,11 @@
 #include <stddef.h>
 #include <stdlib.h>
+#include <string.h>
 #include <algorithm>
 #include <vector>
 
 #include "gs_detfold.hpp"
+#include "gs_drivers.hpp"
 #include "gs_icp.hpp"
 #include "gs_icp_reduce.hpp"
 
@@ -254,7 +256,7 @@
     LoopConst *lc;
     int32_t *cells;
 };
-static inline size_t icp_ws_layout(int max_ns, int max_nt, void *ws, IcpWs *out) {
+static inline size_t icp_ws_layout(int max_ns, int max_nt, void *ws, IcpWs *out, size_t *offs = nullptr) {
     size_t off = 0;
     auto take = [&](size_t bytes) { size_t o = off; off += align_up(bytes, 256); return o; };
     const size_t oS = take(sizeof(IcpState)), oS1 = take(sizeof(IcpState));
@@ -263,6 +265,10 @@
     const size_t oPart = take((size_t)partial_rows_alloc(max_ns) * NACC * 4), oPart1 = take((size_t)partial_rows_alloc(max_ns) * NACC * 4);
     const size_t oBox = take(boxes_bytes(max_nt)), oSBox = take((size_t)cdiv(max_nt > 0 ? max_nt : 1, 1024) * 6 * 4);
     const size_t oLc = take(sizeof(LoopConst)), oCells = take((size_t)max_ns * 12);
+    if (offs) {
+        const size_t o[10] = {oBox, oSBox, oLc, oCells + 2 * (size_t)max_ns * 4, oS, oS1, oP0, oP1 - oP0, oB0, oB1 - oB0};
+        for (int q = 0; q < 10; ++q) offs[q] = o[q];
+    }
     if (ws && out) {
         char *p = (char *)ws;
         out->S[0] = (IcpState *)(p + oS); out->S[1] = (IcpState *)(p + oS1);
@@ -307,11 +313,108 @@
 }
 static inline GradParams lm_grad_params() { return GradParams{0.5f, 1.5f, 1.0f, 1.0f, 0.005f}; }
 
+static_assert(sizeof(LoopConst) <= kLoopConstBytes && sizeof(LoopConst) % 4 == 0, "LoopPrep carries a LoopConst by value");
+static inline LoopConst prep_lc(const LoopPrep &p) {
+    LoopConst lc;
+    memcpy(&lc, p.lc, sizeof(LoopConst));
+    return lc;
+}
+static inline bool loop_grid_search(const gs_icp_hints &hints) {
+    static const bool grid_off = getenv("GS_NO_GRID_SEARCH") != nullptr;
+    return !grid_off && g_grid_mode != 0 && hints.scan_points && hints.scan_orig && hints.src_pix && hints.pix_start &&
+           hints.cam_pose && hints.cam_K && hints.ds > 0 && hints.grid_w > 0 && hints.grid_h > 0;
+}
+static LoopPrep loop_prep(const float *src, const int32_t *d_ns, int max_ns, const float *tgt, const float *nrm, const int32_t *d_nt,
+                          float damp, float thresh, GradParams gp, const gs_icp_hints &hints, float *out_T, float *trace, const IcpWs &w) {
+    static const int cert_off = getenv("GS_CERT_OFF") != nullptr;
+    const int tile_points = loop_tile_points();
+    const int lb = cdiv(max_ns, tile_points);
+    LoopPrep p{};
+    LoopConst &lc = *reinterpret_cast<LoopConst *>(p.lc);
+    lc.user_src = src; lc.tgt = tgt; lc.nrm = nrm; lc.boxes = w.boxes; lc.sboxes = w.sboxes; lc.d_ns = d_ns; lc.d_nt = d_nt;
+    lc.trace = trace; lc.out_T = out_T;
+    lc.hints.scan_points = hints.scan_points; lc.hints.scan_orig = hints.scan_orig; lc.hints.src_pix = hints.src_pix;
+    lc.hints.pix_start = hints.pix_start; lc.hints.tgt_pix = hints.tgt_pix; lc.hints.grid_w = hints.grid_w; lc.hints.grid_h = hints.grid_h;
+    lc.hints.cam_pose = hints.cam_pose; lc.hints.cam_K = hints.cam_K; lc.hints.ds = hints.ds;
+    lc.gp = gp; lc.thresh = thresh; lc.cert_off = cert_off; lc.tile_points = tile_points;
+    lc.grid_variant = loop_grid_search(hints) ? 1 : 0; lc.cells = w.cells; lc.cells_stride = max_ns;
+    p.state = w.S[0]; p.lc_out = w.lc; p.boxes = w.boxes; p.sboxes = w.sboxes; p.part0 = w.partials[0]; p.part1 = w.partials[1];
+    p.rows_written = lb; p.rows_read = std::max(lb, 32 * RP_LOADS); p.damp = damp;
+    return p;
+}
+
+constexpr int kPrepBlocks = 4, kRangeBlocksMax = 256 - kPrepBlocks, kKeyLoads = 20;
+__global__ __launch_bounds__(1024) void front_boxes_k(const float *__restrict__ tgt, const int32_t *__restrict__ d_nt, int cap,
+                                                      const int2 *__restrict__ row_key, const int *__restrict__ cnt, int npix,
+                                                      int32_t *__restrict__ pix_start, float *__restrict__ scan_pts,
+                                                      int32_t *__restrict__ scan_orig, float *__restrict__ boxes,
+                                                      float *__restrict__ sboxes, int nrb, IcpState *S, float damp, LoopConst lc,
+                                                      LoopConst *__restrict__ lc_out, float *__restrict__ part0,
+                                                      float *__restrict__ part1, int rows_written, int rows_read) {
+    __shared__ int starts[kBucketPixMax];
+    __shared__ int sm[1024 / 64 + 1];
+    __shared__ int tile[SUPER * CHUNK];
+    __shared__ float wb[16][6];
+    if ((int)blockIdx.x >= nrb) {
+        loop_prepare_body(S, nullptr, damp, lc, lc_out, part0, part1, rows_written, rows_read, (int)blockIdx.x - nrb, (int)gridDim.x - nrb);
+        return;
+    }
+    const int nt = min(*d_nt, cap);
+    if ((int)blockIdx.x * (SUPER * CHUNK) >= nt && blockIdx.x != 0) return;
+    for (int i = threadIdx.x; i < npix; i += 1024) starts[i] = cnt[i];
+    int2 k[kKeyLoads];
+    auto request = [&](int r0) {
+#pragma unroll
+        for (int u = 0; u < kKeyLoads; ++u) {
+            const int r = r0 + 1024 * u;
+            k[u] = r < nt ? row_key[r] : make_int2(0, 0);
+        }
+    };
+    request(threadIdx.x);
+    __syncthreads();
+    const int per = (npix + 1023) / 1024;
+    const int i0 = min(npix, (int)threadIdx.x * per), i1 = min(npix, i0 + per);
+    int sum = 0;
+    for (int i = i0; i < i1; ++i) sum += starts[i];
+    int total;
+    int run = block_excl_scan<1024>(sum, sm, &total);
+    for (int i = i0; i < i1; ++i) { const int c = starts[i]; starts[i] = run; run += c; }
+    __syncthreads();
+    if (blockIdx.x == 0) {
+        for (int i = threadIdx.x; i < npix; i += 1024) pix_start[i] = starts[i];
+        if (threadIdx.x == 0) pix_start[npix] = total;
+    }
+    for (int sb = blockIdx.x; sb * (SUPER * CHUNK) < nt; sb += nrb) {
+        const int base = sb * (SUPER * CHUNK);
+        for (int r0 = threadIdx.x; r0 < nt; r0 += 1024 * kKeyLoads) {
+            if (r0 != (int)threadIdx.x || sb != (int)blockIdx.x) request(r0);
+#pragma unroll
+            for (int u = 0; u < kKeyLoads; ++u) {
+                const int r = r0 + 1024 * u;
+                if (r < nt) {
+                    const int slot = starts[k[u].x] + k[u].y;
+                    if (slot >= base && slot < base + SUPER * CHUNK) tile[slot - base] = r;
+                }
+            }
+        }
+        __syncthreads();
+        const int j = base + (int)threadIdx.x;
+        f3 p{0.0f, 0.0f, 0.0f};
+        if (j < nt) {
+            const int r = tile[threadIdx.x];
+            p = ld3(tgt, r);
+            st3(scan_pts, j, p);
+            scan_orig[j] = r;
+        }
+        super_box_body(p, sb, nt, boxes, sboxes, wb);
+    }
+}
+
 static int icp_run(bool grad, const float *src, const int32_t *d_ns, int max_ns, const float *tgt, const float *nrm,
                    const int32_t *d_nt, int max_nt, const float *init_T, int numiters, float damp, float thresh,
                    GradParams gp, const gs_icp_hints *hints_in, float *out_T, uint64_t *best_last, float *trace, void *ws,
                    size_t ws_bytes, hipStream_t st, const char *name, void *tape = nullptr, size_t tape_bytes = 0,
-                   const float *compose_right = nullptr, float *compose_out = nullptr) {
+                   const float *compose_right = nullptr, float *compose_out = nullptr, const LoopPrep *prepared = nullptr) {
     gs_icp_hints hints{nullptr, nullptr, nullptr, nullptr, nullptr, 0, 0, nullptr, nullptr, 0};
     if (hints_in) hints = *hints_in;
     GS_REQUIRE(!hints.scan_points || hints.scan_orig, "%s: hints.scan_points needs hints.scan_orig", name);
@@ -347,16 +450,15 @@
     const int lb = (int)kgrid.x;
     const int fb = min(cdiv(max_ns, 256), 256);
 
-    static const int cert_off = getenv("GS_CERT_OFF") != nullptr;
-    static const bool grid_off = getenv("GS_NO_GRID_SEARCH") != nullptr;
-    const bool grid_search = !grid_off && g_grid_mode != 0 && hints.scan_points && hints.scan_orig && hints.src_pix && hints.pix_start &&
-                             hints.cam_pose && hints.cam_K && hints.ds > 0 && hints.grid_w > 0 && hints.grid_h > 0;
-    LoopConst lc{src, tgt, nrm, w.boxes, w.sboxes, d_ns, d_nt, trace, out_T, hints, gp, thresh, 0, 0, cert_off, tile_points,
-                 grid_search ? 1 : 0, CamK{}, 0, w.cells, max_ns};
-    hipLaunchKernelGGL(icp_prepare_k, dim3(cdiv(max_nt, SUPER * CHUNK)), dim3(SUPER * CHUNK), 0, st, w.S[0], init_T, damp,
-                       hints.scan_points ? hints.scan_points : tgt, d_nt, w.boxes, w.sboxes, lc, w.lc, w.partials[0], w.partials[1], lb,
-                       std::max(lb, 32 * RP_LOADS));
-    GS_LAUNCH_CHECK(name);
+    const bool grid_search = loop_grid_search(hints);
+    GS_REQUIRE(!prepared || (prepared->lc_out == (void *)w.lc && !init_T && !trace && numiters > 0), "%s: preparations of another loop", name);
+    if (!prepared) {
+        const LoopPrep p = loop_prep(src, d_ns, max_ns, tgt, nrm, d_nt, damp, thresh, gp, hints, out_T, trace, w);
+        hipLaunchKernelGGL(icp_prepare_k, dim3(cdiv(max_nt, SUPER * CHUNK)), dim3(SUPER * CHUNK), 0, st, (IcpState *)p.state, init_T, p.damp,
+                           hints.scan_points ? hints.scan_points : tgt, d_nt, p.boxes, p.sboxes, prep_lc(p), (LoopConst *)p.lc_out, p.part0,
+                           p.part1, p.rows_written, p.rows_read);
+        GS_LAUNCH_CHECK(name);
+    }
     int cur = 0;
     int pending = -1;
     int pending_slot = -1;
@@ -491,10 +593,45 @@
 int icp_localize_run(int grad_lm, const float *src, const int32_t *d_ns, int max_ns, const float *tgt, const float *nrm,
                      const int32_t *d_nt, int max_nt, int numiters, float damp, float thresh, float lambda_max, float Bp,
                      float B2, float nu, const gs_icp_hints *hints, float *out_T, void *ws, size_t ws_bytes, hipStream_t st,
-                     void *tape, size_t tape_bytes, const float *compose_right, float *compose_out) {
+                     void *tape, size_t tape_bytes, const float *compose_right, float *compose_out, const LoopPrep *prepared) {
     const GradParams gp = grad_lm ? make_grad_params(lambda_max, Bp, B2, nu) : lm_grad_params();
     return icp_run(grad_lm != 0, src, d_ns, max_ns, tgt, nrm, d_nt, max_nt, nullptr, numiters, damp, thresh, gp, hints, out_T, nullptr,
-                   nullptr, ws, ws_bytes, st, "gs_slam_localize/icp", tape, tape_bytes, compose_right, compose_out);
+                   nullptr, ws, ws_bytes, st, "gs_slam_localize/icp", tape, tape_bytes, compose_right, compose_out, prepared);
+}
+
+int icp_localize_prep(int grad_lm, const float *src, const int32_t *d_ns, int max_ns, const float *tgt, const float *nrm,
+                      const int32_t *d_nt, int max_nt, float damp, float thresh, float lambda_max, float Bp, float B2, float nu,
+                      const gs_icp_hints *hints, float *out_T, void *ws, size_t ws_bytes, LoopPrep *out) {
+    const char *name = "gs_slam_localize/prep";
+    GS_REQUIRE(src && d_ns && tgt && nrm && d_nt && hints && out_T && out && max_ns > 0 && max_nt > 0, "%s: bad arguments", name);
+    GS_REQUIRE(hints->scan_points && hints->scan_orig, "%s: the boxes are the pixel-ordered target's", name);
+    if (!ws || ws_bytes < icp_ws_layout(max_ns, max_nt, nullptr, nullptr)) {
+        set_error("%s: workspace too small", name);
+        return GS_ERR_WORKSPACE_TOO_SMALL;
+    }
+    IcpWs w;
+    icp_ws_layout(max_ns, max_nt, ws, &w);
+    *out = loop_prep(src, d_ns, max_ns, tgt, nrm, d_nt, damp, thresh, grad_lm ? make_grad_params(lambda_max, Bp, B2, nu) : lm_grad_params(),
+                     *hints, out_T, nullptr, w);
+    return GS_OK;
+}
+
+void icp_ws_offsets(int max_ns, int max_nt, size_t *out12) {
+    icp_ws_layout(max_ns, max_nt, nullptr, nullptr, out12);
+    out12[10] = sizeof(LoopConst);
+    out12[11] = offsetof(IcpState, p_cur);
+}
+
+int front_boxes_launch(const float *tgt, const int32_t *d_nt, int cap, const int32_t *row_key, const int *cnt, int npix,
+                       int32_t *pix_start, float *scan_points, int32_t *scan_orig, const LoopPrep &prep, hipStream_t st) {
+    const char *name = "gs_slam_localize/front_boxes";
+    GS_REQUIRE(npix > 0 && npix <= kBucketPixMax && cap > 0, "%s: bad shape", name);
+    const int nrb = std::min(cdiv(cap, SUPER * CHUNK), kRangeBlocksMax);
+    hipLaunchKernelGGL(front_boxes_k, dim3(nrb + kPrepBlocks), dim3(1024), 0, st, tgt, d_nt, cap, (const int2 *)row_key, cnt, npix, pix_start,
+                       scan_points, scan_orig, prep.boxes, prep.sboxes, nrb, (IcpState *)prep.state, prep.damp, prep_lc(prep),
+                       (LoopConst *)prep.lc_out, prep.part0, prep.part1, prep.rows_written, prep.rows_read);
+    GS_LAUNCH_CHECK(name);
+    return GS_OK;
 }
 
 }
diff --git a/gradslam_amd/csrc/project.hip b/gradslam_amd/csrc/project.hip
--- a/gradslam_amd/csrc/project.hip
+++ b/gradslam_amd/csrc/project.hip
@@ -106,7 +106,10 @@
     __device__ void block_init(int pass, int bid, int nb) const {
         if (threadIdx.x == 0) cam_cache()[0] = make_cam(poses, Ks);
         if (pass == 0)
-            for (int i = bid * blockDim.x + threadIdx.x; i < npix; i += nb * blockDim.x) { cnt[i] = 0; fill[i] = 0; }
+            for (int i = bid * blockDim.x + threadIdx.x; i < npix; i += nb * blockDim.x) {
+                cnt[i] = 0;
+                if (fill) fill[i] = 0;
+            }
     }
     struct Item { f3 p; };
     __device__ Item fetch(int64_t i) const { return Item{ld3(points, i)}; }
@@ -133,6 +136,7 @@
     __device__ void operator()(int64_t i, int64_t pos) const { put(ActivePredH::Item{ld3(points, i)}, i, pos); }
 };
 
+template <bool RANK>
 struct ActiveWriterT {
     const float *points, *normals;
     int H, W, ds, Wd;
@@ -146,13 +150,19 @@
         int h, w;
         project_point(cam_cache()[0], it.p, H, W, umax, vmax, h, w);
         const int pix = (h / ds) * Wd + (w / ds);
-        atomicAdd(cnt + pix, 1);
-        row_pix[pos] = pix;
+        int rank = 0;
+        if constexpr (RANK) {
+            rank = atomicAdd(cnt + pix, 1);
+        } else {
+            atomicAdd(cnt + pix, 1);
+            row_pix[pos] = pix;
+        }
         if (pos < cap) {
             st3(tgt, pos, it.p);
             st3(tnrm, pos, ld3(normals, i));
             if (tgt_index) tgt_index[pos] = (int32_t)i;
         }
+        if constexpr (RANK) reinterpret_cast<int2 *>(row_pix)[pos] = make_int2(pix, rank);
     }
     __device__ void operator()(int64_t i, int64_t pos) const { put(ActivePredH::Item{ld3(points, i)}, i, pos); }
 };
@@ -449,7 +459,8 @@
 int project_front1(const float *depth, const float *points, const int32_t *counts, int Nmax, const float *poses, const float *intrinsics,
                    int H, int W, int ds, const float *map_normals, int cap, float *vertex, float *normal, float *gvertex, float *gnormal,
                    float *cam_out, int32_t *row_pix, float *tgt, float *tnrm, int32_t *nt, int32_t *tgt_index, float *scan_points,
-                   int32_t *scan_orig, int32_t *pix_start, const DsJob &frame, void *ws, size_t ws_bytes, hipStream_t st) {
+                   int32_t *scan_orig, int32_t *pix_start, const DsJob &frame, void *ws, size_t ws_bytes, hipStream_t st,
+                   const LoopPrep *prep) {
     const char *name = "gs_slam_localize/front";
     if (!ws || ws_bytes < project_target1_ws_bytes(H, W, ds, Nmax)) {
         set_error("%s: workspace too small", name);
@@ -466,8 +477,9 @@
     unsigned char *flags = (unsigned char *)p; p += compact_flags_bytes(Nmax);
     int *countsB = (int *)p;
     const float umax = (float)((double)W - 0.999), vmax = (float)((double)H - 0.999);
-    ActivePredH pa{points, counts, poses, intrinsics, Nmax, H, W, ds, umax, vmax, cnt, fill, npix};
-    ActiveWriterT wa{points, map_normals, H, W, ds, Wd, umax, vmax, cnt, cap, tgt, tnrm, tgt_index, row_pix};
+    ActivePredH pa{points, counts, poses, intrinsics, Nmax, H, W, ds, umax, vmax, cnt, prep ? nullptr : fill, npix};
+    ActiveWriterT<false> wa{points, map_normals, H, W, ds, Wd, umax, vmax, cnt, cap, tgt, tnrm, tgt_index, row_pix};
+    const ActiveWriterT<true> wr{points, map_normals, H, W, ds, Wd, umax, vmax, cnt, cap, tgt, tnrm, tgt_index, row_pix};
     DsPred pb{frame.depth, W, Wd, ds};
     DsWriter wb{frame.gvertex, nullptr, nullptr, frame.out_points, nullptr, nullptr, frame.out_pix, W, Wd, ds};
     const int64_t nA = Nmax, nB = (int64_t)npix;
@@ -480,18 +492,22 @@
     hipLaunchKernelGGL((setup_count_k<ActivePredH, DsPred>), dim3(nbA + nbB + nbV), dim3(kCT), 0, st, nA, pa, countsA, flags, nbA, nB, pb,
                        countsB, nbB, depth, intrinsics, poses, H, W, gx, vertex, normal, gvertex, gnormal, ex);
     GS_LAUNCH_CHECK(name);
-    if (nbA <= kSelfScanBlocks) {
-        hipLaunchKernelGGL((compact_write2_k<ActivePredH, ActiveWriterT, true, DsPred, DsWriter>), dim3(nbA + nbB), dim3(kCT), 0, st, nA, pa, wa,
-                           (const int *)countsA, nt, (const unsigned char *)flags, nbA, nB, pb, wb, (const int *)countsB, frame.count, nbB);
-    } else {
-        int *offsetsA = countsA + nbA;
-        hipLaunchKernelGGL(compact_scan_k, dim3(1), dim3(1024), 0, st, countsA, nbA, offsetsA, nt);
-        GS_LAUNCH_CHECK(name);
-        hipLaunchKernelGGL((compact_write2_k<ActivePredH, ActiveWriterT, false, DsPred, DsWriter>), dim3(nbA + nbB), dim3(kCT), 0, st, nA, pa, wa,
-                           (const int *)offsetsA, (int *)nullptr, (const unsigned char *)flags, nbA, nB, pb, wb, (const int *)countsB,
-                           frame.count, nbB);
-    }
+    auto write2 = [&](auto writer) {
+        using WA = decltype(writer);
+        if (nbA <= kSelfScanBlocks) {
+            hipLaunchKernelGGL((compact_write2_k<ActivePredH, WA, true, DsPred, DsWriter>), dim3(nbA + nbB), dim3(kCT), 0, st, nA, pa, writer,
+                               (const int *)countsA, nt, (const unsigned char *)flags, nbA, nB, pb, wb, (const int *)countsB, frame.count, nbB);
+        } else {
+            int *offsetsA = countsA + nbA;
+            hipLaunchKernelGGL(compact_scan_k, dim3(1), dim3(1024), 0, st, countsA, nbA, offsetsA, nt);
+            hipLaunchKernelGGL((compact_write2_k<ActivePredH, WA, false, DsPred, DsWriter>), dim3(nbA + nbB), dim3(kCT), 0, st, nA, pa, writer,
+                               (const int *)offsetsA, (int *)nullptr, (const unsigned char *)flags, nbA, nB, pb, wb, (const int *)countsB,
+                               frame.count, nbB);
+        }
+    };
+    if (prep) write2(wr); else write2(wa);
     GS_LAUNCH_CHECK(name);
+    if (prep) return front_boxes_launch(tgt, nt, cap, row_pix, cnt, npix, pix_start, scan_points, scan_orig, *prep, st);
     hipLaunchKernelGGL(bucket_scatter_k, dim3(std::min(cdiv(cap, 1024), kBucketBlocks)), dim3(1024), 0, st, (const float *)tgt,
                        (const int32_t *)nt, cap, (const int32_t *)row_pix, (const int *)cnt, fill, npix, pix_start, scan_points, scan_orig);
     GS_LAUNCH_CHECK(name);
diff --git a/gradslam_amd/csrc/slam.hip b/gradslam_amd/csrc/slam.hip
--- a/gradslam_amd/csrc/slam.hip
+++ b/gradslam_amd/csrc/slam.hip
@@ -141,6 +141,9 @@
     float *cam;
     void *sub;
     size_t sub_bytes;
+    void *icp;
+    size_t icp_bytes;
+    size_t icp_off;
 };
 
 static inline int target_cap(int Nmax) {
@@ -159,9 +162,12 @@
     w.rows = c.take<int64_t>((size_t)B * capT * 32); w.nrows = c.take<int32_t>(4);
     w.tgt = c.take<float>((size_t)B * capT * 12); w.tnrm = c.take<float>((size_t)B * capT * 12); w.nt = c.take<int32_t>((size_t)B * 4);
     w.T = c.take<float>((size_t)B * 64); w.eye = c.take<float>((size_t)B * 64); w.cam = c.take<float>((size_t)B * 128);
-    w.sub_bytes = std::max({gs_downsample_frame_ws_bytes(H, W, ds), gs_project_active_ws_bytes(B, Nmax), gs_gather_table_rows_ws_bytes(B),
-                            gs_bucket_by_pixel_ws_bytes(B, H, W, ds), gs_icp_ws_bytes(capS, capT), project_target1_ws_bytes(H, W, ds, Nmax)});
+    w.sub_bytes = std::max({gs_downsample_frame_ws_bytes(H, W, ds), gs_project_active_ws_bytes(B, capT), gs_gather_table_rows_ws_bytes(B),
+                            gs_bucket_by_pixel_ws_bytes(B, H, W, ds), project_target1_ws_bytes(H, W, ds, capT)});
     w.sub = c.take(w.sub_bytes);
+    w.icp_bytes = gs_icp_ws_bytes(capS, capT);
+    w.icp_off = c.off;
+    w.icp = c.take(w.icp_bytes);
     return c.off;
 }
 
@@ -170,17 +176,24 @@
     return g_fused_setup != 0 && B == 1 && (int64_t)cdiv(H, ds) * cdiv(W, ds) <= kBucketPixMax;
 }
 
+constexpr int FRONT_BOXES_DENSE = 64;
+static int g_front_boxes = getenv("GS_FRONT_BOXES") ? atoi(getenv("GS_FRONT_BOXES")) : 1;
+static inline bool front_boxes(int B, int H, int W, int ds, int capT, int numiters) {
+    if (g_front_boxes <= 0 || numiters <= 0 || !fused_front(B, H, W, ds)) return false;
+    return g_front_boxes >= 2 || (int64_t)capT <= (int64_t)FRONT_BOXES_DENSE * cdiv(H, ds) * cdiv(W, ds);
+}
+
 static int enqueue_front(const float *depth, const float *gvertex, const float *intrinsics, const float *prev_poses, int B, int H, int W,
                          int ds, const float *map_points, const float *map_normals, const int32_t *map_counts, int Nmax, const LocWs &w,
                          float *src, int32_t *src_pix, int32_t *ns, int32_t *nt, int32_t *tgt_index, bool compute_maps, float *vertex,
-                         float *normal, float *gvertex_out, float *gnormal, float *cam_out, hipStream_t st) {
+                         float *normal, float *gvertex_out, float *gnormal, float *cam_out, hipStream_t st, const LoopPrep *prep) {
     const int capS = cdiv(H, ds) * cdiv(W, ds), capT = target_cap(Nmax);
     const DsJob frame{depth, gvertex, src, src_pix, ns};
     int rc;
     if (fused_front(B, H, W, ds))
         return project_front1(compute_maps ? depth : nullptr, map_points, map_counts, Nmax, prev_poses, intrinsics, H, W, ds, map_normals,
                               capT, vertex, normal, gvertex_out, gnormal, cam_out, (int32_t *)w.rows, w.tgt, w.tnrm, nt, tgt_index, w.scan,
-                              w.scan_orig, w.pix_start, frame, w.sub, w.sub_bytes, st);
+                              w.scan_orig, w.pix_start, frame, w.sub, w.sub_bytes, st, prep);
     if (compute_maps &&
         (rc = vertex_normal_maps_cam(depth, intrinsics, prev_poses, B, H, W, vertex, normal, gvertex_out, gnormal, cam_out, st))) return rc;
     if (B == 1)
@@ -369,6 +382,11 @@
 
 void gs_set_fused_setup(int on) { g_fused_setup = on; }
 
+int gs_set_front_boxes(int mode) {
+    if (mode >= 0 && mode <= 2) g_front_boxes = mode;
+    return g_front_boxes;
+}
+
 int gs_graph_stats(double *out4) {
     GS_REQUIRE(out4, "gs_graph_stats: NULL argument");
     std::lock_guard<std::mutex> lock(g_graph_mu);
@@ -386,6 +404,16 @@
 size_t gs_slam_localize_ws_bytes(int B, int H, int W, int ds, int Nmax) {
     if (B <= 0 || H <= 0 || W <= 0 || ds <= 0 || Nmax <= 0) return 0;
     return loc_layout(B, H, W, ds, Nmax, nullptr, nullptr);
+}
+
+int gs_slam_localize_ws_offsets(int B, int H, int W, int ds, int Nmax, size_t *out12) {
+    GS_REQUIRE(out12 && B > 0 && H > 0 && W > 0 && ds > 0 && Nmax > 0, "gs_slam_localize_ws_offsets: bad arguments");
+    LocWs w;
+    loc_layout(B, H, W, ds, Nmax, nullptr, &w);
+    icp_ws_offsets(cdiv(H, ds) * cdiv(W, ds), target_cap(Nmax), out12);
+    for (int q = 0; q < 10; ++q)
+        if (q != 7 && q != 9) out12[q] += w.icp_off;
+    return GS_OK;
 }
 
 int gs_slam_localize(const float *depth, const float *intrinsics, const float *prev_poses, int B, int H, int W, int ds,
@@ -405,15 +433,24 @@
     loc_layout(B, H, W, ds, Nmax, ws, &w);
     const int capS = cdiv(H, ds) * cdiv(W, ds), capT = target_cap(Nmax);
     int rc;
+    const bool boxes = front_boxes(B, H, W, ds, capT, numiters);
+    LoopPrep prep;
+    if (boxes) {
+        const gs_icp_hints hints = loc_hints(w, w.src_pix, 0, H, W, ds, capS, capT, w.cam, w.cam + 16);
+        if ((rc = icp_localize_prep(use_grad_lm, w.src, w.ns, capS, w.tgt, w.tnrm, w.nt, capT, damp, dist_thresh, lambda_max, Bp, B2, nu,
+                                    &hints, w.T, w.icp, w.icp_bytes, &prep))) return rc;
+    }
     if ((rc = enqueue_front(depth, gvertex, intrinsics, prev_poses, B, H, W, ds, map_points, map_normals, map_counts, Nmax, w, w.src,
-                            w.src_pix, w.ns, w.nt, nullptr, true, vertex, normal, gvertex, gnormal, w.cam, st))) return rc;
+                            w.src_pix, w.ns, w.nt, nullptr, true, vertex, normal, gvertex, gnormal, w.cam, st, boxes ? &prep : nullptr)))
+        return rc;
     auto enqueue_loops = [&](hipStream_t s, bool fold_compose) -> int {
         for (int b = 0; b < B; ++b) {
             const gs_icp_hints hints = loc_hints(w, w.src_pix, b, H, W, ds, capS, capT, w.cam + 32 * b, w.cam + 32 * b + 16);
             const int r = icp_localize_run(use_grad_lm, w.src + (size_t)b * capS * 3, w.ns + b, capS, w.tgt + (size_t)b * capT * 3,
                                            w.tnrm + (size_t)b * capT * 3, w.nt + b, capT, numiters, damp, dist_thresh, lambda_max, Bp,
-                                           B2, nu, &hints, w.T + 16 * b, w.sub, w.sub_bytes, s, nullptr, 0,
-                                           fold_compose ? prev_poses + 16 * b : nullptr, fold_compose ? out_poses + 16 * b : nullptr);
+                                           B2, nu, &hints, w.T + 16 * b, w.icp, w.icp_bytes, s, nullptr, 0,
+                                           fold_compose ? prev_poses + 16 * b : nullptr, fold_compose ? out_poses + 16 * b : nullptr,
+                                           boxes ? &prep : nullptr);
             if (r) return r;
         }
         return GS_OK;
@@ -421,12 +458,12 @@
     bool launched = false;
     if (graphs_allowed() && numiters > 0) {
         const GraphKey key{ws, B, capS, capT, numiters, use_grad_lm, damp, dist_thresh, lambda_max, Bp, B2, nu,
-                           icp_config_stamp(), H, W, ds};
+                           icp_config_stamp() | ((boxes ? 1 : 0) << 20), H, W, ds};
         if ((rc = graph_replay(key, st, [&](hipStream_t cs) { return enqueue_loops(cs, false); }, &launched))) return rc;
     }
     if (!launched) {
         if (numiters > 0)
-            return eager_timed(B * ((use_grad_lm ? 2 * numiters : numiters + 1) + 2), [&] { return enqueue_loops(st, true); });
+            return eager_timed(B * ((use_grad_lm ? 2 * numiters : numiters + 1) + (boxes ? 1 : 2)), [&] { return enqueue_loops(st, true); });
         if ((rc = enqueue_loops(st, false))) return rc;
     }
     return gs_compose_poses(w.T, prev_poses, B, out_poses, stream);
@@ -594,14 +631,22 @@
     loc_tape_layout(B, H, W, ds, Nmax, numiters, use_grad_lm, tape, &tp);
     const int capS = cdiv(H, ds) * cdiv(W, ds), capT = target_cap(Nmax);
     int rc;
+    const bool boxes = front_boxes(B, H, W, ds, capT, numiters);
+    LoopPrep prep;
+    if (boxes) {
+        const gs_icp_hints hints = loc_hints(w, tp.src_pix, 0, H, W, ds, capS, capT, prev_poses, intrinsics);
+        if ((rc = icp_localize_prep(use_grad_lm, tp.src, tp.ns, capS, w.tgt, w.tnrm, tp.nt, capT, damp, dist_thresh, lambda_max, Bp, B2, nu,
+                                    &hints, tp.T, w.icp, w.icp_bytes, &prep))) return rc;
+    }
     if ((rc = enqueue_front(depth, gvertex, intrinsics, prev_poses, B, H, W, ds, map_points, map_normals, map_counts, Nmax, w, tp.src,
-                            tp.src_pix, tp.ns, tp.nt, tp.tgt_index, false, nullptr, nullptr, nullptr, nullptr, nullptr, st))) return rc;
+                            tp.src_pix, tp.ns, tp.nt, tp.tgt_index, false, nullptr, nullptr, nullptr, nullptr, nullptr, st,
+                            boxes ? &prep : nullptr))) return rc;
     for (int b = 0; b < B; ++b) {
         const gs_icp_hints hints = loc_hints(w, tp.src_pix, b, H, W, ds, capS, capT, prev_poses + 16 * b, intrinsics + 16 * b);
         if ((rc = icp_localize_run(use_grad_lm, tp.src + (size_t)b * capS * 3, tp.ns + b, capS, w.tgt + (size_t)b * capT * 3,
                                    w.tnrm + (size_t)b * capT * 3, tp.nt + b, capT, numiters, damp, dist_thresh, lambda_max, Bp, B2, nu,
-                                   &hints, tp.T + 16 * b, w.sub, w.sub_bytes, st, tp.icp + (size_t)b * tp.icp_bytes, tp.icp_bytes,
-                                   prev_poses + 16 * b, out_poses + 16 * b)))
+                                   &hints, tp.T + 16 * b, w.icp, w.icp_bytes, st, tp.icp + (size_t)b * tp.icp_bytes, tp.icp_bytes,
+                                   prev_poses + 16 * b, out_poses + 16 * b, boxes ? &prep : nullptr)))
             return rc;
     }
     if (numiters == 0) return gs_compose_poses(tp.T, prev_poses, B, out_poses, stream);
diff --git a/include/gradslam_hip.h b/include/gradslam_hip.h
--- a/include/gradslam_hip.h
+++ b/include/gradslam_hip.h
@@ -228,6 +228,7 @@
 int gs_graph_stats(double *out4);
 int gs_compose_poses(const float *T, const float *P, int B, float *out, gs_stream_t stream);
 size_t gs_slam_localize_ws_bytes(int B, int H, int W, int ds, int Nmax);
+int gs_slam_localize_ws_offsets(int B, int H, int W, int ds, int Nmax, size_t *out12);
 int gs_slam_localize(const float *depth, const float *intrinsics, const float *prev_poses, int B,
                      int H, int W, int ds, const float *map_points, const float *map_normals,
                      const int32_t *map_counts, int Nmax, int use_grad_lm, int numiters, float damp,
@@ -241,6 +242,7 @@
 void gs_set_grid_search(int on);
 
 void gs_set_fused_setup(int on);
+int gs_set_front_boxes(int mode);
 
 void gs_set_tile_points(int n);
 int gs_set_loop_waves(int n);
```

Result: slower. 5491 frames/s (-1.2%).
